# LayerXcom/zero-chain

Hardware: AMD Instinct MI355X
Metric: Groth16 proofs/sec (Transfer circuit) (higher is better)
Workload: dtype u32 limbs (Fq 381-bit: 14 x 28-bit; Fr 255-bit: 8 x 32-bit; modular integer arithmetic)

## Files before the change

### include/zkamd.h

```cpp
#ifndef ZKAMD_H
#define ZKAMD_H

#include <stddef.h>
#include <stdint.h>

#ifdef __cplusplus
extern "C" {
#endif

typedef int32_t zk_status;

enum {
    ZK_OK = 0,
    ZK_ERR_ASSIGNMENT_MISSING = 1,
    ZK_ERR_DIVISION_BY_ZERO = 2,
    ZK_ERR_UNSATISFIABLE = 3,
    ZK_ERR_POLYNOMIAL_DEGREE_TOO_LARGE = 4,
    ZK_ERR_UNEXPECTED_IDENTITY = 5,
    ZK_ERR_IO = 6,
    ZK_ERR_MALFORMED_VERIFYING_KEY = 7,
    ZK_ERR_UNCONSTRAINED_VARIABLE = 8,
    ZK_ERR_INVALID_ARGUMENT = 16,
    ZK_ERR_DEVICE = 17,
    ZK_ERR_NO_DEVICE = 18,
    ZK_ERR_OUT_OF_MEMORY = 19
};

#define ZK_FR_MONTGOMERY 1u

const char* zk_strerror(zk_status st);
const char* zk_last_error(void);
zk_status zk_device_count(int* count);
void zk_set_host_threads(int n);

zk_status zk_bind_host_to_device(int device, int* numa_node_out, int* n_cpus_out);

typedef struct zk_params zk_params;

typedef struct {
    uint32_t n_ic, n_h, n_l, n_a, n_b_g1, n_b_g2;
    uint32_t log_domain;
    uint32_t window_bits;
    uint32_t n_windows;
    uint32_t device;
    uint64_t device_bytes;
} zk_params_info;

zk_status zk_params_load(const uint8_t* pk_bytes, size_t len, int checked, int device, zk_params** out);
zk_status zk_params_get_info(const zk_params* p, zk_params_info* info);
zk_status zk_params_get_windows(const zk_params* p, uint32_t out[4]);
zk_status zk_params_get_merged(const zk_params* p, uint32_t out[3]);
void zk_params_free(zk_params* p);

typedef struct {
    uint32_t n_rows;
    uint32_t n_inputs;
    uint32_t n_aux;
    uint32_t flags;
    const uint8_t* a;
    const uint8_t* b;
    const uint8_t* c;
    const uint8_t* inputs;
    const uint8_t* aux;
    const uint8_t* a_aux_density;
    const uint8_t* b_input_density;
    const uint8_t* b_aux_density;
} zk_assignment;

zk_status zk_prove(zk_params* p, const zk_assignment* asg, const uint8_t r[32], const uint8_t s[32],
                   uint8_t proof_out[192]);

zk_status zk_prove_batch(zk_params* p, size_t n, const zk_assignment* asgs, const uint8_t* rs,
                         uint8_t* proofs_out);

typedef struct {
    uint32_t n_rows, n_inputs, n_aux, flags;
    const void* d_a;
    const void* d_b;
    const void* d_c;
    const void* d_wit;
    const uint8_t* a_aux_density;
    const uint8_t* b_input_density;
    const uint8_t* b_aux_density;
} zk_batch_dev;
zk_status zk_prove_batch_dev(zk_params* p, size_t n, const zk_batch_dev* batch, const uint8_t* rs,
                             uint8_t* proofs_out);

typedef struct zk_r1cs zk_r1cs;
typedef struct {
    const uint32_t* row_ptr;
    const uint32_t* col;
    const uint8_t* coeff;
} zk_csr;
zk_status zk_r1cs_load(uint32_t n_inputs, uint32_t n_aux, uint32_t n_constraints, const zk_csr* a, const zk_csr* b,
                       const zk_csr* c, int device, zk_r1cs** out);
void zk_r1cs_free(zk_r1cs* r);
zk_status zk_transfer_r1cs_load(int device, zk_r1cs** out);
zk_status zk_transfer_r1cs_fingerprint(uint8_t hash_out[32], uint32_t* n_inputs, uint32_t* n_aux, uint32_t* n_constraints);
zk_status zk_prove_batch_witness(zk_params* p, zk_r1cs* circuit, size_t n, const uint8_t* witness, uint32_t flags,
                                 const uint8_t* rs, uint8_t* proofs_out);

#define ZK_TRANSFER_N_INPUTS 23u
#define ZK_TRANSFER_N_AUX 19955u
typedef struct {
    uint32_t amount, remaining_balance, fee, reserved;
    uint8_t randomness[32], alpha[32], dec_key_sender[32];
    uint8_t proof_generation_key[32], enc_key_recipient[32], enc_balance_left[32], enc_balance_right[32], g_epoch[32];
} zk_transfer_statement;
zk_status zk_transfer_witness(const zk_transfer_statement* st, size_t n, uint32_t flags, uint8_t* witness_out);
zk_status zk_transfer_prove_batch(zk_params* p, zk_r1cs* circuit, size_t n, const zk_transfer_statement* st,
                                  const uint8_t* rs, uint8_t* proofs_out);
zk_status zk_transfer_witness_gpu(zk_r1cs* circuit, const zk_transfer_statement* st, size_t n, uint32_t flags,
                                  uint8_t* witness_out);

typedef struct zk_pipeline zk_pipeline;
zk_status zk_pipeline_create(zk_params* p, zk_r1cs* circuit, zk_pipeline** out);
zk_status zk_pipeline_submit(zk_pipeline* pl, size_t n, const zk_transfer_statement* st, const uint8_t* rs,
                             uint8_t* proofs_out);
zk_status zk_pipeline_wait(zk_pipeline* pl);
int zk_pipeline_lanes(const zk_pipeline* pl);
void zk_pipeline_free(zk_pipeline* pl);

typedef struct {
    uint32_t amount, fee, remaining_balance, reserved;
    uint8_t spending_key[32];
    uint8_t enc_key_recipient[32], enc_balance_left[32], enc_balance_right[32], g_epoch[32];
    uint8_t randomness[32], alpha[32];
} zk_transfer_request;
typedef struct {
    uint8_t proof[192];
    uint8_t enc_key_sender[32], enc_key_recipient[32], left_amount_sender[32], left_amount_recipient[32], left_fee[32],
        right_randomness[32], rsk[32], rvk[32], enc_balance[64], nonce[32];
} zk_confidential_xt;
zk_status zk_spending_key_from_seed(const uint8_t* seed, size_t len, uint8_t spending_key_out[32]);
// ... 173 lines not shown
```

### include/zkamd_sys.rs

```rust
#![allow(non_camel_case_types, dead_code)]
use std::os::raw::{c_char, c_int, c_void};

pub type zk_status = i32;
pub const ZK_OK: zk_status = 0;
pub const ZK_ERR_ASSIGNMENT_MISSING: zk_status = 1;
pub const ZK_ERR_DIVISION_BY_ZERO: zk_status = 2;
pub const ZK_ERR_UNSATISFIABLE: zk_status = 3;
pub const ZK_ERR_POLYNOMIAL_DEGREE_TOO_LARGE: zk_status = 4;
pub const ZK_ERR_UNEXPECTED_IDENTITY: zk_status = 5;
pub const ZK_ERR_IO: zk_status = 6;
pub const ZK_ERR_MALFORMED_VERIFYING_KEY: zk_status = 7;
pub const ZK_ERR_UNCONSTRAINED_VARIABLE: zk_status = 8;
pub const ZK_ERR_INVALID_ARGUMENT: zk_status = 16;
pub const ZK_ERR_DEVICE: zk_status = 17;
pub const ZK_ERR_NO_DEVICE: zk_status = 18;
pub const ZK_ERR_OUT_OF_MEMORY: zk_status = 19;
pub const ZK_SCAN_SENDER: u8 = 1;
pub const ZK_SCAN_RECIPIENT: u8 = 2;
pub const ZK_SCAN_FOUND_SENT: u8 = 1;
pub const ZK_SCAN_FOUND_FEE: u8 = 2;
pub const ZK_SCAN_FOUND_RECEIVED: u8 = 4;
pub const ZK_PROOF_BAD_ENCODING: u8 = 1;
pub const ZK_PROOF_NOT_ON_CURVE: u8 = 2;
pub const ZK_PROOF_NOT_IN_SUBGROUP: u8 = 3;
// ... 188 lines not shown
pub struct zk_anonymous_statement {
    pub amount: u32,
    pub remaining_balance: u32,
    pub s_index: u32,
    pub t_index: u32,
    pub randomness: [u8; 32],
    pub alpha: [u8; 32],
    pub dec_key: [u8; 32],
    pub proof_generation_key: [u8; 32],
    pub g_epoch: [u8; 32],
    pub enc_keys: [[u8; 32]; ZK_ANONYMOUS_SIZE],
    pub left_ciphertexts: [[u8; 32]; ZK_ANONYMOUS_SIZE],
    pub enc_balances_left: [[u8; 32]; ZK_ANONYMOUS_SIZE],
    pub enc_balances_right: [[u8; 32]; ZK_ANONYMOUS_SIZE],
}
#[repr(C)]
#[derive(Clone, Copy)]
pub struct zk_anonymous_request {
    pub amount: u32,
    pub remaining_balance: u32,
    pub s_index: u32,
    pub t_index: u32,
    pub spending_key: [u8; 32],
    pub enc_key_recipient: [u8; 32],
    pub enc_keys_decoy: [[u8; 32]; { ZK_ANONYMOUS_SIZE - 2 }],
    pub enc_balances_left: [[u8; 32]; ZK_ANONYMOUS_SIZE],
    pub enc_balances_right: [[u8; 32]; ZK_ANONYMOUS_SIZE],
    pub g_epoch: [u8; 32],
    pub randomness: [u8; 32],
    pub alpha: [u8; 32],
}
#[repr(C)]
#[derive(Clone, Copy)]
pub struct zk_anonymous_xt {
    pub proof: [u8; 192],
    pub enc_keys: [[u8; 32]; ZK_ANONYMOUS_SIZE],
    pub left_ciphertexts: [[u8; 32]; ZK_ANONYMOUS_SIZE],
    pub right_ciphertext: [u8; 32],
    pub nonce: [u8; 32],
    pub rsk: [u8; 32],
    pub rvk: [u8; 32],
}
#[repr(C)]
#[derive(Clone, Copy)]
pub struct zk_block_account {
    pub enc_key: [u8; 32],
    pub balance: [u8; 64],
    pub pending: [u8; 64],
    pub flags: u32,
}
#[repr(C)]
#[derive(Clone, Copy)]
pub struct zk_block_verdict {
    pub verdict: u8,
    pub detail: u8,
    pub reserved: [u8; 2],
}
#[repr(C)]
#[derive(Clone, Copy)]
pub struct zk_block_stats {
    pub rounds: u32,
    pub proofs_verified: u32,
    pub points_decoded: u32,
    pub reserved: u32,
}

#[link(name = "zkamd")]
extern "C" {
    pub fn zk_strerror(st: zk_status) -> *const c_char;
    pub fn zk_last_error() -> *const c_char;
    pub fn zk_device_count(count: *mut c_int) -> zk_status;
    pub fn zk_set_host_threads(n: c_int);
    pub fn zk_bind_host_to_device(device: c_int, numa_node_out: *mut c_int, n_cpus_out: *mut c_int) -> zk_status;
    pub fn zk_params_load(
        pk_bytes: *const u8,
        len: usize,
        checked: c_int,
        device: c_int,
        out: *mut *mut zk_params,
    ) -> zk_status;
    pub fn zk_params_get_info(p: *const zk_params, info: *mut zk_params_info) -> zk_status;
    pub fn zk_params_get_windows(p: *const zk_params, out: *mut [u32; 4]) -> zk_status;
    pub fn zk_params_get_merged(p: *const zk_params, out: *mut [u32; 3]) -> zk_status;
    pub fn zk_params_free(p: *mut zk_params);
    pub fn zk_prove(
        p: *mut zk_params,
        asg: *const zk_assignment,
        r: *const [u8; 32],
        s: *const [u8; 32],
        proof_out: *mut [u8; 192],
    ) -> zk_status;
    pub fn zk_prove_batch(
        p: *mut zk_params,
        n: usize,
        asgs: *const zk_assignment,
        rs: *const u8,
        proofs_out: *mut u8,
    ) -> zk_status;
    pub fn zk_prove_batch_dev(
        p: *mut zk_params,
        n: usize,
        batch: *const zk_batch_dev,
        rs: *const u8,
        proofs_out: *mut u8,
    ) -> zk_status;
    pub fn zk_r1cs_load(
        n_inputs: u32,
        n_aux: u32,
        n_constraints: u32,
        a: *const zk_csr,
        b: *const zk_csr,
        c: *const zk_csr,
        device: c_int,
        out: *mut *mut zk_r1cs,
    ) -> zk_status;
    pub fn zk_r1cs_free(r: *mut zk_r1cs);
    pub fn zk_transfer_r1cs_load(device: c_int, out: *mut *mut zk_r1cs) -> zk_status;
    pub fn zk_transfer_r1cs_fingerprint(
        hash_out: *mut [u8; 32],
        n_inputs: *mut u32,
        n_aux: *mut u32,
        n_constraints: *mut u32,
    ) -> zk_status;
    pub fn zk_prove_batch_witness(
        p: *mut zk_params,
        circuit: *mut zk_r1cs,
        n: usize,
        witness: *const u8,
        flags: u32,
        rs: *const u8,
        proofs_out: *mut u8,
    ) -> zk_status;
    pub fn zk_transfer_witness(st: *const zk_transfer_statement, n: usize, flags: u32, witness_out: *mut u8) -> zk_status;
    pub fn zk_transfer_prove_batch(
        p: *mut zk_params,
        circuit: *mut zk_r1cs,
        n: usize,
        st: *const zk_transfer_statement,
        rs: *const u8,
        proofs_out: *mut u8,
    ) -> zk_status;
    pub fn zk_transfer_witness_gpu(
        circuit: *mut zk_r1cs,
        st: *const zk_transfer_statement,
        n: usize,
        flags: u32,
        witness_out: *mut u8,
    ) -> zk_status;
    pub fn zk_pipeline_create(p: *mut zk_params, circuit: *mut zk_r1cs, out: *mut *mut zk_pipeline) -> zk_status;
    pub fn zk_pipeline_submit(
        pl: *mut zk_pipeline,
        n: usize,
        st: *const zk_transfer_statement,
        rs: *const u8,
        proofs_out: *mut u8,
    ) -> zk_status;
    pub fn zk_pipeline_wait(pl: *mut zk_pipeline) -> zk_status;
    pub fn zk_pipeline_lanes(pl: *const zk_pipeline) -> c_int;
    pub fn zk_pipeline_free(pl: *mut zk_pipeline);
    pub fn zk_spending_key_from_seed(seed: *const u8, len: usize, spending_key_out: *mut [u8; 32]) -> zk_status;
    pub fn zk_jubjub_base_mul(scalars: *const u8, n: usize, points_out: *mut u8) -> zk_status;
    pub fn zk_elgamal_encrypt(
        values: *const u32,
        randomness: *const u8,
        enc_keys: *const u8,
        n: usize,
// ... 243 lines not shown
```

### zero-chain_amd/_api.py

```python
import ctypes as C

import numpy as np

from . import _lib
from ._shard import shard_bounds, gather_proofs, prove_sharded
from ._lib import (ZkError, ZkLib, ZK_FR_MONTGOMERY, ZK_NTT_INVERSE, ZK_NTT_COSET, ZK_NTT_IN_BITREV,
                   ZK_NTT_OUT_BITREV)

__all__ = ["Parameters", "Proof", "generate_parameters", "generate_random_parameters", "PreparedVerifyingKey", "prepare_verifying_key", "verify_proof", "verify_proofs", "read_proofs",
           "verify_transfer_batch", "jubjub_into_xy", "redjubjub_sign", "redjubjub_verify", "REDJUBJUB_REASONS", "verify_confidential_xts", "verify_anonymous_xts", "execute_confidential_block", "g_epoch", "BLOCK_VERDICTS", "BLOCK_ROLLOVER_DUE", "BLOCK_ROLLED", "INTO_XY_REASONS", "SCAN_SENDER", "SCAN_RECIPIENT", "CONFIDENTIAL_XT_POINTS", "ANONYMOUS_XT_POINTS", "ProvingAssignment", "create_proof", "create_random_proof", "create_proofs", "create_proofs_dev", "stream", "bind_host_to_device", "KernelTimer", "kernel_forms",
           "multiexp", "multiexp_cache_release", "memory_stats", "MultiexpContext", "ConstraintMatrices", "create_proofs_from_witness", "fs_rand", "spending_key_from_seed", "jubjub_base_mul", "elgamal_encrypt", "ElGamalTable", "elgamal_add", "ledger_apply", "LEDGER_SUBTRACT", "LEDGER_SKIP", "LEDGER_SCAN_WIDTH", "balance_query", "ELGAMAL_DECRYPT_LIMIT", "ZERO_CIPHERTEXT", "transfer_requests", "transfer_derive", "gen_proofs", "xt_fields", "gen_proof", "XT_FIELDS",
           "FS_MODULUS", "transfer_statements", "transfer_witness", "transfer_witness_gpu", "transfer_r1cs_fingerprint", "anonymous_r1cs_fingerprint", "ANONYMOUS_N_INPUTS", "ANONYMOUS_N_AUX", "anonymous_statements", "anonymous_requests", "anonymous_derive", "anonymous_gen_proofs", "anonymous_witness", "anonymous_witness_gpu", "anonymous_prove_batch",
           "transfer_prove_batch", "TransferPipeline", "set_host_threads", "TRANSFER_N_INPUTS", "TRANSFER_N_AUX", "EvaluationDomain", "XorShiftRng", "fr_rand", "ZkError", "FR_MODULUS",
           "scalars_to_bytes", "bytes_to_scalars", "load_library", "ZK_FR_MONTGOMERY", "ZK_NTT_INVERSE",
           "ZK_NTT_COSET", "ZK_NTT_IN_BITREV", "ZK_NTT_OUT_BITREV", "shard_bounds", "gather_proofs", "prove_sharded"]

FR_MODULUS = 0x73eda753299d7d483339d80809a1d80553bda402fffe5bfeffffffff00000001
_FR_R_INV = pow(1 << 256, -1, FR_MODULUS)
PROOF_SIZE = 192


def load_library():
    return _lib.load()

# ... 76 lines not shown

def fr_rand(rng):
    while True:
        limbs = [rng.next_u64() for _ in range(4)]
        limbs[3] &= 0xFFFFFFFFFFFFFFFF >> 1
        v = sum(l << (64 * i) for i, l in enumerate(limbs))
        if v < FR_MODULUS:
            return v * _FR_R_INV % FR_MODULUS


class Proof:

    def __init__(self, data):
        data = bytes(data)
        if len(data) != PROOF_SIZE:
            raise ValueError("a proof is exactly 192 bytes")
        self.bytes = data

    @property
    def a(self):
        return self.bytes[:48]

    @property
    def b(self):
        return self.bytes[48:144]

    @property
    def c(self):
        return self.bytes[144:]

    def write(self, writer=None):
        if writer is not None:
            writer.write(self.bytes)
        return self.bytes

    @classmethod
    def read(cls, reader):
        data = reader if isinstance(reader, (bytes, bytearray)) else reader.read(PROOF_SIZE)
        return cls(data)

    def __eq__(self, other):
        return isinstance(other, Proof) and other.bytes == self.bytes

    def __repr__(self):
        return "Proof(%s)" % self.bytes.hex()


class Parameters:

    def __init__(self, lib, handle, pk_bytes):
        self._lib = lib
        self._h = handle
        self._pk = pk_bytes
        info = _lib.ParamsInfo()
        lib.check(lib.zk_params_get_info(handle, C.byref(info)))
        self.info = {f[0]: getattr(info, f[0]) for f in info._fields_}
        self.info.update(zip(("n_merged_a", "n_merged_b1", "n_merged_b2"), self.merged_bases))

    @classmethod
    def read(cls, reader, checked=True, device=0, lib=None):
        lib = lib or _lib.load()
        data = bytes(reader if isinstance(reader, (bytes, bytearray)) else reader.read())
        buf = _u8(data)
        h = C.c_void_p()
        lib.check(lib.zk_params_load(_ptr(buf), buf.size, 1 if checked else 0, device, C.byref(h)))
        return cls(lib, h, data)

    def write(self, writer=None):
        if writer is not None:
            writer.write(self._pk)
        return self._pk

    @property
    def windows(self):
        w = (C.c_uint32 * 4)()
        self._lib.check(self._lib.zk_params_get_windows(self._h, w))
        return tuple(int(x) for x in w)

    @property
    def merged_bases(self):
        n = (C.c_uint32 * 3)()
        self._lib.check(self._lib.zk_params_get_merged(self._h, n))
        return tuple(int(x) for x in n)

    @property
    def vk(self):
        n_ic = self.info["n_ic"]
        b = self._pk
        return {"alpha_g1": b[0:96], "beta_g1": b[96:192], "beta_g2": b[192:384], "gamma_g2": b[384:576],
                "delta_g1": b[576:672], "delta_g2": b[672:864],
                "ic": [b[868 + 96 * i: 868 + 96 * (i + 1)] for i in range(n_ic)]}

    def close(self):
        if self._h:
            self._lib.zk_params_free(self._h)
            self._h = None

    def __del__(self):
        try:
            self.close()
        except Exception:
            pass


G1_GENERATOR = bytes.fromhex(
    "17f1d3a73197d7942695638c4fa9ac0fc3688c4f9774b905a14e3a3f171bac586c55e83ff97a1aeffb3af00adb22c6bb"
    "08b3f481e3aaa0f1a09e30ed741d8ae4fcf5e095d5d00af600db18cb2c04b3edd03cc744a2888ae40caa232946c5e7e1")
G2_GENERATOR = bytes.fromhex(
    "13e02b6052719f607dacd3a088274f65596bd0d09920b61ab5da61bbdc7f5049334cf11213945d57e5ac7d055d042b7e"
    "024aa2b2f08f0a91260805272dc51051c6e47ad4fa403b02b4510b647ae3d1770bac0326a805bbefd48056c8c121bdb8"
    "0606c4a02ea734cc32acd2b02bc28b99cb3e287e85a763af267492ab572e99ab3f370d275cec1da1aaa9075ff05f79be"
    "0ce5d527727d6e118cc9cdc6da2e351aadfd9baa8cbdd3a76d429a695160d12c923ac9cc3baca289e193548608b82801")


def generate_parameters(matrices, alpha, beta, gamma, delta, tau, g1=None, g2=None):
    lib = matrices._lib
    sc = [scalars_to_bytes([int(v)]) for v in (alpha, beta, gamma, delta, tau)]
    b1, b2 = _u8(g1 or G1_GENERATOR, 96), _u8(g2 or G2_GENERATOR, 192)
    n = C.c_size_t(0)
    args = [matrices._h, _ptr(b1), _ptr(b2)] + [_ptr(x) for x in sc]
    lib.check(lib.zk_generate_parameters(*args, None, 0, C.byref(n)))
    out = np.zeros(n.value, dtype=np.uint8)
    lib.check(lib.zk_generate_parameters(*args, _ptr(out), out.size, C.byref(n)))
    return out[:n.value].tobytes()


def generate_random_parameters(matrices, rng, g1=None, g2=None):
    alpha, beta, gamma, delta, tau = (fr_rand(rng) for _ in range(5))
    return generate_parameters(matrices, alpha, beta, gamma, delta, tau, g1=g1, g2=g2)


class PreparedVerifyingKey:

    def __init__(self, lib, handle):
        self._lib = lib
        self._h = handle
        n = C.c_uint32(0)
        lib.check(lib.zk_vk_num_inputs(handle, C.byref(n)))
        self.n_inputs = n.value

    @classmethod
    def read(cls, reader, device=0, lib=None):
        lib = lib or _lib.load()
        buf = _u8(bytes(reader if isinstance(reader, (bytes, bytearray)) else reader.read()))
        h = C.c_void_p()
        lib.check(lib.zk_vk_read(_ptr(buf), buf.size, device, C.byref(h)))
        return cls(lib, h)

    def write(self, writer=None):
        n = C.c_size_t(0)
        self._lib.check(self._lib.zk_vk_write(self._h, None, 0, C.byref(n)))
        out = np.zeros(n.value, dtype=np.uint8)
        self._lib.check(self._lib.zk_vk_write(self._h, _ptr(out), out.size, C.byref(n)))
        data = out.tobytes()
        if writer is not None:
            writer.write(data)
        return data

    def close(self):
        if self._h:
            self._lib.zk_vk_free(self._h)
            self._h = None

    def __del__(self):
        try:
            self.close()
# ... 926 lines not shown
```

### zero-chain_amd/_lib.py

```python
import ctypes as C
import os

HERE = os.path.dirname(os.path.abspath(__file__))
LIB_PATH = os.path.join(HERE, "libzkamd.so")
HOOKS_LIB_PATH = os.path.join(HERE, "libzkamd_hooks.so")

ZK_OK = 0
ZK_FR_MONTGOMERY = 1
ZK_NTT_INVERSE, ZK_NTT_COSET, ZK_NTT_IN_BITREV, ZK_NTT_OUT_BITREV = 1, 2, 4, 8

STATUS_NAMES = {
    0: "Ok", 1: "AssignmentMissing", 2: "DivisionByZero", 3: "Unsatisfiable",
    4: "PolynomialDegreeTooLarge", 5: "UnexpectedIdentity", 6: "IoError",
    7: "MalformedVerifyingKey", 8: "UnconstrainedVariable", 16: "InvalidArgument",
    17: "DeviceError", 18: "NoDevice", 19: "OutOfMemory",
}


class ZkError(Exception):

    def __init__(self, status, detail):
        self.status = status
        self.variant = STATUS_NAMES.get(status, "Unknown")
        super().__init__("%s (%d): %s" % (self.variant, status, detail))
# ... 11 lines not shown


class Csr(C.Structure):
    _fields_ = [("row_ptr", C.c_void_p), ("col", C.c_void_p), ("coeff", C.c_void_p)]


class TransferStatement(C.Structure):
    _fields_ = [("amount", C.c_uint32), ("remaining_balance", C.c_uint32), ("fee", C.c_uint32), ("reserved", C.c_uint32)] + \
               [(n, C.c_uint8 * 32) for n in ("randomness", "alpha", "dec_key_sender", "proof_generation_key",
                                              "enc_key_recipient", "enc_balance_left", "enc_balance_right", "g_epoch")]


class TransferRequest(C.Structure):
    _fields_ = [("amount", C.c_uint32), ("fee", C.c_uint32), ("remaining_balance", C.c_uint32), ("reserved", C.c_uint32)] + \
               [(n, C.c_uint8 * 32) for n in ("spending_key", "enc_key_recipient", "enc_balance_left", "enc_balance_right",
                                              "g_epoch", "randomness", "alpha")]


class ConfidentialXt(C.Structure):
    _fields_ = [("proof", C.c_uint8 * 192)] + \
               [(n, C.c_uint8 * 32) for n in ("enc_key_sender", "enc_key_recipient", "left_amount_sender", "left_amount_recipient",
                                              "left_fee", "right_randomness", "rsk", "rvk")] + \
               [("enc_balance", C.c_uint8 * 64), ("nonce", C.c_uint8 * 32)]


class AnonymousStatement(C.Structure):
    _fields_ = [("amount", C.c_uint32), ("remaining_balance", C.c_uint32), ("s_index", C.c_uint32), ("t_index", C.c_uint32)] + \
               [(n, C.c_uint8 * 32) for n in ("randomness", "alpha", "dec_key", "proof_generation_key", "g_epoch")] + \
               [(n, (C.c_uint8 * 32) * 12) for n in ("enc_keys", "left_ciphertexts", "enc_balances_left", "enc_balances_right")]


class AnonymousRequest(C.Structure):
    _fields_ = [("amount", C.c_uint32), ("remaining_balance", C.c_uint32), ("s_index", C.c_uint32), ("t_index", C.c_uint32),
                ("spending_key", C.c_uint8 * 32), ("enc_key_recipient", C.c_uint8 * 32), ("enc_keys_decoy", (C.c_uint8 * 32) * 10),
                ("enc_balances_left", (C.c_uint8 * 32) * 12), ("enc_balances_right", (C.c_uint8 * 32) * 12),
                ("g_epoch", C.c_uint8 * 32), ("randomness", C.c_uint8 * 32), ("alpha", C.c_uint8 * 32)]


class AnonymousXt(C.Structure):
    _fields_ = [("proof", C.c_uint8 * 192), ("enc_keys", (C.c_uint8 * 32) * 12), ("left_ciphertexts", (C.c_uint8 * 32) * 12)] + \
               [(n, C.c_uint8 * 32) for n in ("right_ciphertext", "nonce", "rsk", "rvk")]


class LedgerOp(C.Structure):
    _fields_ = [("slot", C.c_uint32), ("flags", C.c_uint32), ("left", C.c_uint8 * 32), ("right", C.c_uint8 * 32)]


class BlockAccount(C.Structure):
    _fields_ = [("enc_key", C.c_uint8 * 32), ("balance", C.c_uint8 * 64), ("pending", C.c_uint8 * 64), ("flags", C.c_uint32)]


class BlockVerdict(C.Structure):
    _fields_ = [("verdict", C.c_uint8), ("detail", C.c_uint8), ("reserved", C.c_uint16)]


class BlockStats(C.Structure):
    _fields_ = [(n, C.c_uint32) for n in ("rounds", "proofs_verified", "points_decoded", "reserved")]


class ConfidentialScanResult(C.Structure):
    _fields_ = [("role", C.c_uint8), ("found", C.c_uint8), ("refusal", C.c_uint8), ("reserved", C.c_uint8),
                ("amount_sent", C.c_uint32), ("fee", C.c_uint32), ("amount_received", C.c_uint32)]


class AnonymousScanResult(C.Structure):
    _fields_ = [("members", C.c_uint16), ("found", C.c_uint8), ("refusal", C.c_uint8), ("reserved", C.c_uint32), ("delta", C.c_int64)]


class BatchDev(C.Structure):
    _fields_ = [("n_rows", C.c_uint32), ("n_inputs", C.c_uint32), ("n_aux", C.c_uint32), ("flags", C.c_uint32),
                ("d_a", C.c_void_p), ("d_b", C.c_void_p), ("d_c", C.c_void_p), ("d_wit", C.c_void_p),
                ("a_aux_density", C.c_void_p), ("b_input_density", C.c_void_p), ("b_aux_density", C.c_void_p)]


_PROTOS = {
    "zk_strerror": (C.c_char_p, [C.c_int32]),
    "zk_last_error": (C.c_char_p, []),
    "zk_device_count": (C.c_int32, [C.POINTER(C.c_int)]),
    "zk_set_host_threads": (None, [C.c_int]),
    "zk_params_load": (C.c_int32, [C.c_void_p, C.c_size_t, C.c_int, C.c_int, C.POINTER(C.c_void_p)]),
    "zk_params_get_info": (C.c_int32, [C.c_void_p, C.POINTER(ParamsInfo)]),
    "zk_params_get_windows": (C.c_int32, [C.c_void_p, C.POINTER(C.c_uint32)]),
    "zk_params_get_merged": (C.c_int32, [C.c_void_p, C.POINTER(C.c_uint32)]),
    "zk_bind_host_to_device": (C.c_int32, [C.c_int, C.POINTER(C.c_int), C.POINTER(C.c_int)]),
    "zk_params_free": (None, [C.c_void_p]),
    "zk_prove": (C.c_int32, [C.c_void_p, C.POINTER(Assignment), C.c_void_p, C.c_void_p, C.c_void_p]),
    "zk_prove_batch": (C.c_int32, [C.c_void_p, C.c_size_t, C.POINTER(Assignment), C.c_void_p, C.c_void_p]),
    "zk_prove_batch_dev": (C.c_int32, [C.c_void_p, C.c_size_t, C.POINTER(BatchDev), C.c_void_p, C.c_void_p]),
    "zk_r1cs_load": (C.c_int32, [C.c_uint32, C.c_uint32, C.c_uint32, C.POINTER(Csr), C.POINTER(Csr), C.POINTER(Csr), C.c_int,
                                 C.POINTER(C.c_void_p)]),
    "zk_r1cs_free": (None, [C.c_void_p]),
    "zk_transfer_r1cs_load": (C.c_int32, [C.c_int, C.POINTER(C.c_void_p)]),
    "zk_transfer_r1cs_fingerprint": (C.c_int32, [C.c_void_p, C.POINTER(C.c_uint32), C.POINTER(C.c_uint32), C.POINTER(C.c_uint32)]),
    "zk_anonymous_r1cs_load": (C.c_int32, [C.c_int, C.POINTER(C.c_void_p)]),
    "zk_anonymous_derive": (C.c_int32, [C.POINTER(AnonymousRequest), C.c_size_t, C.POINTER(AnonymousStatement), C.c_void_p]),
    "zk_anonymous_gen_proof_batch": (C.c_int32, [C.c_void_p, C.c_void_p, C.c_void_p, C.c_size_t, C.POINTER(AnonymousRequest), C.c_void_p,
                                                 C.POINTER(AnonymousXt)]),
    "zk_anonymous_r1cs_fingerprint": (C.c_int32, [C.c_void_p, C.POINTER(C.c_uint32), C.POINTER(C.c_uint32), C.POINTER(C.c_uint32)]),
    "zk_prove_batch_witness": (C.c_int32, [C.c_void_p, C.c_void_p, C.c_size_t, C.c_void_p, C.c_uint32, C.c_void_p, C.c_void_p]),
    "zk_transfer_witness": (C.c_int32, [C.POINTER(TransferStatement), C.c_size_t, C.c_uint32, C.c_void_p]),
    "zk_transfer_witness_gpu": (C.c_int32, [C.c_void_p, C.POINTER(TransferStatement), C.c_size_t, C.c_uint32, C.c_void_p]),
    "zk_transfer_prove_batch": (C.c_int32, [C.c_void_p, C.c_void_p, C.c_size_t, C.POINTER(TransferStatement), C.c_void_p,
                                            C.c_void_p]),
    "zk_pipeline_create": (C.c_int32, [C.c_void_p, C.c_void_p, C.POINTER(C.c_void_p)]),
    "zk_pipeline_submit": (C.c_int32, [C.c_void_p, C.c_size_t, C.POINTER(TransferStatement), C.c_void_p, C.c_void_p]),
    "zk_pipeline_wait": (C.c_int32, [C.c_void_p]),
    "zk_pipeline_lanes": (C.c_int, [C.c_void_p]),
    "zk_pipeline_free": (None, [C.c_void_p]),
    "zk_spending_key_from_seed": (C.c_int32, [C.c_void_p, C.c_size_t, C.c_void_p]),
    "zk_jubjub_base_mul": (C.c_int32, [C.c_void_p, C.c_size_t, C.c_void_p]),
    "zk_elgamal_encrypt": (C.c_int32, [C.c_void_p, C.c_void_p, C.c_void_p, C.c_size_t, C.c_void_p, C.c_void_p]),
    "zk_elgamal_table_create": (C.c_int32, [C.c_uint32, C.c_int, C.POINTER(C.c_void_p)]),
    "zk_elgamal_decrypt": (C.c_int32, [C.c_void_p, C.c_size_t, C.c_void_p, C.c_void_p, C.c_void_p, C.c_size_t, C.c_uint64, C.c_void_p,
                                       C.c_void_p]),
    "zk_elgamal_table_free": (None, [C.c_void_p]),
    "zk_elgamal_add": (C.c_int32, [C.c_void_p, C.c_void_p, C.c_void_p, C.c_void_p, C.c_size_t, C.c_int, C.c_void_p, C.c_void_p]),
    "zk_confidential_scan": (C.c_int32, [C.c_void_p, C.c_size_t, C.POINTER(ConfidentialXt), C.c_void_p, C.c_uint64,
                                         C.POINTER(ConfidentialScanResult)]),
    "zk_anonymous_scan": (C.c_int32, [C.c_void_p, C.c_size_t, C.POINTER(AnonymousXt), C.c_void_p, C.c_uint64, C.POINTER(AnonymousScanResult)]),
    "zk_elgamal_ledger_apply": (C.c_int32, [C.c_size_t, C.c_void_p, C.c_size_t, C.POINTER(LedgerOp), C.c_int, C.c_void_p, C.c_void_p, C.c_void_p,
                                            C.c_void_p]),
    "zk_transfer_derive": (C.c_int32, [C.POINTER(TransferRequest), C.c_size_t, C.POINTER(TransferStatement), C.c_void_p]),
    "zk_transfer_gen_proof_batch": (C.c_int32, [C.c_void_p, C.c_void_p, C.c_void_p, C.c_size_t, C.POINTER(TransferRequest), C.c_void_p,
                                                C.POINTER(ConfidentialXt)]),
    "zk_anonymous_witness": (C.c_int32, [C.POINTER(AnonymousStatement), C.c_size_t, C.c_uint32, C.c_void_p]),
    "zk_anonymous_witness_gpu": (C.c_int32, [C.c_void_p, C.POINTER(AnonymousStatement), C.c_size_t, C.c_uint32, C.c_void_p]),
    "zk_generate_parameters": (C.c_int32, [C.c_void_p] + [C.c_void_p] * 7 + [C.c_void_p, C.c_size_t, C.POINTER(C.c_size_t)]),
    "zk_params_write_vk": (C.c_int32, [C.c_void_p, C.c_void_p, C.c_size_t, C.POINTER(C.c_size_t)]),
    "zk_vk_prepare": (C.c_int32, [C.c_void_p, C.c_size_t, C.c_int, C.POINTER(C.c_void_p)]),
    "zk_vk_read": (C.c_int32, [C.c_void_p, C.c_size_t, C.c_int, C.POINTER(C.c_void_p)]),
    "zk_vk_write": (C.c_int32, [C.c_void_p, C.c_void_p, C.c_size_t, C.POINTER(C.c_size_t)]),
    "zk_vk_num_inputs": (C.c_int32, [C.c_void_p, C.POINTER(C.c_uint32)]),
    "zk_vk_free": (None, [C.c_void_p]),
    "zk_verify_batch": (C.c_int32, [C.c_void_p, C.c_size_t, C.c_void_p, C.c_void_p, C.c_size_t, C.c_void_p]),
    "zk_verify_batch_rlc": (C.c_int32, [C.c_void_p, C.c_size_t, C.c_void_p, C.c_void_p, C.c_size_t, C.c_void_p]),
    "zk_verify_proof": (C.c_int32, [C.c_void_p, C.c_void_p, C.c_void_p, C.c_size_t, C.POINTER(C.c_int)]),
    "zk_proof_read_batch": (C.c_int32, [C.c_void_p, C.c_size_t, C.c_void_p, C.c_void_p]),
    "zk_jubjub_into_xy": (C.c_int32, [C.c_void_p, C.c_size_t, C.c_int, C.c_void_p, C.c_void_p]),
    "zk_confidential_verify_batch": (C.c_int32, [C.c_void_p, C.c_size_t, C.POINTER(ConfidentialXt), C.c_void_p, C.c_void_p, C.c_size_t,
                                                 C.c_void_p, C.c_void_p]),
    "zk_anonymous_verify_batch": (C.c_int32, [C.c_void_p, C.c_size_t, C.POINTER(AnonymousXt), C.c_void_p, C.c_void_p, C.c_size_t,
                                              C.c_void_p, C.c_void_p]),
    "zk_confidential_block_execute": (C.c_int32, [C.c_void_p, C.c_size_t, C.POINTER(ConfidentialXt), C.c_void_p, C.c_void_p, C.c_void_p, C.c_size_t,
                                                  C.POINTER(BlockAccount), C.c_size_t, C.c_void_p, C.c_void_p, C.POINTER(BlockAccount),
                                                  C.POINTER(BlockVerdict), C.POINTER(BlockStats)]),
    "zk_g_epoch": (C.c_int32, [C.c_uint32, C.c_void_p]),
    "zk_redjubjub_sign": (C.c_int32, [C.c_size_t, C.c_void_p, C.c_void_p, C.c_void_p, C.c_void_p, C.c_void_p]),
    "zk_redjubjub_verify_batch": (C.c_int32, [C.c_size_t, C.c_void_p, C.c_void_p, C.c_void_p, C.c_void_p, C.c_int, C.c_void_p, C.c_void_p]),
    "zk_anonymous_prove_batch": (C.c_int32, [C.c_void_p, C.c_void_p, C.c_size_t, C.POINTER(AnonymousStatement), C.c_void_p,
                                             C.c_void_p]),
    "zk_msm_create": (C.c_int32, [C.c_int, C.c_void_p, C.c_size_t, C.c_int, C.c_int, C.c_int, C.POINTER(C.c_void_p)]),
    "zk_msm_create_variable": (C.c_int32, [C.c_int, C.c_void_p, C.c_size_t, C.c_int, C.c_int, C.c_int, C.POINTER(C.c_void_p)]),
    "zk_msm_run": (C.c_int32, [C.c_void_p, C.c_void_p, C.c_uint32, C.c_void_p]),
    "zk_msm_run_dev": (C.c_int32, [C.c_void_p, C.c_void_p, C.c_uint32, C.c_void_p]),
    "zk_msm_free": (None, [C.c_void_p]),
    "zk_msm_g1": (C.c_int32, [C.c_void_p, C.c_void_p, C.c_size_t, C.c_void_p]),
    "zk_msm_g2": (C.c_int32, [C.c_void_p, C.c_void_p, C.c_size_t, C.c_void_p]),
    "zk_msm_cache_release": (None, []),
    "zk_memory_stats": (None, [C.POINTER(C.c_uint64)]),
    "zk_ntt_fr": (C.c_int32, [C.c_void_p, C.c_uint32, C.c_int, C.c_int]),
    "zk_ntt_create": (C.c_int32, [C.c_uint32, C.c_int, C.POINTER(C.c_void_p)]),
    "zk_ntt_run_dev": (C.c_int32, [C.c_void_p, C.c_void_p, C.c_uint32, C.c_uint32]),
    "zk_ntt_free": (None, [C.c_void_p]),
    "zk_debug_field_mul": (C.c_int32, [C.c_int, C.c_void_p, C.c_void_p, C.c_void_p, C.c_size_t]),
    "zk_profile_begin": (None, []),
    "zk_profile_get": (C.c_int, [C.c_char_p, C.POINTER(C.c_double)]),
# ... 44 lines not shown
```

### zero-chain_amd/csrc/msm_group.h

```cpp
#pragma once
#include <stdio.h>
#include <stdlib.h>
#include <string.h>
#include <string>
#include <vector>
#include <algorithm>
#include <utility>
#include <mutex>
#include "../../include/zkamd.h"
#include "gpu_rt.h"
#include "host_common.h"
#include "host_math.h"
#include "msm.h"
#include "coop_tail.h"
#include "msm_plan.h"

namespace zkrt {

inline uint32_t pick_window(size_t n, int group) {
    const char* env = getenv(group == 2 ? "ZKAMD_WINDOW_BITS_G2" : group == 3 ? "ZKAMD_WINDOW_BITS_G1A" : "ZKAMD_WINDOW_BITS_G1");
    if (!env) env = getenv("ZKAMD_WINDOW_BITS");
    if (env && atoi(env) >= 2 && atoi(env) <= 22) return (uint32_t)atoi(env);
    const char* benv = getenv(group == 2 ? "ZKAMD_BUCKET_COST_G2" : "ZKAMD_BUCKET_COST_G1");
    const double beta = benv && atof(benv) > 0 ? atof(benv) : (group == 2 ? 12.0 : group == 1 ? 4.0 : 6.0);
// ... 70 lines not shown
#ifdef ZK_HAVE_RED_ASM
template <> constexpr bool asm_reduce<zkdev::Fq28>() { return true; }
template <>
void launch_red_asm<zkdev::Fq28>(const zkdev::XYZZ<zkdev::Fq28>* tsums, const uint32_t* cnt, const uint32_t* toff, const uint32_t* tbase,
                                 zkdev::XYZZ<zkdev::Fq28>* S, zkdev::XYZZ<zkdev::Fq28>* A, uint32_t nb, uint32_t L, dim3 grid,
                                 hipStream_t st, uint32_t* n_fallback, uint32_t* fallback);
#endif
#ifdef ZK_HAVE_MADD_ASM
int persist_wgs(int group = 1);
template <> constexpr bool asm_loop<zkdev::Fq28>() { return true; }
template <> constexpr bool asm_loop<zkdev::Fq2x>() { return true; }
template <>
void launch_asm_loop<zkdev::Fq28>(const zkdev::Affine<zkdev::Fq28>* table, const uint32_t* pairs, const uint4* sorted,
                                  const uint32_t* d_total, zkdev::XYZZ<zkdev::Fq28>* tsums, uint32_t* d_nredo, uint32_t* redo,
                                  unsigned blocks, hipStream_t st);
template <>
void launch_asm_loop<zkdev::Fq2x>(const zkdev::Affine<zkdev::Fq2x>* table, const uint32_t* pairs, const uint4* sorted,
                                  const uint32_t* d_total, zkdev::XYZZ<zkdev::Fq2x>* tsums, uint32_t* d_nredo, uint32_t* redo,
                                  unsigned blocks, hipStream_t st);
#endif

template <class HF, class DF>
struct MsmGroup {
    typedef zkhost::Affine<HF> HAffine;
    typedef zkhost::Point<HF> HPoint;
    typedef zkdev::Affine<DF> DAffine;
    typedef zkdev::XYZZ<DF> DPoint;
    static_assert(sizeof(HAffine) == 2 * 4 * zkdev::HostWords<DF>::N, "host affine layout");
    static_assert(sizeof(HPoint) == 4 * 4 * zkdev::HostWords<DF>::N, "host point layout");

    static constexpr bool IS_G2 = zkdev::HostWords<DF>::N == 24;

    uint32_t c = 0, maxd = 0, nb = 0;
    size_t n_points = 0;
    DevBuf table;
    DevBuf jobs_d, cnt, off, toff, ntasks, hist, tclass, sorted, heavy, light, blockbase, coarse, tbase, rank, pairs, tsums, red_r, red_w, red_t, result, redo;
    DPoint* res_dev = nullptr;
    PinBuf pin_jobs;
    size_t bytes = 0;
    DevBuf dstat;

    zk_status set_geometry(uint32_t c_, size_t n, bool with_table) {
        c = c_;
        maxd = with_table ? zkdev::msm_max_digits(c) : 1u;
        nb = 1u << (c - 2);
        n_points = n;
        const uint32_t npos = with_table ? zkdev::MSM_NPOS : 1u;
        if ((uint64_t)n_points * npos >= (1ull << 31)) return fail(ZK_ERR_INVALID_ARGUMENT, "doubling table too large");
        bytes = sizeof(DAffine) * n_points * npos;
        return ZK_OK;
    }
    void alias(const MsmGroup& o, uint32_t c_) {
        (void)set_geometry(c_, o.n_points, true);
        bytes = 0;
        table.borrow(o.table);
    }
    zk_status decode_enqueue(const uint8_t* bases, size_t n, uint32_t c_, bool with_table, DevBuf& raw, DevBuf& map, hipStream_t st);
    zk_status decode_finish(const char* what, uint32_t* n_inf, size_t* bad_index = nullptr) {
        uint32_t v[2] = {0xffffffffu, 0};
        HIP_TRY(hipMemcpy(v, dstat.p, 8, hipMemcpyDeviceToHost));
        if (v[0] != 0xffffffffu) {
            if (bad_index) *bad_index = v[0];
            return fail(ZK_ERR_IO, std::string("invalid ") + (IS_G2 ? "G2" : "G1") + " encoding at " + what + " " + std::to_string(v[0]));
        }
        *n_inf = v[1];
        return ZK_OK;
    }
    zk_status table_enqueue(DevBuf& scratch, hipStream_t st);
    zk_status finish_build(bool checked, const char* what, bool with_table);
    zk_status build(const std::vector<HAffine>& pts, uint32_t c_, bool checked, const char* what, bool with_table = true);

    zk_status build_with_tail(const std::vector<HAffine>& pts, const MsmGroup& o, size_t from, size_t count, uint32_t c_);

    zk_status enqueue(std::vector<MsmJob>& jobs, std::vector<HPoint>& out, hipStream_t st, bool to_host = true);
    zk_status normalize_to_host(const DPoint* src, size_t n, HPoint* out, DevBuf& stage, hipStream_t st);
    zk_status export_to_host(const DPoint* src, size_t n, HPoint* out, DevBuf& stage, hipStream_t st);
    zk_status normalize2_to_host(const DPoint* src0, const DPoint* src1, size_t n, HPoint* out0, HPoint* out1, DevBuf& stage0,
                                 DevBuf& stage1, hipStream_t st);
    zk_status collect(hipStream_t st) {
        HIP_TRY(hipStreamSynchronize(st));
        return ZK_OK;
    }
    zk_status run(std::vector<MsmJob>& jobs, std::vector<HPoint>& out);

private:
    zk_status launch_table_build(DevBuf& scratch, hipStream_t st);
    zk_status reserve(const MsmPlan& p, bool to_host);
    zk_status upload_jobs(const std::vector<MsmJob>& jobs, const MsmPlan& p, hipStream_t st);
    zk_status sort_pairs(const MsmPlan& p, hipStream_t st);
    zk_status order_tasks(const MsmPlan& p, hipStream_t st);
    zk_status accumulate(const MsmPlan& p, hipStream_t st);
    zk_status merge_partials(const MsmPlan& p, hipStream_t st);
    zk_status level1(const MsmPlan& p, hipStream_t st);
    zk_status tail(const MsmPlan& p, hipStream_t st);
    zk_status copy_to_host(const DevBuf& stage, size_t n, HPoint* out, hipStream_t st);
    void dump_redo(const MsmPlan& p, hipStream_t st, bool after_level1);
    void dump_heavy(const MsmPlan& p, hipStream_t st);
    enum Counter { N_TASKS = 0, N_HEAVY = 1, N_REDO = 2, N_LIGHT = 4, N_FALLBACK = 5 };
    uint32_t* counter(const MsmPlan& p, Counter k) const { return hist.as<uint32_t>() + 2 * p.n_class + k; }
    DPoint* node_s() const { return red_r.as<DPoint>(); }
    DPoint* node_w() const { return red_w.as<DPoint>(); }
    DPoint* job_sums(const MsmPlan& p) const { return node_w() + p.nj * (size_t)p.T; }
};

typedef MsmGroup<zkhost::Fq, zkdev::Fq> MsmG1;
typedef zkdev::Fq2x DevFq2;
typedef MsmGroup<zkhost::Fq2, DevFq2> MsmG2;
typedef zkhost::Affine<zkhost::Fq> HG1A;
typedef zkhost::Affine<zkhost::Fq2> HG2A;
typedef zkhost::Point<zkhost::Fq> HG1;
typedef zkhost::Point<zkhost::Fq2> HG2;

zk_status calibrate_g2_accumulate(const zkdev::Affine<DevFq2>* table, uint32_t n_entries, float ms[2]);
zk_status calibrate_g1_reduce(const zkdev::Affine<zkdev::Fq28>* table, uint32_t n_entries, float ms[2]);

#ifndef ZK_MSM_GROUP_INSTANTIATE
extern template struct MsmGroup<zkhost::Fq, zkdev::Fq>;
extern template struct MsmGroup<zkhost::Fq2, DevFq2>;
extern template zk_status check_points_dev<zkhost::Fq, zkdev::Fq>(const zkdev::Affine<zkdev::Fq>*, size_t, const char*);
extern template zk_status check_points_dev<zkhost::Fq2, DevFq2>(const zkdev::Affine<DevFq2>*, size_t, const char*);
extern template zk_status check_points_host<zkhost::Fq, zkdev::Fq>(const std::vector<zkhost::Affine<zkhost::Fq>>&, const char*);
extern template zk_status check_points_host<zkhost::Fq2, DevFq2>(const std::vector<zkhost::Affine<zkhost::Fq2>>&, const char*);
#endif

}
```

### zero-chain_amd/csrc/ntt.h

```cpp
#pragma once
#include "dev_field.h"
#include "prove_plan.h"

namespace zkdev {

constexpr int NTT_MAX_G = 8;
constexpr int NTT_TILE_LOG = 10;
constexpr int NTT_THREADS = 256;
constexpr int NTT_BIG_LOG = 17, NTT_BIG_MAX_G = 10, NTT_BIG_TILE_LOG = 12, NTT_BIG_THREADS = 1024;

struct NttPass {
    uint32_t log_n;
    uint32_t t0;
    uint32_t g;
    uint32_t log_cw;
    uint32_t dif;
    uint32_t stride;
    uint32_t src_stride;
    uint32_t src_valid;
};

ZK_DI Fr ld_fr(const uint32_t* p) {
    Fr r;
    const uint4* q = reinterpret_cast<const uint4*>(p);
// ... 161 lines not shown
        if (e & 1u) r = mul(r, base);
        base = sqr(base);
        e >>= 1;
    }
    return r;
}

static __global__ void __launch_bounds__(256)
k_fr_pow_table(uint32_t* out, const uint32_t* __restrict__ base, const uint32_t* __restrict__ scale,
               uint32_t log_n, uint32_t mode, uint32_t raw_out, uint32_t count) {
    uint32_t i = blockIdx.x * blockDim.x + threadIdx.x;
    if (i >= count) return;
    uint32_t e = i;
    if (mode == 1) e = log_n ? (__builtin_bitreverse32(i) >> (32 - log_n)) : 0;
    Fr v;
    if (mode == 3) {
        v = Fr::zero();
        v.l[0] = log_n ? (__builtin_bitreverse32(i) >> (32 - log_n)) : 0;
        v = to_mont(v);
    } else {
        v = fr_pow_u32(ld_fr(base), e);
    }
    if (mode) v = mul(v, ld_fr(scale));
    if (raw_out) v = from_mont(v);
    st_fr(out + (size_t)i * 8, v);
}

static __global__ void __launch_bounds__(256)
k_fr_convert(uint32_t* out, const uint32_t* __restrict__ in, uint32_t from, size_t count, uint32_t* bad = nullptr) {
    size_t i = (size_t)blockIdx.x * blockDim.x + threadIdx.x;
    if (i >= count) return;
    Fr v = ld_fr(in + i * 8);
    if (bad && fr_geq_r(v)) raise_flag(bad, ZK_BAD_SCALAR);
    st_fr(out + i * 8, from ? from_mont(v) : to_mont(v));
}

static __global__ void __launch_bounds__(256)
k_fr_first_noncanonical(const uint32_t* __restrict__ in, size_t count, uint32_t* stat) {
    size_t i = (size_t)blockIdx.x * blockDim.x + threadIdx.x;
    if (i >= count) return;
    if (fr_geq_r(ld_fr(in + i * 8))) atomicMin(&stat[0], (uint32_t)i);
}

template <class C>
static __global__ void __launch_bounds__(64)
k_field_mul_raw(uint32_t* out, const uint32_t* __restrict__ a, const uint32_t* __restrict__ b, uint32_t n) {
    uint32_t i = blockIdx.x * blockDim.x + threadIdx.x;
    if (i >= n) return;
    Fp<C> x, y;
#pragma unroll
    for (int j = 0; j < C::N; j++) {
        x.l[j] = a[(size_t)i * C::N + j];
        y.l[j] = b[(size_t)i * C::N + j];
    }
    Fp<C> z = mul(x, y);
#pragma unroll
    for (int j = 0; j < C::N; j++) out[(size_t)i * C::N + j] = z.l[j];
}

struct R1csMat {
    const uint32_t* row_ptr;
    const uint32_t* col;
    const uint32_t* coeff;
};
static __global__ void __launch_bounds__(256)
k_r1cs_eval(R1csMat ma, R1csMat mb, R1csMat mc, const uint32_t* __restrict__ z, uint32_t* out, uint32_t n_con,
            uint32_t n_in, uint32_t nv, uint32_t n_rows, size_t out_mat_stride) {
    uint32_t row = blockIdx.x * blockDim.x + threadIdx.x;
    if (row >= n_rows) return;
    const uint32_t mat = blockIdx.y;
    const size_t p = blockIdx.z;
    const R1csMat m = mat == 0 ? ma : (mat == 1 ? mb : mc);
    const uint32_t* zp = z + p * (size_t)nv * 8;
    Fr acc = Fr::zero();
    if (row < n_con) {
        for (uint32_t k = m.row_ptr[row]; k < m.row_ptr[row + 1]; k++)
            acc = add(acc, mul(ld_fr(m.coeff + (size_t)k * 8), ld_fr(zp + (size_t)m.col[k] * 8)));
    } else if (mat == 0) {
        acc = ld_fr(zp + (size_t)(row - n_con) * 8);
    }
    st_fr(out + (size_t)mat * out_mat_stride * 8 + (p * n_rows + row) * 8, acc);
}

static __global__ void __launch_bounds__(256)
k_build_scalars(uint32_t* wit_out, uint32_t* cvec, const uint32_t* __restrict__ wit, const uint32_t* __restrict__ tail,
                const zkrt::CJobLayout L, uint32_t mont, uint32_t* bad, const uint32_t* __restrict__ groups) {
    uint32_t i = blockIdx.x * blockDim.x + threadIdx.x;
    if (i >= L.wstride + L.gb1) return;
    const size_t p = blockIdx.y;
    uint32_t* cv = cvec + p * (size_t)L.cstride * 8;
    const uint32_t nv = L.w_one, fold = L.fold;
    Fr r = ld_fr(tail + (p * 3 + 1) * 8);
    Fr sR = fold ? mul(ld_fr(tail + (p * 3 + 2) * 8), Fr::r2()) : Fr::zero();
    Fr v;
    if (i >= L.w_sum_a) {
        const uint32_t g = i - L.w_sum_a;
        const uint32_t* mem = groups + (L.ga + L.gb2 + L.gb1 + 1);
        Fr sum = Fr::zero();
        for (uint32_t k = groups[g]; k < groups[g + 1]; k++) {
            const Fr raw = ld_fr(wit + (p * nv + mem[k]) * 8);
            if (!fr_geq_r(raw)) sum = add(sum, raw);
        }
        if (i < L.wstride) {
            v = mont ? from_mont(sum) : sum;
            if (fold && g < L.ga) st_fr(cv + (size_t)(L.sum_a + g) * 8, mul(v, sR));
            st_fr(wit_out + (p * L.wstride + i) * 8, v);
        } else {
            const Fr rz = mont ? mul(sum, r) : mul(mul(sum, r), Fr::r2());
            st_fr(cv + (size_t)(L.sum_b1 + (i - L.wstride)) * 8, rz);
        }
        return;
    }
    if (i < nv) {
        Fr raw = ld_fr(wit + (p * nv + i) * 8);
        if (fr_geq_r(raw)) {
            raise_flag(bad, ZK_BAD_SCALAR);
            raw = Fr::zero();
        }
        if (i == 0 && !(mont ? raw == Fr::one() : (raw.l[0] == 1u && (raw.l[1] | raw.l[2] | raw.l[3] | raw.l[4] | raw.l[5] | raw.l[6] | raw.l[7]) == 0u)))
            raise_flag(bad, ZK_BAD_ONE);
        Fr rz;
        if (mont) {
            v = from_mont(raw);
            rz = mul(raw, r);
        } else {
            v = raw;
            rz = mul(mul(raw, r), Fr::r2());
        }
        if (i >= L.n_in) st_fr(cv + (size_t)(L.aux + (i - L.n_in)) * 8, v);
        st_fr(cv + (size_t)(L.rz + i) * 8, rz);
        if (fold) st_fr(cv + (size_t)(L.sz + i) * 8, mul(v, sR));
        if (L.in_tail && i < L.n_in) st_fr(cv + (size_t)(L.in_tail + i) * 8, v);
    } else {
        v = ld_fr(tail + (p * 3 + (i - nv)) * 8);
        if (i == nv) st_fr(cv + (size_t)L.r * 8, r);
        if (fold && i == nv + 1) st_fr(cv + (size_t)L.rs * 8, mul(r, sR));
        if (fold && i == nv + 2) st_fr(cv + (size_t)L.s * 8, v);
    }
    st_fr(wit_out + (p * L.wstride + i) * 8, v);
}

}
```

### zero-chain_amd/csrc/prove_plan.h

```cpp
#pragma once
#include <stddef.h>
#include <stdint.h>
#include <stdlib.h>

namespace zkrt {

constexpr size_t PROVE_FOLD_IN_MSM_MAX = 128;

struct ProveTunables {
    size_t batch_chunk;
    size_t host_chunk;
    size_t fold_in_msm_max;
    size_t g2_lone_max;
    size_t host_normalize_max;
    size_t split_min;
    bool no_overlap;
    bool trace_host;

    static ProveTunables read() {
        auto env_chunk = [](const char* name, size_t dflt) {
            const char* e = getenv(name);
            return e && atoi(e) > 0 ? (size_t)atoi(e) : dflt;
        };
        auto env_n = [](const char* name, size_t dflt) {
            const char* e = getenv(name);
            return e ? (size_t)atoll(e) : dflt;
        };
        ProveTunables t;
        t.batch_chunk = env_chunk("ZKAMD_BATCH_CHUNK", 1024);
        t.host_chunk = env_chunk("ZKAMD_HOST_CHUNK", 0);
        t.fold_in_msm_max = env_n("ZKAMD_FOLD_IN_MSM_MAX", PROVE_FOLD_IN_MSM_MAX);
        t.g2_lone_max = env_n("ZKAMD_G2_LONE_MAX", 2);
        t.host_normalize_max = env_n("ZKAMD_HOST_NORMALIZE_MAX", 16);
        t.split_min = env_n("ZKAMD_SPLIT_MIN", 64);
        t.no_overlap = getenv("ZKAMD_NO_OVERLAP") != nullptr;
        t.trace_host = getenv("ZKAMD_TRACE_HOST") != nullptr;
        return t;
    }
};

struct CJobLayout {
    uint32_t n_in, n_aux, head, ga, gb2, gb1, fold, derived;
    uint32_t w_one, w_sum_a, w_sum_b2, wstride;
    uint32_t aux, rz, r;
    uint32_t sz, s, rs;
    uint32_t in_tail;
    uint32_t sum_b1, sum_a;
    uint32_t cstride;
};

inline CJobLayout cjob_layout(uint32_t n_in, uint32_t n_aux, uint32_t head, uint32_t ga, uint32_t gb2, uint32_t gb1, bool fold,
                              bool derived) {
    const uint32_t nv = n_in + n_aux;
    CJobLayout L = {};
    L.n_in = n_in; L.n_aux = n_aux; L.head = head; L.ga = ga; L.gb2 = gb2; L.gb1 = gb1; L.fold = fold; L.derived = derived;
    L.w_one = nv;
    L.w_sum_a = nv + 3;
    L.w_sum_b2 = L.w_sum_a + ga;
    L.wstride = L.w_sum_b2 + gb2;
    uint32_t at = head;
    auto section = [&at](uint32_t len) { const uint32_t off = at; at += len; return off; };
    L.aux = section(n_aux);
    L.rz = section(nv);
    L.r = section(1);
    if (fold) {
        L.sz = section(nv);
        L.s = section(1);
        L.rs = section(1);
    }
    if (derived) L.in_tail = section(n_in);
    L.sum_b1 = section(gb1);
    if (fold) L.sum_a = section(ga);
    L.cstride = at;
    return L;
}

enum class PG1 { G1, G1_LONE, G1D, G1D_LONE };
enum class PMap { MAP_C, MAP_CF, MAP_CD, MAP_CFD };

struct ProvePlan {
    bool fold_in_msm;
    bool host_norm;
    bool g2_lone;
    bool split;
    bool one_stream;
    PG1 g1;
    PMap map;
    CJobLayout layout;
};

inline ProvePlan prove_plan(size_t np, uint32_t n_in, uint32_t n_aux, uint32_t n_rows, size_t m, uint32_t ga, uint32_t gb2,
                            uint32_t gb1, bool derived, const ProveTunables& tun) {
    ProvePlan p;
    p.fold_in_msm = np <= tun.fold_in_msm_max;
    p.host_norm = np <= tun.host_normalize_max;
    p.g2_lone = np <= tun.g2_lone_max;
    p.split = np >= tun.split_min;
    p.one_stream = tun.no_overlap;
    p.g1 = derived ? (p.split ? PG1::G1D : PG1::G1D_LONE) : (p.split ? PG1::G1 : PG1::G1_LONE);
    p.map = derived ? (p.fold_in_msm ? PMap::MAP_CFD : PMap::MAP_CD) : (p.fold_in_msm ? PMap::MAP_CF : PMap::MAP_C);
    p.layout = cjob_layout(n_in, n_aux, derived ? 2 * n_rows : (uint32_t)m, ga, gb2, gb1, p.fold_in_msm, derived);
    return p;
}

}
```

### zero-chain_amd/csrc/zkamd.cpp

```cpp
#include <stdio.h>
#include <stdlib.h>
#include <string.h>
#include <string>
#include <vector>
#include <map>
#include <thread>
#include <chrono>
#include <algorithm>
#include <new>
#include <mutex>
#include <condition_variable>
#include <deque>
#if defined(__linux__)
#include <sched.h>
#endif

#include "../../include/zkamd.h"
#include "gpu_rt.h"
#include "host_common.h"
#include "host_math.h"
#include "ntt.h"
#include "msm_group.h"
#include "prove_plan.h"
#include "transfer_witness.h"
#include "handles.h"
#include "transfer_r1cs.h"

using zkdev::MsmJob;
using zkdev::NttPass;

namespace {

using namespace zkrt;

using zkhost::Fr;

Fr fr_from_u64(uint64_t v) {
    Fr x = Fr::zero();
    x.l[0] = v;
    return x.to_mont();
}
Fr fr_const(const uint64_t (&v)[4]) {
    Fr x;
    for (int i = 0; i < 4; i++) x.l[i] = v[i];
    return x;
}


struct NttPlan {
    uint32_t log_n = 0;
    size_t n = 0;
    DevBuf tw_fwd, tw_inv;
    DevBuf s1_plain, s1_mont, s2;
    DevBuf sc_plain, sc_mont;
    DevBuf coset_fwd, coset_inv;
    DevBuf dt;
    DevBuf consts;
    Fr w_inv, n_inv, z_inv;
    DevBuf scratch;
    size_t bytes = 0;

    static int tile_form() {
        static const int f = [] {
            const char* e = getenv("ZKAMD_NTT_TILES");
            return !e ? 1 : !strcmp(e, "big") ? 2 : !strcmp(e, "small") ? 0 : 1;
        }();
        return f;
    }
    static bool big(uint32_t k) { return tile_form() == 2 && k >= (uint32_t)zkdev::NTT_BIG_LOG; }
    static bool mid(uint32_t k) { return tile_form() == 1 && k >= (uint32_t)zkdev::NTT_BIG_LOG; }
    static uint32_t threads_for(uint32_t k) { return mid(k) ? 512u : big(k) ? (uint32_t)zkdev::NTT_BIG_THREADS : (uint32_t)zkdev::NTT_THREADS; }
    static bool latency_form(uint32_t k, uint32_t batch) { return k >= 9 && k < (uint32_t)zkdev::NTT_BIG_LOG && ((uint64_t)batch << k) <= (1u << 17); }
    static std::vector<NttPass> passes(uint32_t k, bool dif, uint32_t stride, bool latency = false) {
        std::vector<NttPass> out;
        if (k == 0) return out;
        std::vector<uint32_t> gs;
        uint32_t tile_log;
        if (latency) {
            tile_log = 8;
            const uint32_t np = (k + 7) / 8;
            for (uint32_t i = 0; i < np; i++) gs.push_back(k / np + (i < k % np ? 1 : 0));
        } else if (mid(k)) {
            tile_log = 11;
            const uint32_t g0 = 11, rest = k - g0, np = (rest + 8) / 9;
            std::vector<uint32_t> strided;
            for (uint32_t i = 0; i < np; i++) strided.push_back(rest / np + (i < rest % np ? 1 : 0));
            if (dif) {
                gs = strided;
                gs.push_back(g0);
            } else {
                gs.push_back(g0);
                gs.insert(gs.end(), strided.begin(), strided.end());
            }
        } else {
            const uint32_t max_g = big(k) ? zkdev::NTT_BIG_MAX_G : zkdev::NTT_MAX_G;
            tile_log = big(k) ? zkdev::NTT_BIG_TILE_LOG : zkdev::NTT_TILE_LOG;
            const uint32_t np = (k + max_g - 1) / max_g;
            for (uint32_t i = 0; i < np; i++) gs.push_back(k / np + (i < k % np ? 1 : 0));
        }
        uint32_t t0 = 0;
        for (uint32_t g : gs) {
            NttPass p;
            p.log_n = k;
            p.t0 = t0;
            p.g = g;
            uint32_t lcw = tile_log - p.g;
            if (lcw > k - p.g) lcw = k - p.g;
// ... 85 lines not shown
            if (shmem > 65536) {
                static std::mutex mu;
                static uint64_t raised = 0;
                std::lock_guard<std::mutex> lock(mu);
                const uint64_t bit = 1ull << (g_device & 63);
                if (!(raised & bit)) {
                    HIP_TRY(hipFuncSetAttribute(reinterpret_cast<const void*>(zkdev::k_ntt_pass), hipFuncAttributeMaxDynamicSharedMemorySize, 160 * 1024));
                    raised |= bit;
                }
            }
#endif
            ZK_LAUNCH_SYNC(zkdev::k_ntt_pass, grid, dim3(latency ? (1u << (p.g + p.log_cw - 1)) : threads_for(log_n)), shmem, g_stream, data, s, tw,
                           i == 0 ? pre : (const uint32_t*)nullptr,
                           i + 1 == ps.size() ? post : (const uint32_t*)nullptr, p, i == 0 && s ? bad : (uint32_t*)nullptr,
                           i + 1 == ps.size() ? sub : (const uint32_t*)nullptr, sub_stride);
        }
        if (ps.empty() && (pre || post || src)) return fail(ZK_ERR_INVALID_ARGUMENT, "size-1 transform");
        HIP_TRY(hipGetLastError());
        return ZK_OK;
    }
};



struct Reader {
    const uint8_t* p;
    size_t left;
    bool take(size_t n, const uint8_t** out) {
        if (left < n) return false;
        *out = p;
        p += n;
        left -= n;
        return true;
    }
    bool u32be(uint32_t* v) {
        const uint8_t* b;
        if (!take(4, &b)) return false;
        *v = ((uint32_t)b[0] << 24) | ((uint32_t)b[1] << 16) | ((uint32_t)b[2] << 8) | b[3];
        return true;
    }
};

zk_status read_g1(Reader& r, HG1A* out, const char* what, bool allow_inf = false) {
    const uint8_t* b;
    if (!r.take(96, &b)) return fail(ZK_ERR_IO, std::string("unexpected end of parameters in ") + what);
    if (zkhost::g1_from_uncompressed(b, out) != zkhost::DEC_OK) return fail(ZK_ERR_IO, std::string("invalid G1 encoding in ") + what);
    if (!allow_inf && out->is_inf()) return fail(ZK_ERR_IO, std::string("point at infinity in ") + what);
    return ZK_OK;
}
zk_status read_g2(Reader& r, HG2A* out, const char* what, bool allow_inf = false) {
    const uint8_t* b;
    if (!r.take(192, &b)) return fail(ZK_ERR_IO, std::string("unexpected end of parameters in ") + what);
    if (zkhost::g2_from_uncompressed(b, out) != zkhost::DEC_OK) return fail(ZK_ERR_IO, std::string("invalid G2 encoding in ") + what);
    if (!allow_inf && out->is_inf()) return fail(ZK_ERR_IO, std::string("point at infinity in ") + what);
    return ZK_OK;
}

bool scalar_lt_r(const uint64_t v[4]) { return !Fr::geq_p(v); }

}

struct zk_params {
    int device = 0;
    uint32_t n_ic = 0, n_h = 0, n_l = 0, n_a = 0, n_b1 = 0, n_b2 = 0;
    uint32_t log_m = 0;
    size_t m = 0;
    uint32_t off_h = 0, off_l = 0, off_a = 0, off_b1 = 0;
    MsmG1 g1;
    MsmG1 g1a, g1_lone;
    MsmG2 g2;
    MsmG2 g2_lone;
    NttPlan ntt;
    struct Derived {
        bool ready = false;
        uint64_t circuit = 0;
        uint32_t serial = 0;
        uint32_t n_rows = 0;
        uint32_t off_a = 0, off_b1 = 0;
        std::vector<int32_t> pos;
        double bind_ms = 0;
    } drv;
    MsmG1 g1d, g1d_lone;
    DevBuf map_cd, map_cfd;
    std::vector<uint8_t> dens_key;
    DevBuf map_a, map_b2, map_c, map_cf;
    uint32_t map_nv = 0;
    struct Groups {
        std::vector<uint32_t> ptr, mem;
        uint32_t count() const { return ptr.empty() ? 0u : (uint32_t)ptr.size() - 1; }
        uint32_t merged() const { return (uint32_t)mem.size() - count(); }
    } grp_a, grp_b1, grp_b2;
    uint32_t mg_a = 0, mg_b2 = 0, mg_b1 = 0;
    DevBuf grp_dev;
    DevBuf abc, wit, cvec, tail, stage_a, stage_b, stage_c, stage_w, fold_tbl, fold_c, fold_a1, fold_c1, fold_b2;
    PinBuf pin_g1, pin_g2, pin_tail;
    DevBuf bad;
    PinBuf pin_bad;
    bool alpha_g1_inf = false, beta_g1_inf = false, beta_g2_inf = false, delta_g1_inf = false, delta_g2_inf = false;
    std::vector<uint8_t> vk_bytes;
    std::vector<MsmJob> jobs1, jobs1a, jobs2;
    std::vector<HG1> res1, res1a;
    std::vector<HG2> res2;
};

namespace {

zk_status calibrate_kernel_forms(zk_params* P);

void group_equal_points(const uint8_t* enc, uint32_t n, size_t size, zk_params::Groups& G) {
    std::vector<uint32_t> order;
    order.reserve(n);
    for (uint32_t i = 0; i < n; i++)
        if (!(enc[i * size] & 0x40)) order.push_back(i);
    std::sort(order.begin(), order.end(), [&](uint32_t x, uint32_t y) {
        const int c = memcmp(enc + x * size, enc + y * size, size);
        return c ? c < 0 : x < y;
    });
    std::vector<std::pair<uint32_t, uint32_t>> runs;
    for (size_t i = 0, j; i < order.size(); i = j) {
        for (j = i + 1; j < order.size() && !memcmp(enc + order[i] * size, enc + order[j] * size, size);) j++;
        if (j - i > 1) runs.push_back({order[i], (uint32_t)i});
    }
    std::sort(runs.begin(), runs.end());
    G.ptr.assign(1, 0u);
    G.mem.clear();
    for (const auto& run : runs) {
        for (size_t j = run.second; j < order.size() && !memcmp(enc + run.first * size, enc + order[j] * size, size); j++)
            G.mem.push_back(order[j]);
        G.ptr.push_back((uint32_t)G.mem.size());
    }
}

zk_status params_load(const uint8_t* pk, size_t len, int checked, int device, zk_params** out) {
    ZK_TRY(use_device(device));
    zk_params* P = new (std::nothrow) zk_params();
    if (!P) return fail(ZK_ERR_OUT_OF_MEMORY, "host allocation failed");
    struct Guard {
        zk_params* p;
        ~Guard() { delete p; }
    } guard{P};
    P->device = device;
    Reader r{pk, len};
    HG1A alpha_g1, beta_g1, delta_g1;
    HG2A beta_g2, gamma_g2, delta_g2;
    ZK_TRY(read_g1(r, &alpha_g1, "vk.alpha_g1", true));
    ZK_TRY(read_g1(r, &beta_g1, "vk.beta_g1", true));
    ZK_TRY(read_g2(r, &beta_g2, "vk.beta_g2", true));
    ZK_TRY(read_g2(r, &gamma_g2, "vk.gamma_g2", true));
    ZK_TRY(read_g1(r, &delta_g1, "vk.delta_g1", true));
    ZK_TRY(read_g2(r, &delta_g2, "vk.delta_g2", true));
    P->alpha_g1_inf = alpha_g1.is_inf();
    P->beta_g1_inf = beta_g1.is_inf();
    P->beta_g2_inf = beta_g2.is_inf();
    P->delta_g1_inf = delta_g1.is_inf();
    P->delta_g2_inf = delta_g2.is_inf();
    if (!r.u32be(&P->n_ic)) return fail(ZK_ERR_IO, "unexpected end of parameters (ic length)");
    if ((size_t)P->n_ic * 96 > r.left) return fail(ZK_ERR_IO, "unexpected end of parameters in vk.ic");
    std::vector<HG1A> ic(P->n_ic);
    for (uint32_t i = 0; i < P->n_ic; i++) ZK_TRY(read_g1(r, &ic[i], "vk.ic"));

    P->vk_bytes.assign(pk, pk + (len - r.left));
    struct Section {
        const uint8_t* at;
        uint32_t n;
        const char* what;
        bool inf_ok;
    };
    auto locate = [&](uint32_t* n, size_t size, const char* what, const uint8_t** at) -> zk_status {
        if (!r.u32be(n)) return fail(ZK_ERR_IO, std::string("unexpected end of parameters (length of ") + what + ")");
        if ((size_t)*n * size > r.left) return fail(ZK_ERR_IO, std::string("unexpected end of parameters in ") + what);
        (void)r.take((size_t)*n * size, at);
        return ZK_OK;
    };
    const uint8_t *at_h, *at_l, *at_a, *at_b1, *at_b2;
    ZK_TRY(locate(&P->n_h, 96, "h", &at_h));
    ZK_TRY(locate(&P->n_l, 96, "l", &at_l));
    ZK_TRY(locate(&P->n_a, 96, "a", &at_a));
    ZK_TRY(locate(&P->n_b1, 96, "b_g1", &at_b1));
    ZK_TRY(locate(&P->n_b2, 192, "b_g2", &at_b2));
    group_equal_points(at_a, P->n_a, 96, P->grp_a);
    group_equal_points(at_b1, P->n_b1, 96, P->grp_b1);
    group_equal_points(at_b2, P->n_b2, 192, P->grp_b2);
    const Section sec1[7] = {{at_h, P->n_h, "h", false},       {at_l, P->n_l, "l", false},          {at_a, P->n_a, "a", false},
                             {pk, 1, "vk.alpha_g1", true},     {pk + 576, 1, "vk.delta_g1", true},  {at_b1, P->n_b1, "b_g1", false},
                             {pk + 96, 1, "vk.beta_g1", true}};
    const Section sec2[3] = {{at_b2, P->n_b2, "b_g2", false}, {pk + 192, 1, "vk.beta_g2", true}, {pk + 672, 1, "vk.delta_g2", true}};
    P->off_h = 0;
    P->off_l = P->n_h;
    P->off_a = P->off_l + P->n_l;
    P->off_b1 = P->off_a + P->n_a + 2;
    auto gather = [](const Section* sec, int k, size_t size, std::vector<uint8_t>& out) {
        size_t total = 0;
        for (int i = 0; i < k; i++) total += sec[i].n;
        out.resize(total * size);
        size_t at = 0;
        for (int i = 0; i < k; i++) {
            memcpy(out.data() + at, sec[i].at, (size_t)sec[i].n * size);
            at += (size_t)sec[i].n * size;
        }
        return total;
    };
    std::vector<uint8_t> enc1, enc2;
    const size_t n1 = gather(sec1, 7, 96, enc1), n2 = gather(sec2, 3, 192, enc2);
    auto name_of = [](const Section* sec, int k, size_t idx) -> const Section& {
        for (int i = 0; i < k; i++) {
            if (idx < sec[i].n) return sec[i];
            idx -= sec[i].n;
        }
        return sec[k - 1];
    };
    auto infinity_check = [&](const Section* sec, int k, size_t size, const std::vector<uint8_t>& enc, uint32_t n_inf) -> zk_status {
        if (!n_inf) return ZK_OK;
        size_t idx = 0;
        for (int i = 0; i < k; i++)
            for (uint32_t j = 0; j < sec[i].n; j++, idx++)
                if ((enc[idx * size] & 0x40) && !sec[i].inf_ok) return fail(ZK_ERR_IO, std::string("point at infinity in ") + sec[i].what);
        return ZK_OK;
    };

    size_t m = (size_t)P->n_h + 1;
    if (m < 2 || (m & (m - 1))) return fail(ZK_ERR_IO, "h query length + 1 is not a power of two");
    P->m = m;
    while (((size_t)1 << P->log_m) < m) P->log_m++;
    {
        std::vector<HG1A> vk1 = ic;
        vk1.push_back(alpha_g1);
        vk1.push_back(beta_g1);
        vk1.push_back(delta_g1);
        ZK_TRY((check_points_host<zkhost::Fq, zkdev::Fq>(vk1, "vk (G1: ic | alpha | beta | delta)")));
        ZK_TRY((check_points_host<zkhost::Fq2, DevFq2>(std::vector<HG2A>{beta_g2, gamma_g2, delta_g2}, "vk (G2: beta | gamma | delta)")));
    }
    const uint32_t c_avg = pick_window(((size_t)P->n_h + P->n_l + P->n_a + P->n_b1) / 2, 4);
    const uint32_t c1 = pick_window((size_t)P->n_h + P->n_l + P->n_b1, 1);
    const uint32_t c2 = pick_window(P->n_b2, 2);
    {
        DevBuf raw1, raw2, map1, map2, scratch1, scratch2;
        ZK_TRY(P->g1.decode_enqueue(enc1.data(), n1, c1, true, raw1, map1, g_stream));
        ZK_TRY(P->g2.decode_enqueue(enc2.data(), n2, c2, true, raw2, map2, g_stream2));
        HIP_TRY(hipStreamSynchronize(g_stream));
        HIP_TRY(hipStreamSynchronize(g_stream2));
        uint32_t inf1 = 0, inf2 = 0;
        size_t bad1 = (size_t)-1, bad2 = (size_t)-1;
        zk_status d1 = P->g1.decode_finish("", &inf1, &bad1);
        if (d1 != ZK_OK) return bad1 != (size_t)-1 ? fail(ZK_ERR_IO, std::string("invalid G1 encoding in ") + name_of(sec1, 7, bad1).what) : d1;
        zk_status d2 = P->g2.decode_finish("", &inf2, &bad2);
        if (d2 != ZK_OK) return bad2 != (size_t)-1 ? fail(ZK_ERR_IO, std::string("invalid G2 encoding in ") + name_of(sec2, 3, bad2).what) : d2;
        ZK_TRY(infinity_check(sec1, 7, 96, enc1, inf1));
        ZK_TRY(infinity_check(sec2, 3, 192, enc2, inf2));
        if (checked) {
            ZK_TRY((check_points_dev<zkhost::Fq, zkdev::Fq>(P->g1.table.as<zkdev::Affine<zkdev::Fq>>(), n1, "parameters (G1)")));
            ZK_TRY((check_points_dev<zkhost::Fq2, DevFq2>(P->g2.table.as<zkdev::Affine<DevFq2>>(), n2, "parameters (G2)")));
        }
        ZK_TRY(P->g1.table_enqueue(scratch1, g_stream));
        ZK_TRY(P->g2.table_enqueue(scratch2, g_stream2));
        HIP_TRY(hipStreamSynchronize(g_stream));
        HIP_TRY(hipStreamSynchronize(g_stream2));
    }
    P->g1a.alias(P->g1, pick_window(P->n_a, 3));
    P->g1_lone.alias(P->g1, c_avg);
    P->g2_lone.alias(P->g2, getenv("ZKAMD_WINDOW_BITS_G2") || c2 <= 10 ? c2 : 10u);
    ZK_TRY(P->ntt.init(P->log_m));
    ZK_TRY(calibrate_kernel_forms(P));
    guard.p = nullptr;
    *out = P;
    return ZK_OK;
}

zk_status calibrate_kernel_forms(zk_params* P) {
#if defined(ZK_HAVE_MADD_ASM) && defined(ZK_HAVE_RED_ASM)
    std::lock_guard<std::mutex> lock(g_forms_mu);
    KernelForms& F = g_forms[P->device & 63];
    if (F.done) return ZK_OK;
    const uint32_t n2 = (uint32_t)std::min<size_t>(P->g2.n_points * (size_t)zkdev::MSM_NPOS, 1u << 24);
    const uint32_t n1 = (uint32_t)std::min<size_t>(P->g1.n_points * (size_t)zkdev::MSM_NPOS, 1u << 24);
    if (n1 < 1024 || n2 < 1024 || getenv("ZKAMD_NO_CALIBRATE")) {
        F.done = true;
        return ZK_OK;
    }
    ZK_TRY(calibrate_g2_accumulate(P->g2.table.as<zkdev::Affine<DevFq2>>(), n2, &F.ms[0]));
    ZK_TRY(calibrate_g1_reduce(P->g1.table.as<zkdev::Affine<zkdev::Fq28>>(), n1, &F.ms[2]));
    const float slow = hook_env("ZKAMD_INJECT_SCRATCH_SLOW") && atoi(hook_env("ZKAMD_INJECT_SCRATCH_SLOW")) ? 3.0f : 1.0f;
    F.ms[0] *= slow;
    F.ms[2] *= slow;
    F.form[0] = F.ms[0] > 1.4f * F.ms[1] ? 1u : 0u;
    F.form[1] = F.ms[2] > 1.4f * F.ms[3] ? 1u : 0u;
    F.done = true;
#else
    (void)P;
#endif
    return ZK_OK;
}

zk_params* params_clone_for_lane(const zk_params* P) {
    zk_params* Q = new (std::nothrow) zk_params();
    if (!Q) return nullptr;
    Q->device = P->device;
    Q->n_ic = P->n_ic; Q->n_h = P->n_h; Q->n_l = P->n_l; Q->n_a = P->n_a; Q->n_b1 = P->n_b1; Q->n_b2 = P->n_b2;
    Q->log_m = P->log_m;
    Q->m = P->m;
    Q->off_h = P->off_h; Q->off_l = P->off_l; Q->off_a = P->off_a; Q->off_b1 = P->off_b1;
    Q->g1.alias(P->g1, P->g1.c);
    Q->g1a.alias(P->g1, P->g1a.c);
    Q->g1_lone.alias(P->g1, P->g1_lone.c);
    Q->g2.c = P->g2.c; Q->g2.maxd = P->g2.maxd; Q->g2.nb = P->g2.nb; Q->g2.n_points = P->g2.n_points;
    Q->g2.table.borrow(P->g2.table);
    Q->g2_lone.alias(P->g2, P->g2_lone.c);
    if (P->drv.ready) {
        Q->drv = P->drv;
        Q->g1d.alias(P->g1d, P->g1d.c);
        Q->g1d_lone.alias(P->g1d, P->g1d_lone.c);
    }
    Q->ntt.log_n = P->ntt.log_n;
    Q->ntt.n = P->ntt.n;
    Q->ntt.tw_fwd.borrow(P->ntt.tw_fwd);
    Q->ntt.tw_inv.borrow(P->ntt.tw_inv);
    Q->ntt.s1_plain.borrow(P->ntt.s1_plain);
    Q->ntt.s1_mont.borrow(P->ntt.s1_mont);
    Q->ntt.s2.borrow(P->ntt.s2);
    Q->ntt.dt.borrow(P->ntt.dt);
    Q->ntt.sc_plain.borrow(P->ntt.sc_plain);
    Q->ntt.sc_mont.borrow(P->ntt.sc_mont);
    Q->ntt.coset_fwd.borrow(P->ntt.coset_fwd);
    Q->ntt.coset_inv.borrow(P->ntt.coset_inv);
    Q->ntt.consts.borrow(P->ntt.consts);
    Q->alpha_g1_inf = P->alpha_g1_inf; Q->beta_g1_inf = P->beta_g1_inf; Q->beta_g2_inf = P->beta_g2_inf;
    Q->delta_g1_inf = P->delta_g1_inf; Q->delta_g2_inf = P->delta_g2_inf;
    Q->vk_bytes = P->vk_bytes;
    Q->grp_a = P->grp_a; Q->grp_b1 = P->grp_b1; Q->grp_b2 = P->grp_b2;
    return Q;
}
zk_r1cs* r1cs_clone_for_lane(const zk_r1cs* R) {
    zk_r1cs* Q = new (std::nothrow) zk_r1cs();
    if (!Q) return nullptr;
    Q->device = R->device;
    Q->id = R->id;
    Q->n_in = R->n_in; Q->n_aux = R->n_aux; Q->n_con = R->n_con;
    for (int m = 0; m < 3; m++) {
        Q->row_ptr[m].borrow(R->row_ptr[m]);
        Q->col[m].borrow(R->col[m]);
        Q->coeff[m].borrow(R->coeff[m]);
    }
    Q->a_aux_density = R->a_aux_density;
    Q->b_input_density = R->b_input_density;
    Q->b_aux_density = R->b_aux_density;
    return Q;
}

zk_status ensure_maps(zk_params* P, uint32_t n_in, uint32_t n_aux, const uint8_t* a_aux_d, const uint8_t* b_in_d,
                      const uint8_t* b_aux_d) {
    const char* merge_env = getenv("ZKAMD_MERGE_BASES");
    const bool merge = !(merge_env && atoi(merge_env) == 0);
    std::vector<uint8_t> key;
    key.reserve(9 + n_in + 2 * (size_t)n_aux);
    for (int i = 0; i < 4; i++) key.push_back((uint8_t)(n_in >> (8 * i)));
    for (int i = 0; i < 4; i++) key.push_back((uint8_t)(n_aux >> (8 * i)));
    key.insert(key.end(), a_aux_d, a_aux_d + n_aux);
    key.insert(key.end(), b_in_d, b_in_d + n_in);
    key.insert(key.end(), b_aux_d, b_aux_d + n_aux);
    for (int i = 0; i < 4; i++) key.push_back((uint8_t)((P->drv.ready ? P->drv.serial : 0u) >> (8 * i)));
    key.push_back(merge ? 1 : 0);
    if (key == P->dens_key) return ZK_OK;
    const uint32_t nv = n_in + n_aux;
    std::vector<int32_t> ma(nv + 3, -1), mb1(nv + 3, -1), mb2(nv + 3, -1);
    std::vector<uint32_t> var_a, var_b;
    var_a.reserve(P->n_a);
    var_b.reserve(P->n_b1);
    uint32_t pa = n_in;
    for (uint32_t i = 0; i < n_in; i++) {
        ma[i] = (int32_t)i;
        var_a.push_back(i);
    }
    for (uint32_t j = 0; j < n_aux; j++)
        if (a_aux_d[j]) {
            ma[n_in + j] = (int32_t)pa++;
            var_a.push_back(n_in + j);
        }
    if (pa != P->n_a)
        return fail(ZK_ERR_IO, "the A density of the assignment (" + std::to_string(pa) + ") differs from the key's a query (" +
                                   std::to_string(P->n_a) + ")");
    if (!P->alpha_g1_inf) ma[nv] = (int32_t)P->n_a;
    ma[nv + 1] = (int32_t)P->n_a + 1;
    uint32_t pb = 0;
    for (uint32_t i = 0; i < n_in; i++)
        if (b_in_d[i]) {
            mb1[i] = mb2[i] = (int32_t)pb++;
            var_b.push_back(i);
        }
    for (uint32_t j = 0; j < n_aux; j++)
        if (b_aux_d[j]) {
            mb1[n_in + j] = mb2[n_in + j] = (int32_t)pb++;
            var_b.push_back(n_in + j);
        }
    if (pb != P->n_b1 || pb != P->n_b2)
        return fail(ZK_ERR_IO, "the B density of the assignment (" + std::to_string(pb) + ") differs from the key's b queries (" +
                                   std::to_string(P->n_b1) + " in G1, " + std::to_string(P->n_b2) + " in G2)");
    if (!P->beta_g1_inf) mb1[nv] = (int32_t)P->n_b1;
    if (!P->beta_g2_inf) mb2[nv] = (int32_t)P->n_b2;
    mb2[nv + 2] = (int32_t)P->n_b2 + 1;
    static const zk_params::Groups none;
    std::vector<uint32_t> gptr(1, 0u), gmem;
    auto mute = [&](const zk_params::Groups& G, const std::vector<uint32_t>& var, std::vector<int32_t>& map, std::vector<int32_t>& base) {
        for (uint32_t g = 0; g < G.count(); g++) {
            base.push_back((int32_t)G.mem[G.ptr[g]]);
            for (uint32_t k = G.ptr[g]; k < G.ptr[g + 1]; k++) {
                map[var[G.mem[k]]] = -1;
                gmem.push_back(var[G.mem[k]]);
            }
            gptr.push_back((uint32_t)gmem.size());
        }
    };
    std::vector<int32_t> base_a, base_b2, base_b1;
    mute(merge ? P->grp_a : none, var_a, ma, base_a);
    mute(merge ? P->grp_b2 : none, var_b, mb2, base_b2);
    mute(merge ? P->grp_b1 : none, var_b, mb1, base_b1);
    const uint32_t ga = (uint32_t)base_a.size(), gb2 = (uint32_t)base_b2.size(), gb1 = (uint32_t)base_b1.size();
    const CJobLayout W = cjob_layout(n_in, n_aux, (uint32_t)P->m, ga, gb2, gb1, false, false);
    ma.resize(W.wstride, -1);
    mb2.resize(W.wstride, -1);
    for (uint32_t g = 0; g < ga; g++) ma[W.w_sum_a + g] = base_a[g];
    for (uint32_t g = 0; g < gb2; g++) mb2[W.w_sum_b2 + g] = base_b2[g];
    std::vector<int32_t> mh(P->m);
    for (size_t pos = 0; pos < P->m; pos++) {
        uint32_t e = P->log_m ? (__builtin_bitreverse32((uint32_t)pos) >> (32 - P->log_m)) : 0;
        mh[pos] = e < P->n_h ? (int32_t)e : -1;
    }
    auto upload = [](DevBuf& dst, const auto& v) -> zk_status {
        ZK_TRY(dst.ensure(v.size() * 4));
        HIP_TRY(hipMemcpy(dst.p, v.data(), v.size() * 4, hipMemcpyHostToDevice));
        return ZK_OK;
    };
    auto upload_c_map = [&](DevBuf& dst, const CJobLayout& L, const int32_t* head, const int32_t* aux, const int32_t* inputs,
                            uint32_t off_a, uint32_t off_b1) -> zk_status {
        std::vector<int32_t> map(head, head + L.head);
        map.reserve(L.cstride);
        bool fits = true;
        auto section = [&](uint32_t off) { fits = fits && map.size() == off; };
        auto query = [&](const std::vector<int32_t>& q, uint32_t from, uint32_t n, uint32_t off) {
            for (uint32_t i = from; i < from + n; i++) map.push_back(q[i] < 0 ? -1 : (int32_t)(off + q[i]));
        };
        section(L.aux);
        map.insert(map.end(), aux, aux + n_aux);
        section(L.rz);
        query(mb1, 0, nv, off_b1);
        section(L.r);
        query(mb1, nv, 1, off_b1);
        if (L.fold) {
            section(L.sz);
            query(ma, 0, nv, off_a);
            section(L.s);
            query(ma, nv, 1, off_a);
            section(L.rs);
            query(ma, nv + 1, 1, off_a);
        }
        if (L.derived) {
            section(L.in_tail);
            map.insert(map.end(), inputs, inputs + n_in);
        }
        section(L.sum_b1);
        query(base_b1, 0, gb1, off_b1);
        if (L.fold) {
            section(L.sum_a);
            query(base_a, 0, ga, off_a);
        }
        section(L.cstride);
        if (!fits) return fail(ZK_ERR_INVALID_ARGUMENT, "internal: the C map does not follow its layout");
        return upload(dst, map);
    };
    std::vector<int32_t> hk;
    hk.reserve(P->m + n_aux);
    for (size_t pos = 0; pos < P->m; pos++) hk.push_back(mh[pos] < 0 ? -1 : (int32_t)(P->off_h + mh[pos]));
    for (uint32_t j = 0; j < n_aux; j++) hk.push_back((int32_t)(P->off_l + j));
    for (bool fold : {false, true})
        ZK_TRY(upload_c_map(fold ? P->map_cf : P->map_c, cjob_layout(n_in, n_aux, (uint32_t)P->m, ga, gb2, gb1, fold, false), hk.data(),
                            hk.data() + P->m, nullptr, P->off_a, P->off_b1));
    if (P->drv.ready && P->drv.pos.size() == 2 * (size_t)P->drv.n_rows + nv) {
        const zk_params::Derived& D = P->drv;
        const uint32_t head = 2 * D.n_rows;
        for (bool fold : {false, true})
            ZK_TRY(upload_c_map(fold ? P->map_cfd : P->map_cd, cjob_layout(n_in, n_aux, head, ga, gb2, gb1, fold, true), D.pos.data(),
                                D.pos.data() + head + n_in, D.pos.data() + head, D.off_a, D.off_b1));
    }
    gptr.insert(gptr.end(), gmem.begin(), gmem.end());
    ZK_TRY(upload(P->grp_dev, gptr));
    ZK_TRY(upload(P->map_a, ma));
    ZK_TRY(upload(P->map_b2, mb2));
    P->dens_key.swap(key);
    P->map_nv = nv;
    P->mg_a = ga;
    P->mg_b2 = gb2;
    P->mg_b1 = gb1;
    return ZK_OK;
}


static_assert(PROVE_FOLD_IN_MSM_MAX == MSM_FEW_JOBS, "the fold rides in the multiexp up to the few-jobs limit of a launch set");
typedef zkdev::XYZZ<zkdev::Fq> DP1;
struct ChunkRun {
    zk_params* P;
    size_t np;
    const zk_batch_dev* bt;
    size_t first;
    bool derived, mont;
    ProvePlan plan;
    hipStream_t side;
    MsmG2* G2;
    MsmG1* G1C;
    const int32_t* map_c;
    uint32_t *wit, *cvec, *bad;
    const DP1* a_dev = nullptr;

    zk_status scalars(const uint8_t* rs) {
        const CJobLayout& L = plan.layout;
        const uint32_t nv = L.n_in + L.n_aux;
        ZK_TRY(P->wit.ensure(np * (size_t)L.wstride * 32));
        wit = P->wit.as<uint32_t>();
        ZK_TRY(P->pin_tail.ensure(np * 96));
        uint8_t* tail = P->pin_tail.as<uint8_t>();
        memset(tail, 0, np * 96);
        std::vector<uint64_t> rsv(np * 8);
        for (size_t p = 0; p < np; p++) {
            const uint8_t* rr = rs + (first + p) * 64;
            load_scalar_le(rr, &rsv[p * 8]);
            load_scalar_le(rr + 32, &rsv[p * 8 + 4]);
            if (!scalar_lt_r(&rsv[p * 8]) || !scalar_lt_r(&rsv[p * 8 + 4]))
                return fail(ZK_ERR_INVALID_ARGUMENT, "r or s is not a canonical scalar (>= field modulus)");
            tail[p * 96] = 1;
            memcpy(&tail[p * 96 + 32], rr, 64);
        }
        ZK_TRY(P->tail.ensure(np * 96));
        HIP_TRY(hipMemcpyAsync(P->tail.p, tail, np * 96, hipMemcpyHostToDevice, g_stream));
        ZK_TRY(P->bad.ensure(8));
        ZK_TRY(P->pin_bad.ensure(8));
        bad = P->bad.as<uint32_t>();
        HIP_TRY(hipMemsetAsync(bad, 0, 4, g_stream));
        ZK_TRY(P->cvec.ensure(np * (size_t)L.cstride * 32));
        cvec = P->cvec.as<uint32_t>();
        ZK_LAUNCH(zkdev::k_build_scalars, dim3((L.wstride + L.gb1 + 255) / 256, (unsigned)np), dim3(256), 0, g_stream, wit, cvec,
                  (const uint32_t*)bt->d_wit + first * (size_t)nv * 8, P->tail.as<uint32_t>(), L, mont ? 1u : 0u, bad,
                  P->grp_dev.as<uint32_t>());
        return ZK_OK;
    }

    zk_status g2_set() {
        const uint32_t wstride = plan.layout.wstride;
        P->jobs2.clear();
        for (size_t p = 0; p < np; p++) {
            MsmJob j2 = {wit + p * (size_t)wstride * 8, P->map_b2.as<int32_t>(), wstride, 0, (uint32_t)P->g2.n_points, 0, 0, 0};
            P->jobs2.push_back(j2);
        }
        HIP_TRY(hipEventRecord(g_ev_fork, g_stream));
        HIP_TRY(hipStreamWaitEvent(side, g_ev_fork, 0));
        ZK_TRY(G2->enqueue(P->jobs2, P->res2, side, false));
        ZK_TRY(P->pin_g2.ensure(np * sizeof(HG2)));
        if (plan.host_norm) ZK_TRY(G2->export_to_host(G2->res_dev, np, P->pin_g2.as<HG2>(), P->fold_b2, side));
        else ZK_TRY(G2->normalize_to_host(G2->res_dev, np, P->pin_g2.as<HG2>(), P->fold_b2, side));
        return ZK_OK;
    }

    zk_status h_pipeline() {
        const size_t m = P->m;
        const uint32_t n_rows = bt->n_rows, cstride = plan.layout.cstride;
        ZK_TRY(P->abc.ensure((derived ? 2 : 3) * np * m * 32));
        uint32_t* A = P->abc.as<uint32_t>();
        uint32_t* B = A + np * m * 8;
        uint32_t* C = B + np * m * 8;
        const uint32_t* srcs[3] = {(const uint32_t*)bt->d_a + first * (size_t)n_rows * 8,
                                   (const uint32_t*)bt->d_b + first * (size_t)n_rows * 8,
                                   (const uint32_t*)bt->d_c + first * (size_t)n_rows * 8};
        uint32_t* dsts[3] = {A, B, C};
        const uint32_t* s1 = derived ? P->ntt.dt.as<uint32_t>() : mont ? P->ntt.s1_mont.as<uint32_t>() : P->ntt.s1_plain.as<uint32_t>();
        const uint32_t* sc = mont ? P->ntt.sc_mont.as<uint32_t>() : P->ntt.sc_plain.as<uint32_t>();
        for (int k = 0; k < (derived ? 2 : 3); k++)
            ZK_TRY(P->ntt.chain(dsts[k], (uint32_t)np, (uint32_t)m, true, true, nullptr, k < 2 ? s1 : sc, srcs[k], n_rows, n_rows, bad));
        ZK_TRY(P->ntt.chain(A, (uint32_t)(2 * np), (uint32_t)m, false, false, nullptr, nullptr));
        {
            ProfScope ps("h_pointwise");
            if (derived) {
                const size_t count = np * (size_t)n_rows;
                ZK_LAUNCH(zkdev::k_h_live_rows, dim3((unsigned)((count + 255) / 256)), dim3(256), 0, g_stream, (const uint32_t*)A,
                          (const uint32_t*)B, srcs[0], srcs[1], srcs[2], cvec, (uint32_t)m, n_rows, cstride, count);
            } else {
                const size_t count = np * m;
                ZK_LAUNCH(zkdev::k_h_pointwise, dim3((unsigned)((count + 255) / 256)), dim3(256), 0, g_stream, (const uint32_t*)A,
                          (const uint32_t*)B, (const uint32_t*)nullptr, P->ntt.consts.as<uint32_t>() + 8, cvec, (uint32_t)m, cstride, count);
            }
        }
        if (!derived)
            ZK_TRY(P->ntt.chain(cvec, (uint32_t)np, cstride, true, true, nullptr, P->ntt.s2.as<uint32_t>(), nullptr, 0, 0, nullptr,
                                (const uint32_t*)C, (uint32_t)m));
        return ZK_OK;
    }

    zk_status g1_sets() {
        const bool split = plan.split;
        const uint32_t wstride = plan.layout.wstride, cstride = plan.layout.cstride;
        const uint32_t npts1 = (uint32_t)P->g1.n_points, npts1c = (uint32_t)G1C->n_points;
        P->jobs1.clear();
        P->jobs1a.clear();
        for (size_t p = 0; p < np; p++) {
            MsmJob jc = {cvec + p * (size_t)cstride * 8, map_c, cstride, 0, npts1c, 0, 0, 0};
            P->jobs1.push_back(jc);
        }
        for (size_t p = 0; p < np; p++) {
            MsmJob ja = {wit + p * (size_t)wstride * 8, P->map_a.as<int32_t>(), wstride, P->off_a, npts1, 0, 0, 0};
            if (!split && derived) {
                ja.table_base = P->drv.off_a;
                ja.n_table = npts1c;
            }
            (split ? P->jobs1a : P->jobs1).push_back(ja);
        }
        if (split) {
            ZK_TRY(P->g1a.enqueue(P->jobs1a, P->res1a, side, false));
            a_dev = P->g1a.res_dev;
            HIP_TRY(hipEventRecord(g_ev_join, side));
            ZK_TRY(G1C->enqueue(P->jobs1, P->res1, g_stream, false));
            HIP_TRY(hipStreamWaitEvent(g_stream, g_ev_join, 0));
        } else {
            ZK_TRY(G1C->enqueue(P->jobs1, P->res1, g_stream, false));
            a_dev = G1C->res_dev + np;
        }
        return ZK_OK;
    }

    zk_status fold_export() {
        ProfScope ps("proof_fold", g_stream);
        const DP1* cprime = G1C->res_dev;
        const DP1* cfin = cprime;
        if (!plan.fold_in_msm) {
            ZK_TRY(P->fold_tbl.ensure(np * 15 * sizeof(DP1)));
            ZK_TRY(P->fold_c.ensure(np * sizeof(DP1)));
            zkcoop::scale_add(a_dev, cprime, (const uint32_t*)P->tail.as<uint32_t>() + 16, 24u, P->fold_tbl.as<DP1>(),
                              P->fold_c.as<DP1>(), (uint32_t)np, g_stream);
            cfin = P->fold_c.as<DP1>();
        }
        ZK_TRY(P->pin_g1.ensure(2 * np * sizeof(HG1)));
        if (plan.host_norm) {
            ZK_TRY(G1C->export_to_host(a_dev, np, P->pin_g1.as<HG1>() + np, P->fold_a1, g_stream));
            ZK_TRY(G1C->export_to_host(cfin, np, P->pin_g1.as<HG1>(), P->fold_c1, g_stream));
        } else {
            ZK_TRY(G1C->normalize2_to_host(a_dev, cfin, np, P->pin_g1.as<HG1>() + np, P->pin_g1.as<HG1>(), P->fold_a1, P->fold_c1, g_stream));
        }
        return ZK_OK;
    }

    zk_status collect(std::chrono::steady_clock::time_point& t_wait) {
        HIP_TRY(hipMemcpyAsync(P->pin_bad.p, bad, 8, hipMemcpyDeviceToHost, g_stream));
        t_wait = std::chrono::steady_clock::now();
        ZK_TRY(G1C->collect(g_stream));
        ZK_TRY(G2->collect(side));
        const uint32_t flags = P->pin_bad.as<uint32_t>()[0];
        if (flags & zkdev::ZK_BAD_SCALAR)
            return fail(ZK_ERR_INVALID_ARGUMENT, "an assignment scalar (a, b, c, input or aux) is not a canonical field element (>= r)");
        if (flags & zkdev::ZK_BAD_ONE) return fail(ZK_ERR_INVALID_ARGUMENT, "input 0 of an assignment is not ONE = 1");
        return ZK_OK;
    }

    void encode(uint8_t* proofs_out) {
        const unsigned nthreads = host_threads(np, 32);
        uint8_t* const own_affine = g_own_affine_sink;
        auto work = [&](size_t lo, size_t hi) {
            for (size_t p = lo; p < hi; p++)
            {
                uint8_t* out = proofs_out + (first + p) * 192;
                const HG1A pa = zkhost::to_affine(P->pin_g1.as<HG1>()[np + p]), pc = zkhost::to_affine(P->pin_g1.as<HG1>()[p]);
                const HG2A pb = zkhost::to_affine(P->pin_g2.as<HG2>()[p]);
                zkhost::g1_to_compressed(pa, out);
                zkhost::g2_to_compressed(pb, out + 48);
                zkhost::g1_to_compressed(pc, out + 144);
                if (own_affine) {
                    uint8_t* o = own_affine + p * OWN_AFFINE_BYTES;
                    memcpy(o, &pa.x, 48);
                    memcpy(o + 48, &pa.y, 48);
                    memcpy(o + 96, &pb.x, 96);
                    memcpy(o + 192, &pb.y, 96);
                    memcpy(o + 288, &pc.x, 48);
                    memcpy(o + 336, &pc.y, 48);
                }
            }
        };
        auto part = [&](unsigned t) { work(np * t / nthreads, np * (t + 1) / nthreads); };
        run_threads(nthreads, part);
        if (g_own_affine_sink) g_own_affine_sink += np * OWN_AFFINE_BYTES;
    }
};

zk_status prove_chunk(zk_params* P, size_t np, const zk_batch_dev* bt, size_t first, const uint8_t* rs, uint8_t* proofs_out, bool derived) {
    const auto t_begin = std::chrono::steady_clock::now();
    const ProveTunables tun = ProveTunables::read();
    const bool mont = (bt->flags & ZK_FR_MONTGOMERY) != 0;
    if (derived && (!mont || P->drv.n_rows != bt->n_rows)) return fail(ZK_ERR_INVALID_ARGUMENT, "internal: the batch is not the derived set's");
    ChunkRun c = {P, np, bt, first, derived, mont,
                  prove_plan(np, bt->n_inputs, bt->n_aux, bt->n_rows, P->m, P->mg_a, P->mg_b2, P->mg_b1, derived, tun)};
    c.side = c.plan.one_stream ? g_stream : g_stream2;
    c.G2 = c.plan.g2_lone ? &P->g2_lone : &P->g2;
    MsmG1* const g1s[] = {&P->g1, &P->g1_lone, &P->g1d, &P->g1d_lone};
    DevBuf* const maps[] = {&P->map_c, &P->map_cf, &P->map_cd, &P->map_cfd};
    c.G1C = g1s[(int)c.plan.g1];
    c.map_c = maps[(int)c.plan.map]->as<int32_t>();
    ZK_TRY(c.scalars(rs));
    ZK_TRY(c.g2_set());
    ZK_TRY(c.h_pipeline());
    ZK_TRY(c.g1_sets());
    ZK_TRY(c.fold_export());
    std::chrono::steady_clock::time_point t_wait;
    ZK_TRY(c.collect(t_wait));
    const auto t_enc = std::chrono::steady_clock::now();
    c.encode(proofs_out);
    if (tun.trace_host) {
        const auto t_end = std::chrono::steady_clock::now();
        fprintf(stderr, "[zkamd] chunk of %zu: enqueue %.2f ms, wait for the GPU %.2f ms, host encoding %.2f ms\n", np,
                std::chrono::duration<double, std::milli>(t_wait - t_begin).count(),
                std::chrono::duration<double, std::milli>(t_enc - t_wait).count(),
                std::chrono::duration<double, std::milli>(t_end - t_enc).count());
    }
    return ZK_OK;
}

zk_status prove_batch_dev(zk_params* P, size_t n, const zk_batch_dev* bt, const uint8_t* rs, uint8_t* proofs_out, bool derived = false) {
    if (!P || !bt || !rs || !proofs_out) return fail(ZK_ERR_INVALID_ARGUMENT, "null argument");
    if (n == 0) return ZK_OK;
    ZK_TRY(use_device(P->device));
    if (P->delta_g1_inf || P->delta_g2_inf) return fail(ZK_ERR_UNEXPECTED_IDENTITY, "vk.delta is the point at infinity");
    if (bt->n_inputs == 0) return fail(ZK_ERR_INVALID_ARGUMENT, "n_inputs must include ONE");
    if (bt->n_rows > P->m) return fail(ZK_ERR_POLYNOMIAL_DEGREE_TOO_LARGE, "more rows than the key's evaluation domain");
    if (bt->n_inputs != P->n_ic) return fail(ZK_ERR_MALFORMED_VERIFYING_KEY, "number of inputs differs from vk.ic");
    if (bt->n_aux != P->n_l) return fail(ZK_ERR_IO, "number of aux variables differs from the l query");
    if (!bt->d_a || !bt->d_b || !bt->d_c || !bt->d_wit || !bt->a_aux_density || !bt->b_input_density || !bt->b_aux_density)
        return fail(ZK_ERR_ASSIGNMENT_MISSING, "assignment pointer is null");
    ZK_TRY(ensure_maps(P, bt->n_inputs, bt->n_aux, bt->a_aux_density, bt->b_input_density, bt->b_aux_density));
    const size_t chunk = ProveTunables::read().batch_chunk;
    for (size_t first = 0; first < n; first += chunk) {
        size_t np = std::min(chunk, n - first);
        ZK_TRY(prove_chunk(P, np, bt, first, rs, proofs_out, derived));
    }
    return ZK_OK;
}

bool same_circuit(const zk_assignment& x, const zk_assignment& y) {
    return x.n_rows == y.n_rows && x.n_inputs == y.n_inputs && x.n_aux == y.n_aux && x.flags == y.flags &&
           memcmp(x.a_aux_density, y.a_aux_density, x.n_aux) == 0 &&
           memcmp(x.b_input_density, y.b_input_density, x.n_inputs) == 0 &&
           memcmp(x.b_aux_density, y.b_aux_density, x.n_aux) == 0;
}

zk_status prove_batch_host(zk_params* P, size_t n, const zk_assignment* asgs, const uint8_t* rs, uint8_t* proofs_out) {
    if (!P || !asgs || !rs || !proofs_out) return fail(ZK_ERR_INVALID_ARGUMENT, "null argument");
    if (n == 0) return ZK_OK;
    ZK_TRY(use_device(P->device));
    const zk_assignment& z = asgs[0];
    for (size_t i = 0; i < n; i++) {
        const zk_assignment& x = asgs[i];
        if (!x.a || !x.b || !x.c || !x.inputs || !x.aux || !x.a_aux_density || !x.b_input_density || !x.b_aux_density)
            return fail(ZK_ERR_ASSIGNMENT_MISSING, "assignment pointer is null");
        if (i && !same_circuit(z, x)) return fail(ZK_ERR_INVALID_ARGUMENT, "batch mixes different circuits");
    }
    const size_t rb = (size_t)z.n_rows * 32, nvb = (size_t)(z.n_inputs + z.n_aux) * 32;
    const ProveTunables tun = ProveTunables::read();
    const size_t chunk = tun.batch_chunk;
    size_t hc = n > chunk ? chunk : (n >= 512 ? (n + 1) / 2 : n);
    if (tun.host_chunk) hc = std::min(chunk, tun.host_chunk);
    hc = std::min(hc, n);
    const size_t slots = n > hc ? 2 : 1;
    ZK_TRY(P->stage_a.ensure(slots * hc * rb));
    ZK_TRY(P->stage_b.ensure(slots * hc * rb));
    ZK_TRY(P->stage_c.ensure(slots * hc * rb));
    ZK_TRY(P->stage_w.ensure(slots * hc * nvb));
    const hipStream_t copy_stream = g_copy_stream;
    auto stage = [&, copy_stream](size_t slot, size_t first, size_t np) -> zk_status {
        HIP_TRY(hipSetDevice(P->device));
        uint8_t* da = (uint8_t*)P->stage_a.p + slot * hc * rb;
        uint8_t* db = (uint8_t*)P->stage_b.p + slot * hc * rb;
        uint8_t* dc = (uint8_t*)P->stage_c.p + slot * hc * rb;
        uint8_t* dw = (uint8_t*)P->stage_w.p + slot * hc * nvb;
        for (size_t i = 0; i < np; i++) {
            const zk_assignment& x = asgs[first + i];
            HIP_TRY(hipMemcpyAsync(da + i * rb, x.a, rb, hipMemcpyHostToDevice, copy_stream));
            HIP_TRY(hipMemcpyAsync(db + i * rb, x.b, rb, hipMemcpyHostToDevice, copy_stream));
            HIP_TRY(hipMemcpyAsync(dc + i * rb, x.c, rb, hipMemcpyHostToDevice, copy_stream));
            HIP_TRY(hipMemcpyAsync(dw + i * nvb, x.inputs, (size_t)z.n_inputs * 32, hipMemcpyHostToDevice, copy_stream));
            HIP_TRY(hipMemcpyAsync(dw + i * nvb + (size_t)z.n_inputs * 32, x.aux, (size_t)z.n_aux * 32, hipMemcpyHostToDevice,
                                   copy_stream));
        }
        HIP_TRY(hipStreamSynchronize(copy_stream));
        return ZK_OK;
    };
    ZK_TRY(stage(0, 0, hc));
    size_t cur = 0;
    for (size_t first = 0; first < n; first += hc) {
        const size_t np = std::min(hc, n - first), next = first + hc;
        zk_status next_rc = ZK_OK;
        std::string next_err;
        SideThread copier;
        if (next < n)
            copier.start([&, next] {
                next_rc = stage(cur ^ 1, next, std::min(hc, n - next));
                if (next_rc != ZK_OK) next_err = g_err;
// ... 8 lines not shown
        bt.d_c = (uint8_t*)P->stage_c.p + cur * hc * rb;
        bt.d_wit = (uint8_t*)P->stage_w.p + cur * hc * nvb;
        bt.a_aux_density = z.a_aux_density;
        bt.b_input_density = z.b_input_density;
        bt.b_aux_density = z.b_aux_density;
        zk_status rc = prove_batch_dev(P, np, &bt, rs + first * 64, proofs_out + first * 192);
        copier.join();
        if (rc != ZK_OK) return rc;
        if (next_rc != ZK_OK) return fail(next_rc, next_err);
        cur ^= 1;
    }
    return ZK_OK;
}

}

namespace {

zk_status r1cs_load(uint32_t n_in, uint32_t n_aux, uint32_t n_con, const zk_csr* const mats[3], int device, zk_r1cs** out) {
    ZK_TRY(use_device(device));
    if (n_in == 0) return fail(ZK_ERR_INVALID_ARGUMENT, "n_inputs must include ONE");
    zk_r1cs* R = new (std::nothrow) zk_r1cs();
    if (!R) return fail(ZK_ERR_OUT_OF_MEMORY, "host allocation failed");
    struct Guard {
        zk_r1cs* p;
        ~Guard() { delete p; }
    } guard{R};
    R->device = device;
    static std::atomic<uint64_t> next_id{1};
    R->id = next_id++;
    R->n_in = n_in;
    R->n_aux = n_aux;
    R->n_con = n_con;
    const uint32_t nv = n_in + n_aux;
    R->a_aux_density.assign(n_aux, 0);
    R->b_input_density.assign(n_in, 0);
    R->b_aux_density.assign(n_aux, 0);
    for (int m = 0; m < 3; m++) {
        const zk_csr* M = mats[m];
        if (!M || !M->row_ptr || (n_con && M->row_ptr[n_con] && (!M->col || !M->coeff)))
            return fail(ZK_ERR_INVALID_ARGUMENT, "null matrix pointer");
        if (M->row_ptr[0] != 0) return fail(ZK_ERR_INVALID_ARGUMENT, "row_ptr[0] must be 0");
        for (uint32_t r = 0; r < n_con; r++)
            if (M->row_ptr[r + 1] < M->row_ptr[r]) return fail(ZK_ERR_INVALID_ARGUMENT, "row_ptr is not monotone");
        const uint32_t nnz = M->row_ptr[n_con];
        for (uint32_t k = 0; k < nnz; k++) {
            const uint32_t v = M->col[k];
            if (v >= nv) return fail(ZK_ERR_INVALID_ARGUMENT, "variable index out of range in matrix " + std::to_string(m));
            uint64_t c[4];
            load_scalar_le(M->coeff + (size_t)k * 32, c);
            if (!scalar_lt_r(c)) return fail(ZK_ERR_INVALID_ARGUMENT, "coefficient is not < r");
            if (m == 0 && v >= n_in) R->a_aux_density[v - n_in] = 1;
            if (m == 1) {
                if (v >= n_in)
                    R->b_aux_density[v - n_in] = 1;
                else
                    R->b_input_density[v] = 1;
            }
        }
        R->h_row_ptr[m].assign(M->row_ptr, M->row_ptr + n_con + 1);
        R->h_col[m].assign(M->col, M->col + nnz);
        R->h_coeff[m].resize(nnz);
        for (uint32_t k = 0; k < nnz; k++) {
            zkhost::Fr c;
            load_scalar_le(M->coeff + (size_t)k * 32, c.l);
            R->h_coeff[m][k] = c.to_mont();
        }
        ZK_TRY(R->row_ptr[m].ensure(((size_t)n_con + 1) * 4));
        ZK_TRY(R->col[m].ensure((size_t)(nnz ? nnz : 1) * 4));
        ZK_TRY(R->coeff[m].ensure((size_t)(nnz ? nnz : 1) * 32));
        HIP_TRY(hipMemcpy(R->row_ptr[m].p, M->row_ptr, ((size_t)n_con + 1) * 4, hipMemcpyHostToDevice));
        if (nnz) {
            HIP_TRY(hipMemcpy(R->col[m].p, M->col, (size_t)nnz * 4, hipMemcpyHostToDevice));
            HIP_TRY(hipMemcpy(R->coeff[m].p, M->coeff, (size_t)nnz * 32, hipMemcpyHostToDevice));
            ZK_LAUNCH(zkdev::k_fr_convert, dim3((nnz + 255) / 256), dim3(256), 0, g_stream, R->coeff[m].as<uint32_t>(),
                      (const uint32_t*)R->coeff[m].as<uint32_t>(), 0u, (size_t)nnz);
        }
    }
    HIP_TRY(hipGetLastError());
    HIP_TRY(hipStreamSynchronize(g_stream));
    guard.p = nullptr;
    *out = R;
    return ZK_OK;
}

zk_status ensure_derived(zk_params* P, zk_r1cs* R) {
    if (P->drv.ready && P->drv.circuit == R->id) return ZK_OK;
    const uint32_t n_in = R->n_in, n_aux = R->n_aux, nv = n_in + n_aux, n_con = R->n_con, n_rows = n_con + n_in, k = P->log_m;
    const size_t m = P->m;
    if (!P->g1.table.owned || R->h_row_ptr[2].size() != (size_t)n_con + 1 || n_in != P->n_ic || n_aux != P->n_l ||
        (size_t)n_con + n_in > m || P->n_h + 1 != m)
        return ZK_OK;
    ZK_TRY(use_device(P->device));
    const auto t0 = std::chrono::steady_clock::now();
    typedef zkdev::XYZZ<zkdev::Fq> DP;
    typedef zkdev::Affine<zkdev::Fq> DA;
    P->drv.ready = false;
    const DA* key = P->g1.table.as<DA>();
    const std::vector<uint32_t>& rp = R->h_row_ptr[2];
    const std::vector<uint32_t>& cl = R->h_col[2];
    const uint32_t nnz = rp[n_con];
    std::vector<uint32_t> ptr(nv + 1, 0), t_row(nnz ? nnz : 1), each(n_rows + 1);
    std::vector<Fr> t_s(nnz ? nnz : 1);
    for (uint32_t e = 0; e < nnz; e++) ptr[cl[e] + 1]++;
    for (uint32_t i = 0; i < nv; i++) ptr[i + 1] += ptr[i];
    {
        std::vector<uint32_t> at(ptr.begin(), ptr.end() - 1);
        for (uint32_t row = 0; row < n_con; row++)
            for (uint32_t e = rp[row]; e < rp[row + 1]; e++) {
                const uint32_t slot = at[cl[e]]++;
                t_row[slot] = row;
                t_s[slot] = R->h_coeff[2][e].from_mont();
            }
    }
    for (uint32_t i = 0; i <= n_rows; i++) each[i] = i;
    std::vector<int32_t> idx(m + nv);
    for (size_t pos = 0; pos < m; pos++) {
        const uint32_t e = k ? (__builtin_bitreverse32((uint32_t)pos) >> (32 - k)) : 0;
        idx[pos] = e < P->n_h ? (int32_t)(P->off_h + e) : -1;
    }
    for (uint32_t i = 0; i < nv; i++) idx[m + i] = i < n_in ? -1 : (int32_t)(P->off_l + (i - n_in));
    const size_t rows = std::max<size_t>(m, nnz), n_set = 2 * (size_t)n_rows + nv;
    DevBuf d_idx, d_ptr, d_each, d_row, d_s, d_tw, d_w, d_sl, d_sm, d_se, src, ping, pong, lam, mk, terms, tbl, all, stage;
    for (DevBuf* b : {&d_idx, &d_ptr, &d_each, &d_row, &d_s, &d_tw, &d_w, &d_sl, &d_sm, &d_se, &src, &ping, &pong, &lam, &mk, &terms, &tbl, &all, &stage})
        b->is_public = true;
    ZK_TRY(d_idx.ensure(idx.size() * 4));
    ZK_TRY(d_ptr.ensure(ptr.size() * 4));
    ZK_TRY(d_each.ensure(each.size() * 4));
    ZK_TRY(d_row.ensure(t_row.size() * 4));
    ZK_TRY(d_s.ensure(t_s.size() * 32));
    ZK_TRY(d_tw.ensure(m * 32));
    ZK_TRY(d_w.ensure(5 * 32));
    ZK_TRY(d_sl.ensure(m * 32));
    ZK_TRY(d_sm.ensure(m * 32));
    ZK_TRY(d_se.ensure((size_t)n_rows * 32));
    ZK_TRY(src.ensure((m + nv) * sizeof(DP)));
    ZK_TRY(ping.ensure(m * sizeof(DP)));
    ZK_TRY(pong.ensure(m * sizeof(DP)));
    ZK_TRY(lam.ensure(m * sizeof(DP)));
    ZK_TRY(mk.ensure(m * sizeof(DP)));
    ZK_TRY(terms.ensure(std::max<size_t>(nnz ? nnz : 1, n_rows) * sizeof(DP)));
    ZK_TRY(tbl.ensure(15 * rows * sizeof(DP)));
    ZK_TRY(all.ensure(n_set * sizeof(DP)));
    HIP_TRY(hipMemcpy(d_idx.p, idx.data(), idx.size() * 4, hipMemcpyHostToDevice));
    HIP_TRY(hipMemcpy(d_ptr.p, ptr.data(), ptr.size() * 4, hipMemcpyHostToDevice));
    HIP_TRY(hipMemcpy(d_each.p, each.data(), each.size() * 4, hipMemcpyHostToDevice));
    HIP_TRY(hipMemcpy(d_row.p, t_row.data(), t_row.size() * 4, hipMemcpyHostToDevice));
    HIP_TRY(hipMemcpy(d_s.p, t_s.data(), t_s.size() * 32, hipMemcpyHostToDevice));
    const Fr ninv2 = P->ntt.n_inv * P->ntt.n_inv;
    const Fr wv[5] = {P->ntt.w_inv, Fr::one(), ninv2, -ninv2, fr_from_u64((uint64_t)m) * P->ntt.z_inv};
    HIP_TRY(hipMemcpy(d_w.p, wv, sizeof(wv), hipMemcpyHostToDevice));
    const uint32_t* cw = d_w.as<uint32_t>();
    auto table = [&](DevBuf& out, const uint32_t* base, const uint32_t* scale, uint32_t mode, size_t count) {
        ZK_LAUNCH(zkdev::k_fr_pow_table, dim3((unsigned)((count + 255) / 256)), dim3(256), 0, g_stream, out.as<uint32_t>(), base, scale,
                  k, mode, 1u, (uint32_t)count);
    };
    if (m > 1) table(d_tw, cw, cw + 8, 0, m / 2);
    table(d_sl, cw + 8, cw + 16, 2, m);
    table(d_sm, cw + 8, cw + 24, 3, m);
    table(d_se, cw + 8, cw + 32, 2, n_rows);
    zkcoop::basis_gather(key, d_idx.as<int32_t>(), src.as<DP>(), (uint32_t)(m + nv), g_stream);
    auto transform = [&](const uint32_t* scale, DP* out) -> zk_status {
        DP *a = ping.as<DP>(), *b = pong.as<DP>();
        zkcoop::basis_scale(src.as<DP>(), nullptr, scale, tbl.as<DP>(), k ? a : out, (uint32_t)m, g_stream);
        for (uint32_t st = 0; st < k; st++) {
            zkcoop::basis_dft_stage(a, st + 1 == k ? out : b, d_tw.as<uint32_t>(), tbl.as<DP>(), k, st, g_stream);
            std::swap(a, b);
        }
        HIP_TRY(hipGetLastError());
        return ZK_OK;
    };
    ZK_TRY(transform(d_sl.as<uint32_t>(), lam.as<DP>()));
    ZK_TRY(transform(d_sm.as<uint32_t>(), mk.as<DP>()));
    DP* set = all.as<DP>();
    HIP_TRY(hipMemcpyAsync(set, lam.p, (size_t)n_rows * sizeof(DP), hipMemcpyDeviceToDevice, g_stream));
    zkcoop::basis_scale(lam.as<DP>(), nullptr, d_se.as<uint32_t>(), tbl.as<DP>(), terms.as<DP>(), n_rows, g_stream);
    zkcoop::basis_segment_sums(mk.as<DP>(), terms.as<DP>(), d_each.as<uint32_t>(), set + n_rows, n_rows, g_stream);
    if (nnz) zkcoop::basis_scale(mk.as<DP>(), d_row.as<uint32_t>(), d_s.as<uint32_t>(), tbl.as<DP>(), terms.as<DP>(), nnz, g_stream);
    zkcoop::basis_segment_sums(src.as<DP>() + m, terms.as<DP>(), d_ptr.as<uint32_t>(), set + 2 * (size_t)n_rows, nv, g_stream);
    HIP_TRY(hipGetLastError());
    std::vector<HG1> host(n_set);
    ZK_TRY(P->g1.normalize_to_host(set, n_set, host.data(), stage, g_stream));
    HIP_TRY(hipStreamSynchronize(g_stream));
    std::vector<HG1A> pts(n_set);
    P->drv.pos.assign(n_set, -1);
    size_t live = 0;
    for (size_t i = 0; i < n_set; i++) {
        pts[i] = host[i].is_inf() ? HG1A::inf() : HG1A{host[i].x, host[i].y};
        if (!host[i].is_inf()) {
            P->drv.pos[i] = (int32_t)i;
            if (i < n_rows || i >= 2 * (size_t)n_rows) live++;
        }
    }
    const uint32_t c_set = pick_window(live + P->n_b1, 1);
    ZK_TRY(P->g1d.build_with_tail(pts, P->g1, P->off_a, P->g1.n_points - P->off_a, c_set));
    P->g1d_lone.alias(P->g1d, P->g1_lone.c);
    P->drv.n_rows = n_rows;
    P->drv.off_a = (uint32_t)n_set;
    P->drv.off_b1 = P->drv.off_a + P->n_a + 2;
    P->drv.circuit = R->id;
    static std::atomic<uint32_t> serial{1};
    P->drv.serial = serial++;
    P->drv.bind_ms = std::chrono::duration<double, std::milli>(std::chrono::steady_clock::now() - t0).count();
    P->drv.ready = true;
    if (getenv("ZKAMD_TRACE_HOST"))
        fprintf(stderr, "[zkamd] derived bases: 2 x %u + %u points, %u entries of C, width %u, %.1f ms, table %.2f GB\n", n_rows, nv, nnz,
                c_set, P->drv.bind_ms, (double)P->g1d.bytes / 1e9);
    return ZK_OK;
}

zk_status prove_from_z(zk_params* P, zk_r1cs* R, size_t np, int slot, const uint8_t* rs, uint8_t* proofs_out, bool derived) {
    const uint32_t nv = R->n_in + R->n_aux, n_rows = R->n_con + R->n_in;
    if (derived) {
        ZK_TRY(ensure_derived(P, R));
        derived = P->drv.ready && P->drv.circuit == R->id;
    }
    ZK_TRY(R->abc.ensure(3 * np * (size_t)n_rows * 32));
    zkdev::R1csMat mm[3];
    for (int m = 0; m < 3; m++)
        mm[m] = zkdev::R1csMat{R->row_ptr[m].as<uint32_t>(), R->col[m].as<uint32_t>(), R->coeff[m].as<uint32_t>()};
    {
        ProfScope ps("r1cs_eval");
        ZK_LAUNCH(zkdev::k_r1cs_eval, dim3((n_rows + 255) / 256, 3, (unsigned)np), dim3(256), 0, g_stream, mm[0], mm[1], mm[2],
                  (const uint32_t*)R->z[slot].as<uint32_t>(), R->abc.as<uint32_t>(), R->n_con, R->n_in, nv, n_rows,
                  np * (size_t)n_rows);
    }
    HIP_TRY(hipGetLastError());
    zk_batch_dev bt;
    bt.n_rows = n_rows;
    bt.n_inputs = R->n_in;
    bt.n_aux = R->n_aux;
    bt.flags = ZK_FR_MONTGOMERY;
    bt.d_a = R->abc.as<uint32_t>();
    bt.d_b = R->abc.as<uint32_t>() + np * (size_t)n_rows * 8;
    bt.d_c = R->abc.as<uint32_t>() + 2 * np * (size_t)n_rows * 8;
    bt.d_wit = R->z[slot].p;
    bt.a_aux_density = R->a_aux_density.data();
    bt.b_input_density = R->b_input_density.data();
    bt.b_aux_density = R->b_aux_density.data();
    return prove_batch_dev(P, np, &bt, rs, proofs_out, derived);
}

zk_status prove_batch_witness(zk_params* P, zk_r1cs* R, size_t n, const uint8_t* witness, uint32_t flags, const uint8_t* rs,
                              uint8_t* proofs_out, bool derived) {
    if (!P || !R || !witness || !rs || !proofs_out) return fail(ZK_ERR_INVALID_ARGUMENT, "null argument");
    if (n == 0) return ZK_OK;
    if (R->device != P->device) return fail(ZK_ERR_INVALID_ARGUMENT, "parameters and circuit live on different devices");
    ZK_TRY(use_device(P->device));
    const uint32_t nv = R->n_in + R->n_aux, n_rows = R->n_con + R->n_in;
    if (n_rows > P->m) return fail(ZK_ERR_POLYNOMIAL_DEGREE_TOO_LARGE, "more rows than the key's evaluation domain");
    const size_t chunk = ProveTunables::read().batch_chunk;
    for (size_t first = 0; first < n; first += chunk) {
        const size_t np = std::min(chunk, n - first);
        ZK_TRY(R->z[0].ensure(np * (size_t)nv * 32));
        HIP_TRY(hipMemcpyAsync(R->z[0].p, witness + first * (size_t)nv * 32, np * (size_t)nv * 32, hipMemcpyHostToDevice, g_stream));
        ZK_TRY(P->bad.ensure(8));
        HIP_TRY(hipMemsetAsync(P->bad.as<uint32_t>() + 1, 0, 4, g_stream));
        if (!(flags & ZK_FR_MONTGOMERY)) {
            const size_t cnt = np * (size_t)nv;
            ZK_LAUNCH(zkdev::k_fr_convert, dim3((unsigned)((cnt + 255) / 256)), dim3(256), 0, g_stream, R->z[0].as<uint32_t>(),
                      (const uint32_t*)R->z[0].as<uint32_t>(), 0u, cnt, P->bad.as<uint32_t>() + 1);
        }
        ZK_TRY(prove_from_z(P, R, np, 0, rs + first * 64, proofs_out + first * 192, derived));
        if (P->pin_bad.as<uint32_t>()[1] & zkdev::ZK_BAD_SCALAR)
            return fail(ZK_ERR_INVALID_ARGUMENT, "a witness scalar is not a canonical field element (>= r)");
    }
    return ZK_OK;
}

}

namespace {

zk_status transfer_decode(const zk_transfer_statement& in, size_t index, zkwit::Statement* out) {
    static const uint64_t FS[4] = ZK_JUBJUB_FS_MODULUS_64;
    auto scalar = [&](const uint8_t* b, uint64_t (&v)[4], const char* what) -> zk_status {
        load_scalar_le(b, v);
        for (int i = 3; i >= 0; i--) {
            if (v[i] < FS[i]) return ZK_OK;
            if (v[i] > FS[i]) break;
        }
        return fail(ZK_ERR_INVALID_ARGUMENT, "statement " + std::to_string(index) + ": " + what + " is not a canonical Fs scalar");
    };
    auto point = [&](const uint8_t* b, zkwit::JPoint* p, const char* what) -> zk_status {
        if (!zkwit::decode_point(b, p))
            return fail(ZK_ERR_INVALID_ARGUMENT, "statement " + std::to_string(index) + ": " + what + " is not a Jubjub point");
        return ZK_OK;
    };
    out->amount = in.amount;
    out->remaining_balance = in.remaining_balance;
// ... 410 lines not shown
    }
    HIP_TRY(hipGetLastError());
    return ZK_OK;
}

}

namespace zkrt {
zk_status lib_prove_from_z(zk_params* P, zk_r1cs* R, size_t np, int slot, const uint8_t* rs, uint8_t* proofs_out) {
    return prove_from_z(P, R, np, slot, rs, proofs_out, true);
}
size_t lib_batch_chunk() { return ProveTunables::read().batch_chunk; }
bool lib_witness_on_host(size_t n) { return witness_on_host(n); }
int lib_params_device(const zk_params* P) { return P->device; }
size_t lib_params_domain(const zk_params* P) { return P->m; }
}

extern "C" {

const char* zk_strerror(zk_status st) {
    switch (st) {
        case ZK_OK: return "ok";
        case ZK_ERR_ASSIGNMENT_MISSING: return "an assignment for a variable could not be computed";
        case ZK_ERR_DIVISION_BY_ZERO: return "division by zero";
        case ZK_ERR_UNSATISFIABLE: return "unsatisfiable constraint system";
        case ZK_ERR_POLYNOMIAL_DEGREE_TOO_LARGE: return "polynomial degree is too large";
        case ZK_ERR_UNEXPECTED_IDENTITY: return "encountered an identity element in the CRS";
        case ZK_ERR_IO: return "encountered an I/O error";
        case ZK_ERR_MALFORMED_VERIFYING_KEY: return "malformed verifying key";
        case ZK_ERR_UNCONSTRAINED_VARIABLE: return "auxiliary variable was unconstrained";
        case ZK_ERR_INVALID_ARGUMENT: return "invalid argument";
        case ZK_ERR_DEVICE: return "HIP runtime error";
        case ZK_ERR_NO_DEVICE: return "no HIP device";
        case ZK_ERR_OUT_OF_MEMORY: return "out of memory";
    }
    return "unknown status";
}
const char* zk_last_error(void) { return g_err.c_str(); }
void zk_set_host_threads(int n) { g_host_threads = n > 0 ? n : 0; }

zk_status zk_device_count(int* count) try {
    if (!count) return fail(ZK_ERR_INVALID_ARGUMENT, "null argument");
    int n = 0;
    if (hipGetDeviceCount(&n) != hipSuccess) n = 0;
    *count = n;
    return ZK_OK;
} ZK_ABI_CATCH

zk_status zk_params_load(const uint8_t* pk_bytes, size_t len, int checked, int device, zk_params** out) try {
    if (!pk_bytes || !out) return fail(ZK_ERR_INVALID_ARGUMENT, "null argument");
    *out = nullptr;
    return params_load(pk_bytes, len, checked, device, out);
} ZK_ABI_CATCH
zk_status zk_params_get_info(const zk_params* p, zk_params_info* info) try {
    if (!p || !info) return fail(ZK_ERR_INVALID_ARGUMENT, "null argument");
    info->n_ic = p->n_ic;
    info->n_h = p->n_h;
    info->n_l = p->n_l;
    info->n_a = p->n_a;
    info->n_b_g1 = p->n_b1;
    info->n_b_g2 = p->n_b2;
    info->log_domain = p->log_m;
    info->window_bits = p->g1.c;
    info->n_windows = zkdev::MSM_NPOS;
    info->device = (uint32_t)p->device;
    info->device_bytes = p->g1.bytes + p->g2.bytes + p->ntt.bytes;
    return ZK_OK;
} ZK_ABI_CATCH
zk_status zk_params_get_windows(const zk_params* p, uint32_t out[4]) try {
    if (!p || !out) return fail(ZK_ERR_INVALID_ARGUMENT, "null argument");
    out[0] = p->g1.c;
    out[1] = p->g1a.c;
    out[2] = p->g1_lone.c;
    out[3] = p->g2.c;
    return ZK_OK;
} ZK_ABI_CATCH
zk_status zk_params_get_merged(const zk_params* p, uint32_t out[3]) try {
    if (!p || !out) return fail(ZK_ERR_INVALID_ARGUMENT, "null argument");
    out[0] = p->grp_a.merged();
    out[1] = p->grp_b1.merged();
    out[2] = p->grp_b2.merged();
    return ZK_OK;
} ZK_ABI_CATCH
void zk_params_free(zk_params* p) { delete p; }
zk_status zk_params_write_vk(const zk_params* p, uint8_t* out, size_t cap, size_t* len) try {
    if (!p || !len) return fail(ZK_ERR_INVALID_ARGUMENT, "null argument");
    *len = p->vk_bytes.size();
    if (out) {
        if (cap < p->vk_bytes.size()) return fail(ZK_ERR_INVALID_ARGUMENT, "output buffer too small");
        memcpy(out, p->vk_bytes.data(), p->vk_bytes.size());
    }
    return ZK_OK;
} ZK_ABI_CATCH

zk_status zk_prove(zk_params* p, const zk_assignment* asg, const uint8_t r[32], const uint8_t s[32], uint8_t proof_out[192]) try {
    if (!r || !s) return fail(ZK_ERR_INVALID_ARGUMENT, "null argument");
    uint8_t rs[64];
    memcpy(rs, r, 32);
    memcpy(rs + 32, s, 32);
    return prove_batch_host(p, 1, asg, rs, proof_out);
} ZK_ABI_CATCH
zk_status zk_prove_batch(zk_params* p, size_t n, const zk_assignment* asgs, const uint8_t* rs, uint8_t* proofs_out) try {
    return prove_batch_host(p, n, asgs, rs, proofs_out);
} ZK_ABI_CATCH
zk_status zk_prove_batch_dev(zk_params* p, size_t n, const zk_batch_dev* batch, const uint8_t* rs, uint8_t* proofs_out) try {
    return prove_batch_dev(p, n, batch, rs, proofs_out);
} ZK_ABI_CATCH

zk_status zk_r1cs_load(uint32_t n_inputs, uint32_t n_aux, uint32_t n_constraints, const zk_csr* a, const zk_csr* b,
                       const zk_csr* c, int device, zk_r1cs** out) try {
    if (!out) return fail(ZK_ERR_INVALID_ARGUMENT, "null argument");
    *out = nullptr;
    const zk_csr* mats[3] = {a, b, c};
    return r1cs_load(n_inputs, n_aux, n_constraints, mats, device, out);
} ZK_ABI_CATCH
void zk_r1cs_free(zk_r1cs* r) { delete r; }

static const zkr1cs::System& transfer_system_cached() {
    static const zkr1cs::System sys = zkr1cs::transfer_system();
    return sys;
}
zk_status zk_transfer_r1cs_fingerprint(uint8_t hash_out[32], uint32_t* n_inputs, uint32_t* n_aux, uint32_t* n_constraints) try {
    const zkr1cs::System& sys = transfer_system_cached();
    if (hash_out) sys.fingerprint(hash_out);
    if (n_inputs) *n_inputs = sys.n_inputs;
    if (n_aux) *n_aux = sys.n_aux;
    if (n_constraints) *n_constraints = sys.n_constraints;
    return ZK_OK;
} ZK_ABI_CATCH
static zk_status system_load(const zkr1cs::System& sys, int device, zk_r1cs** out) {
    std::vector<uint8_t> coeff[3];
    zk_csr mats[3];
    for (int m = 0; m < 3; m++) {
        const zkr1cs::Csr& M = sys.m[m];
        coeff[m].resize(M.coeff.size() * 32 + 32);
        for (size_t k = 0; k < M.coeff.size(); k++) {
            const zkhost::Fr p = M.coeff[k].from_mont();
            memcpy(&coeff[m][k * 32], p.l, 32);
        }
        mats[m].row_ptr = M.row_ptr.data();
        mats[m].col = M.col.data();
        mats[m].coeff = coeff[m].data();
    }
    const zk_csr* ptrs[3] = {&mats[0], &mats[1], &mats[2]};
    return r1cs_load(sys.n_inputs, sys.n_aux, sys.n_constraints, ptrs, device, out);
}
zk_status zk_transfer_r1cs_load(int device, zk_r1cs** out) try {
    if (!out) return fail(ZK_ERR_INVALID_ARGUMENT, "null argument");
    *out = nullptr;
    const zkr1cs::System& sys = transfer_system_cached();
    if (sys.n_inputs != ZK_TRANSFER_N_INPUTS || sys.n_aux != ZK_TRANSFER_N_AUX)
        return fail(ZK_ERR_INVALID_ARGUMENT, "internal: emitted system has the wrong shape");
    return system_load(sys, device, out);
} ZK_ABI_CATCH
static const zkr1cs::System& anonymous_system_cached() {
    static const zkr1cs::System sys = zkr1cs::anonymous_system();
    return sys;
}
zk_status zk_anonymous_r1cs_fingerprint(uint8_t hash_out[32], uint32_t* n_inputs, uint32_t* n_aux, uint32_t* n_constraints) try {
    const zkr1cs::System& sys = anonymous_system_cached();
    if (hash_out) sys.fingerprint(hash_out);
    if (n_inputs) *n_inputs = sys.n_inputs;
    if (n_aux) *n_aux = sys.n_aux;
    if (n_constraints) *n_constraints = sys.n_constraints;
    return ZK_OK;
} ZK_ABI_CATCH
zk_status zk_anonymous_r1cs_load(int device, zk_r1cs** out) try {
    if (!out) return fail(ZK_ERR_INVALID_ARGUMENT, "null argument");
    *out = nullptr;
    const zkr1cs::System& sys = anonymous_system_cached();
    if (sys.n_inputs != ZK_ANONYMOUS_N_INPUTS || sys.n_aux != ZK_ANONYMOUS_N_AUX)
        return fail(ZK_ERR_INVALID_ARGUMENT, "internal: emitted system has the wrong shape");
    return system_load(sys, device, out);
} ZK_ABI_CATCH
zk_status zk_prove_batch_witness(zk_params* p, zk_r1cs* circuit, size_t n, const uint8_t* witness, uint32_t flags,
                                 const uint8_t* rs, uint8_t* proofs_out) try {
    return prove_batch_witness(p, circuit, n, witness, flags, rs, proofs_out, false);
} ZK_ABI_CATCH
#ifdef ZK_TEST_HOOKS
zk_status zk_hook_prove_batch_witness_derived(zk_params* p, zk_r1cs* circuit, size_t n, const uint8_t* witness, uint32_t flags,
                                              const uint8_t* rs, uint8_t* proofs_out, uint32_t info[2]) try {
    const zk_status rc = prove_batch_witness(p, circuit, n, witness, flags, rs, proofs_out, true);
    if (info && p && circuit) {
        info[0] = p->drv.ready && p->drv.circuit == circuit->id ? 1u : 0u;
        info[1] = (uint32_t)std::count(p->drv.pos.begin(), p->drv.pos.end(), -1);
    }
    return rc;
} ZK_ABI_CATCH
zk_status zk_hook_derived_layout(zk_params* p, zk_r1cs* circuit, uint32_t info[7]) try {
    if (!p || !circuit || !info) return fail(ZK_ERR_INVALID_ARGUMENT, "null argument");
    std::fill(info, info + 7, 0u);
    const zk_params::Derived& D = p->drv;
    if (!D.ready || D.circuit != circuit->id) return ZK_OK;
    info[0] = 1;
    info[1] = info[2] = D.n_rows;
    info[3] = (uint32_t)D.pos.size() - 2 * D.n_rows;
    info[4] = D.off_a;
    info[5] = D.off_b1;
    info[6] = p->g1d.c;
    return ZK_OK;
} ZK_ABI_CATCH
zk_status zk_hook_prove_plan(size_t np, uint32_t n_in, uint32_t n_aux, uint32_t n_rows, size_t m, uint32_t ga, uint32_t gb2, uint32_t gb1,
                             int derived, uint64_t* out, size_t out_words) try {
    if (!out || out_words < 32) return fail(ZK_ERR_INVALID_ARGUMENT, "output too short");
    const ProveTunables tun = ProveTunables::read();
    const ProvePlan p = prove_plan(np, n_in, n_aux, n_rows, m, ga, gb2, gb1, derived != 0, tun);
    const CJobLayout& L = p.layout;
    const uint64_t f[32] = {p.fold_in_msm, p.host_norm, p.g2_lone, p.split, p.one_stream, (uint64_t)p.g1, (uint64_t)p.map,
                            tun.batch_chunk, tun.host_chunk, tun.trace_host,
                            L.n_in, L.n_aux, L.head, L.ga, L.gb2, L.gb1, L.fold, L.derived, L.w_one, L.w_sum_a, L.w_sum_b2, L.wstride,
                            L.aux, L.rz, L.r, L.sz, L.s, L.rs, L.in_tail, L.sum_b1, L.sum_a, L.cstride};
    std::copy(f, f + 32, out);
    return ZK_OK;
} ZK_ABI_CATCH
#endif

zk_status zk_transfer_witness(const zk_transfer_statement* st, size_t n, uint32_t flags, uint8_t* witness_out) try {
    return transfer_witness(st, n, flags, witness_out);
} ZK_ABI_CATCH
zk_status zk_anonymous_witness(const zk_anonymous_statement* st, size_t n, uint32_t flags, uint8_t* witness_out) try {
    return anonymous_witness(st, n, flags, witness_out);
} ZK_ABI_CATCH
zk_status zk_transfer_prove_batch(zk_params* p, zk_r1cs* circuit, size_t n, const zk_transfer_statement* st,
                                  const uint8_t* rs, uint8_t* proofs_out) try {
    if (!p || !circuit || !rs || !proofs_out || (!st && n)) return fail(ZK_ERR_INVALID_ARGUMENT, "null argument");
    if (circuit->n_in != ZK_TRANSFER_N_INPUTS || circuit->n_aux != ZK_TRANSFER_N_AUX)
        return fail(ZK_ERR_INVALID_ARGUMENT, "the loaded constraint matrices are not the transfer circuit's");
    if (circuit->device != p->device) return fail(ZK_ERR_INVALID_ARGUMENT, "parameters and circuit live on different devices");
    if (n == 0) return ZK_OK;
    const size_t nv = ZK_TRANSFER_N_INPUTS + ZK_TRANSFER_N_AUX;
    const size_t chunk = ProveTunables::read().batch_chunk;
    zk_status rc = use_device(p->device);
    if (rc != ZK_OK) return rc;
    if ((size_t)circuit->n_con + circuit->n_in > p->m)
        return fail(ZK_ERR_POLYNOMIAL_DEGREE_TOO_LARGE, "more rows than the key's evaluation domain");
    if (!witness_on_host(n)) {
        int slot = 0;
        ZK_TRY(witness_gpu_enqueue(circuit, st, std::min(chunk, n), slot, g_copy_stream));
        for (size_t first = 0; first < n; first += chunk) {
            const size_t np = std::min(chunk, n - first), next = first + chunk;
            ZK_TRY(witness_gpu_finish(circuit, np, slot, first));
            if (next < n) ZK_TRY(witness_gpu_enqueue(circuit, st + next, std::min(chunk, n - next), slot ^ 1, g_copy_stream));
            ZK_TRY(prove_from_z(p, circuit, np, slot, rs + first * 64, proofs_out + first * 192, true));
            slot ^= 1;
        }
        return ZK_OK;
    }
    const size_t cap = std::min(chunk, n) * nv * 32;
    rc = circuit->host_ensure(2 * cap);
    if (rc != ZK_OK) return rc;
    uint8_t* buf[2] = {(uint8_t*)circuit->host_z, (uint8_t*)circuit->host_z + cap};
    rc = transfer_witness(st, std::min(chunk, n), ZK_FR_MONTGOMERY, buf[0]);
    if (rc != ZK_OK) return rc;
    int cur = 0;
    for (size_t first = 0; first < n; first += chunk) {
        const size_t np = std::min(chunk, n - first);
        const size_t next = first + chunk;
        zk_status next_rc = ZK_OK;
        std::string next_err;
        SideThread producer;
        if (next < n)
            producer.start([&, next] {
                next_rc = transfer_witness(st + next, std::min(chunk, n - next), ZK_FR_MONTGOMERY, buf[cur ^ 1], next);
                if (next_rc != ZK_OK) next_err = g_err;
            });
        rc = prove_batch_witness(p, circuit, np, buf[cur], ZK_FR_MONTGOMERY, rs + first * 64, proofs_out + first * 192, true);
        producer.join();
        if (rc != ZK_OK) return rc;
        if (next_rc != ZK_OK) return fail(next_rc, next_err);
        cur ^= 1;
    }
    return ZK_OK;
} ZK_ABI_CATCH

zk_status zk_anonymous_prove_batch(zk_params* p, zk_r1cs* circuit, size_t n, const zk_anonymous_statement* st, const uint8_t* rs,
                                   uint8_t* proofs_out) try {
    if (!p || !circuit || !rs || !proofs_out || (!st && n)) return fail(ZK_ERR_INVALID_ARGUMENT, "null argument");
    if (circuit->n_in != ZK_ANONYMOUS_N_INPUTS || circuit->n_aux != ZK_ANONYMOUS_N_AUX)
        return fail(ZK_ERR_INVALID_ARGUMENT, "the loaded constraint matrices are not the anonymous-transfer circuit's");
    if (n == 0) return ZK_OK;
    ZK_TRY(use_device(p->device));
    const size_t nv = ZK_ANONYMOUS_N_INPUTS + ZK_ANONYMOUS_N_AUX;
    size_t chunk = ProveTunables::read().batch_chunk;
    if (chunk > 512) chunk = 512;
    if (!witness_on_host(n)) {
        if (circuit->device != p->device) return fail(ZK_ERR_INVALID_ARGUMENT, "parameters and circuit live on different devices");
        int slot = 0;
        zk_status rc = witness_anon_gpu_enqueue(circuit, st, std::min(chunk, n), slot, g_copy_stream);
        for (size_t first = 0; first < n && rc == ZK_OK; first += chunk) {
            const size_t np = std::min(chunk, n - first), next = first + chunk;
            rc = witness_anon_gpu_finish(circuit, np, slot, first);
            if (rc == ZK_OK && next < n) rc = witness_anon_gpu_enqueue(circuit, st + next, std::min(chunk, n - next), slot ^ 1, g_copy_stream, next);
            if (rc == ZK_OK) rc = prove_from_z(p, circuit, np, slot, rs + first * 64, proofs_out + first * 192, true);
            slot ^= 1;
        }
// ... 558 lines not shown
```

Baseline: 4433.

## Merge equal-valued witness scalars into pre-summed MSM bases via value-pair chains

Adds setup-time detection, from seeded probe witnesses, of chains of witness variables that usually hold the same full-width value in the A, B and L/aux multiexps. The build-scalars kernel checks equality at run time and, where a pair matches, writes the scalar once into an extra slot for a pre-summed base. It zeroes the two original slots so the bucket MSMs should do fewer point additions. The cost is longer scalar vectors, chain walks and extra memory traffic in the scalar kernel, and more precomputed bases in the parameters.

```diff
diff --git a/include/zkamd.h b/include/zkamd.h
--- a/include/zkamd.h
+++ b/include/zkamd.h
@@ -50,6 +50,7 @@
 zk_status zk_params_get_info(const zk_params* p, zk_params_info* info);
 zk_status zk_params_get_windows(const zk_params* p, uint32_t out[4]);
 zk_status zk_params_get_merged(const zk_params* p, uint32_t out[3]);
+zk_status zk_params_get_pairs(const zk_params* p, uint32_t out[8]);
 void zk_params_free(zk_params* p);
 
 typedef struct {
diff --git a/include/zkamd_sys.rs b/include/zkamd_sys.rs
--- a/include/zkamd_sys.rs
+++ b/include/zkamd_sys.rs
@@ -294,6 +294,7 @@
     pub fn zk_params_get_info(p: *const zk_params, info: *mut zk_params_info) -> zk_status;
     pub fn zk_params_get_windows(p: *const zk_params, out: *mut [u32; 4]) -> zk_status;
     pub fn zk_params_get_merged(p: *const zk_params, out: *mut [u32; 3]) -> zk_status;
+    pub fn zk_params_get_pairs(p: *const zk_params, out: *mut [u32; 8]) -> zk_status;
     pub fn zk_params_free(p: *mut zk_params);
     pub fn zk_prove(
         p: *mut zk_params,
diff --git a/zero-chain_amd/_api.py b/zero-chain_amd/_api.py
--- a/zero-chain_amd/_api.py
+++ b/zero-chain_amd/_api.py
@@ -182,6 +182,13 @@
         n = (C.c_uint32 * 3)()
         self._lib.check(self._lib.zk_params_get_merged(self._h, n))
         return tuple(int(x) for x in n)
+
+    @property
+    def value_pairs(self):
+        n = (C.c_uint32 * 8)()
+        self._lib.check(self._lib.zk_params_get_pairs(self._h, n))
+        names = ("a", "b_g1", "b_g2", "l")
+        return {"bases": dict(zip(names, (int(x) for x in n[:4]))), "expected_merges": dict(zip(names, (int(x) for x in n[4:])))}
 
     @property
     def vk(self):
diff --git a/zero-chain_amd/_lib.py b/zero-chain_amd/_lib.py
--- a/zero-chain_amd/_lib.py
+++ b/zero-chain_amd/_lib.py
@@ -117,6 +117,7 @@
     "zk_params_get_info": (C.c_int32, [C.c_void_p, C.POINTER(ParamsInfo)]),
     "zk_params_get_windows": (C.c_int32, [C.c_void_p, C.POINTER(C.c_uint32)]),
     "zk_params_get_merged": (C.c_int32, [C.c_void_p, C.POINTER(C.c_uint32)]),
+    "zk_params_get_pairs": (C.c_int32, [C.c_void_p, C.POINTER(C.c_uint32)]),
     "zk_bind_host_to_device": (C.c_int32, [C.c_int, C.POINTER(C.c_int), C.POINTER(C.c_int)]),
     "zk_params_free": (None, [C.c_void_p]),
     "zk_prove": (C.c_int32, [C.c_void_p, C.POINTER(Assignment), C.c_void_p, C.c_void_p, C.c_void_p]),
diff --git a/zero-chain_amd/csrc/msm_group.h b/zero-chain_amd/csrc/msm_group.h
--- a/zero-chain_amd/csrc/msm_group.h
+++ b/zero-chain_amd/csrc/msm_group.h
@@ -176,6 +176,14 @@
         return ZK_OK;
     }
     zk_status run(std::vector<MsmJob>& jobs, std::vector<HPoint>& out);
+    zk_status count_pairs(size_t nj, uint64_t* total) {
+        std::vector<uint32_t> h(nj * (size_t)nb);
+        *total = 0;
+        if (h.empty() || !cnt.p) return ZK_OK;
+        HIP_TRY(hipMemcpy(h.data(), cnt.p, h.size() * 4, hipMemcpyDeviceToHost));
+        for (uint32_t x : h) *total += x;
+        return ZK_OK;
+    }
 
 private:
     zk_status launch_table_build(DevBuf& scratch, hipStream_t st);
diff --git a/zero-chain_amd/csrc/ntt.h b/zero-chain_amd/csrc/ntt.h
--- a/zero-chain_amd/csrc/ntt.h
+++ b/zero-chain_amd/csrc/ntt.h
@@ -267,11 +267,43 @@
     st_fr(out + (size_t)mat * out_mat_stride * 8 + (p * n_rows + row) * 8, acc);
 }
 
+constexpr uint32_t PAIR_WALK_MAX = 32;
+ZK_DI uint32_t pair_decide(const int32_t* __restrict__ pairs, uint32_t nv, const uint32_t* __restrict__ zp, uint32_t i, const Fr& raw,
+                           uint32_t* emit, uint32_t mask = 15u) {
+    uint32_t own = 15u;
+    *emit = 0u;
+    if (raw == Fr::zero()) return own;
+    const int32_t* q = pairs + 6 * (size_t)nv;
+#pragma unroll 1
+    for (uint32_t c = 0; c < 3; c++) {
+        if (!(mask & (c == 0 ? 1u : c == 1 ? 10u : 4u))) continue;
+        const int32_t* pred = pairs + 2 * c * (size_t)nv;
+        const int32_t* succ = pred + nv;
+        uint32_t t = 0;
+        for (int32_t k = pred[i]; k >= 0 && t < PAIR_WALK_MAX && ld_fr(zp + (size_t)k * 8) == raw; k = pred[k]) t++;
+        int32_t e = -1;
+        if (t & 1u) {
+            e = (int32_t)i;
+            *emit |= c == 0 ? 1u : c == 1 ? 10u : 4u;
+        } else {
+            const int32_t sc = succ[i];
+            if (sc >= 0 && ld_fr(zp + (size_t)sc * 8) == raw) e = sc;
+        }
+        if (e >= 0) {
+            if (c == 0 && q[e] >= 0) own &= ~1u;
+            if (c == 1 && q[nv + e] >= 0) own &= ~2u;
+            if (c == 2 && q[2 * (size_t)nv + e] >= 0) own &= ~4u;
+            if (c == 1 && q[3 * (size_t)nv + e] >= 0) own &= ~8u;
+        }
+    }
+    return own;
+}
 static __global__ void __launch_bounds__(256)
 k_build_scalars(uint32_t* wit_out, uint32_t* cvec, const uint32_t* __restrict__ wit, const uint32_t* __restrict__ tail,
-                const zkrt::CJobLayout L, uint32_t mont, uint32_t* bad, const uint32_t* __restrict__ groups) {
+                const zkrt::CJobLayout L, uint32_t mont, uint32_t* bad, const uint32_t* __restrict__ groups,
+                const int32_t* __restrict__ pairs = nullptr) {
     uint32_t i = blockIdx.x * blockDim.x + threadIdx.x;
-    if (i >= L.wstride + L.gb1) return;
+    if (i >= L.w_end + L.gb1) return;
     const size_t p = blockIdx.y;
     uint32_t* cv = cvec + p * (size_t)L.cstride * 8;
     const uint32_t nv = L.w_one, fold = L.fold;
@@ -282,17 +314,22 @@
         const uint32_t g = i - L.w_sum_a;
         const uint32_t* mem = groups + (L.ga + L.gb2 + L.gb1 + 1);
         Fr sum = Fr::zero();
+        const bool with_pairs = pairs && L.w_b2v;
+        const uint32_t bit = g < L.ga ? 1u : g < L.ga + L.gb2 ? 2u : 8u;
         for (uint32_t k = groups[g]; k < groups[g + 1]; k++) {
             const Fr raw = ld_fr(wit + (p * nv + mem[k]) * 8);
-            if (!fr_geq_r(raw)) sum = add(sum, raw);
-        }
-        if (i < L.wstride) {
+            if (fr_geq_r(raw)) continue;
+            uint32_t emit;
+            if (with_pairs && !(pair_decide(pairs, nv, wit + p * (size_t)nv * 8, mem[k], raw, &emit, bit) & bit)) continue;
+            sum = add(sum, raw);
+        }
+        if (i < L.w_end) {
             v = mont ? from_mont(sum) : sum;
             if (fold && g < L.ga) st_fr(cv + (size_t)(L.sum_a + g) * 8, mul(v, sR));
             st_fr(wit_out + (p * L.wstride + i) * 8, v);
         } else {
             const Fr rz = mont ? mul(sum, r) : mul(mul(sum, r), Fr::r2());
-            st_fr(cv + (size_t)(L.sum_b1 + (i - L.wstride)) * 8, rz);
+            st_fr(cv + (size_t)(L.sum_b1 + (i - L.w_end)) * 8, rz);
         }
         return;
     }
@@ -312,10 +349,26 @@
             v = raw;
             rz = mul(mul(raw, r), Fr::r2());
         }
-        if (i >= L.n_in) st_fr(cv + (size_t)(L.aux + (i - L.n_in)) * 8, v);
-        st_fr(cv + (size_t)(L.rz + i) * 8, rz);
-        if (fold) st_fr(cv + (size_t)(L.sz + i) * 8, mul(v, sR));
+        const Fr sz = fold ? mul(v, sR) : Fr::zero();
+        uint32_t own = 15u, emit = 0u;
+        int32_t qa = -1, qb2 = -1, ql = -1, qb1 = -1;
+        if (pairs && L.w_b2v) {
+            const int32_t* q = pairs + 6 * (size_t)nv;
+            qa = q[i]; qb2 = q[nv + i]; ql = q[2 * (size_t)nv + i]; qb1 = q[3 * (size_t)nv + i];
+            own = pair_decide(pairs, nv, wit + p * (size_t)nv * 8, i, raw, &emit);
+            const Fr zero = Fr::zero();
+            st_fr(wit_out + (p * L.wstride + L.w_b2v + i) * 8, own & 2u ? v : zero);
+            if (qa >= 0) st_fr(wit_out + (p * L.wstride + L.w_pair_a + qa) * 8, emit & 1u ? v : zero);
+            if (qb2 >= 0) st_fr(wit_out + (p * L.wstride + L.w_pair_b2 + qb2) * 8, emit & 2u ? v : zero);
+            if (ql >= 0) st_fr(cv + (size_t)(L.pair_l + ql) * 8, emit & 4u ? v : zero);
+            if (qb1 >= 0) st_fr(cv + (size_t)(L.pair_b1 + qb1) * 8, emit & 8u ? rz : zero);
+            if (fold && qa >= 0) st_fr(cv + (size_t)(L.pair_a + qa) * 8, emit & 1u ? sz : zero);
+        }
+        if (i >= L.n_in) st_fr(cv + (size_t)(L.aux + (i - L.n_in)) * 8, own & 4u ? v : Fr::zero());
+        st_fr(cv + (size_t)(L.rz + i) * 8, own & 8u ? rz : Fr::zero());
+        if (fold) st_fr(cv + (size_t)(L.sz + i) * 8, own & 1u ? sz : Fr::zero());
         if (L.in_tail && i < L.n_in) st_fr(cv + (size_t)(L.in_tail + i) * 8, v);
+        if (!(own & 1u)) v = Fr::zero();
     } else {
         v = ld_fr(tail + (p * 3 + (i - nv)) * 8);
         if (i == nv) st_fr(cv + (size_t)L.r * 8, r);
diff --git a/zero-chain_amd/csrc/prove_plan.h b/zero-chain_amd/csrc/prove_plan.h
--- a/zero-chain_amd/csrc/prove_plan.h
+++ b/zero-chain_amd/csrc/prove_plan.h
@@ -47,17 +47,33 @@
     uint32_t in_tail;
     uint32_t sum_b1, sum_a;
     uint32_t cstride;
+    uint32_t pa, pb2, pl, pb1;
+    uint32_t w_end;
+    uint32_t w_b2v, w_pair_a, w_pair_b2;
+    uint32_t pair_l, pair_b1, pair_a;
+};
+
+struct PairCounts {
+    uint32_t a = 0, b2 = 0, l = 0, b1 = 0;
+    bool any() const { return (a | b2 | l | b1) != 0; }
 };
 
 inline CJobLayout cjob_layout(uint32_t n_in, uint32_t n_aux, uint32_t head, uint32_t ga, uint32_t gb2, uint32_t gb1, bool fold,
-                              bool derived) {
+                              bool derived, const PairCounts& pc = PairCounts()) {
     const uint32_t nv = n_in + n_aux;
     CJobLayout L = {};
     L.n_in = n_in; L.n_aux = n_aux; L.head = head; L.ga = ga; L.gb2 = gb2; L.gb1 = gb1; L.fold = fold; L.derived = derived;
     L.w_one = nv;
     L.w_sum_a = nv + 3;
     L.w_sum_b2 = L.w_sum_a + ga;
-    L.wstride = L.w_sum_b2 + gb2;
+    L.w_end = L.wstride = L.w_sum_b2 + gb2;
+    L.pa = pc.a; L.pb2 = pc.b2; L.pl = pc.l; L.pb1 = pc.b1;
+    if (pc.any()) {
+        L.w_b2v = L.wstride;
+        L.w_pair_a = L.w_b2v + nv;
+        L.w_pair_b2 = L.w_pair_a + pc.a;
+        L.wstride = L.w_pair_b2 + pc.b2;
+    }
     uint32_t at = head;
     auto section = [&at](uint32_t len) { const uint32_t off = at; at += len; return off; };
     L.aux = section(n_aux);
@@ -71,6 +87,11 @@
     if (derived) L.in_tail = section(n_in);
     L.sum_b1 = section(gb1);
     if (fold) L.sum_a = section(ga);
+    if (pc.any()) {
+        L.pair_l = section(pc.l);
+        L.pair_b1 = section(pc.b1);
+        if (fold) L.pair_a = section(pc.a);
+    }
     L.cstride = at;
     return L;
 }
@@ -90,7 +111,7 @@
 };
 
 inline ProvePlan prove_plan(size_t np, uint32_t n_in, uint32_t n_aux, uint32_t n_rows, size_t m, uint32_t ga, uint32_t gb2,
-                            uint32_t gb1, bool derived, const ProveTunables& tun) {
+                            uint32_t gb1, bool derived, const ProveTunables& tun, const PairCounts& pc = PairCounts()) {
     ProvePlan p;
     p.fold_in_msm = np <= tun.fold_in_msm_max;
     p.host_norm = np <= tun.host_normalize_max;
@@ -99,7 +120,8 @@
     p.one_stream = tun.no_overlap;
     p.g1 = derived ? (p.split ? PG1::G1D : PG1::G1D_LONE) : (p.split ? PG1::G1 : PG1::G1_LONE);
     p.map = derived ? (p.fold_in_msm ? PMap::MAP_CFD : PMap::MAP_CD) : (p.fold_in_msm ? PMap::MAP_CF : PMap::MAP_C);
-    p.layout = cjob_layout(n_in, n_aux, derived ? 2 * n_rows : (uint32_t)m, ga, gb2, gb1, p.fold_in_msm, derived);
+    p.layout = cjob_layout(n_in, n_aux, derived ? 2 * n_rows : (uint32_t)m, ga, gb2, gb1, p.fold_in_msm, derived,
+                           derived ? pc : PairCounts());
     return p;
 }
 
diff --git a/zero-chain_amd/csrc/value_pairs.h b/zero-chain_amd/csrc/value_pairs.h
--- /dev/null
+++ b/zero-chain_amd/csrc/value_pairs.h
@@ -0,0 +1,177 @@
+#pragma once
+#include <stdint.h>
+#include <algorithm>
+#include <map>
+#include <array>
+#include <vector>
+#include "transfer_witness.h"
+
+namespace zkpairs {
+
+using zkhost::Fr;
+
+constexpr uint32_t CHAIN_MAX = 32;
+constexpr int N_PROBES = 8;
+
+inline bool full_width(const Fr& x) {
+    const Fr v = x.from_mont(), w = (-x).from_mont();
+    return (v.l[1] | v.l[2] | v.l[3]) != 0 && (w.l[1] | w.l[2] | w.l[3]) != 0;
+}
+
+inline std::vector<int32_t> links_from_probes(const std::vector<std::vector<Fr>>& probes, const std::vector<uint8_t>& in) {
+    const size_t nv = in.size();
+    std::vector<int32_t> pred(nv, -1);
+    std::vector<uint8_t> seen(nv, 0), clash(nv, 0);
+    for (const std::vector<Fr>& z : probes) {
+        if (z.size() != nv) continue;
+        std::map<std::array<uint64_t, 4>, int32_t> last;
+        for (size_t i = 0; i < nv; i++) {
+            if (!in[i] || !full_width(z[i])) continue;
+            const std::array<uint64_t, 4> key = {z[i].l[0], z[i].l[1], z[i].l[2], z[i].l[3]};
+            auto it = last.find(key);
+            if (it != last.end()) {
+                if (seen[i] && pred[i] != it->second) clash[i] = 1;
+                seen[i] = 1;
+                pred[i] = it->second;
+                it->second = (int32_t)i;
+            } else {
+                last.emplace(key, (int32_t)i);
+            }
+        }
+    }
+    for (size_t i = 0; i < nv; i++)
+        if (clash[i]) pred[i] = -1;
+    return pred;
+}
+
+inline std::vector<int32_t> chains_finalize(std::vector<int32_t>& pred) {
+    const size_t nv = pred.size();
+    std::vector<int32_t> succ(nv, -1);
+    std::vector<uint32_t> depth(nv, 0);
+    for (size_t i = 0; i < nv; i++) {
+        const int32_t p = pred[i];
+        if (p < 0) continue;
+        if ((size_t)p >= i || succ[p] >= 0 || depth[p] + 1 >= CHAIN_MAX) {
+            pred[i] = -1;
+            continue;
+        }
+        succ[p] = (int32_t)i;
+        depth[i] = depth[p] + 1;
+    }
+    return succ;
+}
+
+struct Seeded {
+    uint64_t s;
+    uint64_t next() {
+        uint64_t z = (s += 0x9e3779b97f4a7c15ull);
+        z = (z ^ (z >> 30)) * 0xbf58476d1ce4e5b9ull;
+        z = (z ^ (z >> 27)) * 0x94d049bb133111ebull;
+        return z ^ (z >> 31);
+    }
+    void scalar(uint64_t (&v)[4]) {
+        for (int i = 0; i < 4; i++) v[i] = next();
+        v[3] &= (1ull << 58) - 1;
+    }
+    zkwit::JPoint point() {
+        uint64_t k[4];
+        scalar(k);
+        return zkwit::fixed_base_value(zkwit::fs_bits(k));
+    }
+};
+
+inline std::vector<Fr> flat(const zkwit::Wit& w) {
+    std::vector<Fr> z(w.inputs);
+    z.insert(z.end(), w.aux.begin(), w.aux.end());
+    return z;
+}
+
+inline std::vector<std::vector<Fr>> transfer_probes() {
+    std::vector<std::vector<Fr>> out;
+    for (int k = 0; k < N_PROBES; k++) {
+        Seeded g{0x7a6b616d64000000ull + (uint64_t)k};
+        zkwit::Statement s;
+        s.amount = (uint32_t)g.next();
+        s.remaining_balance = (uint32_t)g.next();
+        s.fee = (uint32_t)g.next();
+        g.scalar(s.randomness);
+        g.scalar(s.alpha);
+        g.scalar(s.dec_key);
+        s.pgk = g.point();
+        s.enc_key_recipient = g.point();
+        s.enc_balance_left = g.point();
+        s.enc_balance_right = g.point();
+        s.g_epoch = g.point();
+        zkwit::Wit w;
+        zkwit::synthesize(s, w);
+        out.push_back(flat(w));
+    }
+    return out;
+}
+
+inline std::vector<std::vector<Fr>> anonymous_probes() {
+    std::vector<std::vector<Fr>> out;
+    for (int k = 0; k < N_PROBES; k++) {
+        Seeded g{0x7a6b616e6f6e0000ull + (uint64_t)k};
+        zkwit::AnonStatement s;
+        s.amount = (uint32_t)g.next();
+        s.remaining_balance = (uint32_t)g.next();
+        s.s_index = (uint32_t)(g.next() % zkwit::ANON_SIZE);
+        s.t_index = (uint32_t)(g.next() % zkwit::ANON_SIZE);
+        g.scalar(s.randomness);
+        g.scalar(s.alpha);
+        g.scalar(s.dec_key);
+        s.pgk = g.point();
+        s.g_epoch = g.point();
+        for (size_t i = 0; i < zkwit::ANON_SIZE; i++) {
+            s.enc_keys[i] = g.point();
+            s.left_ciphertexts[i] = g.point();
+            s.balance_left[i] = g.point();
+            s.balance_right[i] = g.point();
+        }
+        zkwit::Wit w;
+        zkwit::synthesize_anonymous(s, w);
+        out.push_back(flat(w));
+    }
+    return out;
+}
+
+enum Circuit { TRANSFER = 0, ANONYMOUS = 1 };
+
+inline const std::vector<std::vector<Fr>>& circuit_probes(Circuit c) {
+    if (c == TRANSFER) {
+        static const std::vector<std::vector<Fr>> t = transfer_probes();
+        return t;
+    }
+    static const std::vector<std::vector<Fr>> a = anonymous_probes();
+    return a;
+}
+constexpr int N_CHAINS = 3;
+
+inline std::vector<int32_t> chains_of(const std::vector<std::vector<Fr>>& probes, uint32_t n_in, const std::vector<uint8_t>& a_dense,
+                                      const std::vector<uint8_t>& b_dense) {
+    const size_t nv = a_dense.size();
+    std::vector<uint8_t> aux(nv, 0);
+    for (size_t i = n_in; i < nv; i++) aux[i] = 1;
+    std::vector<int32_t> out;
+    for (const std::vector<uint8_t>* in : {&a_dense, &b_dense, (const std::vector<uint8_t>*)&aux}) {
+        std::vector<int32_t> pred = links_from_probes(probes, *in);
+        const std::vector<int32_t> succ = chains_finalize(pred);
+        out.insert(out.end(), pred.begin(), pred.end());
+        out.insert(out.end(), succ.begin(), succ.end());
+    }
+    return out;
+}
+
+inline uint64_t count_merges(const int32_t* pred, const int32_t* q, const std::vector<Fr>& z) {
+    uint64_t merged = 0;
+    for (size_t j = 0; j < z.size(); j++) {
+        if (q[j] < 0 || z[j].is_zero()) continue;
+        uint32_t t = 0;
+        for (int32_t k = pred[j]; k >= 0 && t < CHAIN_MAX && z[k] == z[j]; k = pred[k]) t++;
+        merged += t & 1u;
+    }
+    return merged;
+}
+
+}
diff --git a/zero-chain_amd/csrc/zkamd.cpp b/zero-chain_amd/csrc/zkamd.cpp
--- a/zero-chain_amd/csrc/zkamd.cpp
+++ b/zero-chain_amd/csrc/zkamd.cpp
@@ -23,6 +23,7 @@
 #include "msm_group.h"
 #include "prove_plan.h"
 #include "transfer_witness.h"
+#include "value_pairs.h"
 #include "handles.h"
 #include "transfer_r1cs.h"
 
@@ -274,6 +275,18 @@
     } drv;
     MsmG1 g1d, g1d_lone;
     DevBuf map_cd, map_cfd;
+    struct Pairs {
+        bool ready = false;
+        std::vector<int32_t> links;
+        uint32_t base_l = 0, base_b1 = 0, base_a = 0, base_b2 = 0;
+        PairCounts n;
+        uint32_t exp_a = 0, exp_b2 = 0, exp_l = 0, exp_b1 = 0;
+    } prs;
+    MsmG1 g1da;
+    MsmG2 g2p, g2p_lone;
+    DevBuf map_ad, map_b2d, pairs_dev;
+    PairCounts mpairs;
+    std::vector<uint8_t> enc_a, enc_b1, enc_b2;
     std::vector<uint8_t> dens_key;
     DevBuf map_a, map_b2, map_c, map_cf;
     uint32_t map_nv = 0;
@@ -373,6 +386,11 @@
     group_equal_points(at_a, P->n_a, 96, P->grp_a);
     group_equal_points(at_b1, P->n_b1, 96, P->grp_b1);
     group_equal_points(at_b2, P->n_b2, 192, P->grp_b2);
+    if ((P->n_ic == ZK_TRANSFER_N_INPUTS && P->n_l == ZK_TRANSFER_N_AUX) || (P->n_ic == ZK_ANONYMOUS_N_INPUTS && P->n_l == ZK_ANONYMOUS_N_AUX)) {
+        P->enc_a.assign(at_a, at_a + (size_t)P->n_a * 96);
+        P->enc_b1.assign(at_b1, at_b1 + (size_t)P->n_b1 * 96);
+        P->enc_b2.assign(at_b2, at_b2 + (size_t)P->n_b2 * 192);
+    }
     const Section sec1[7] = {{at_h, P->n_h, "h", false},       {at_l, P->n_l, "l", false},          {at_a, P->n_a, "a", false},
                              {pk, 1, "vk.alpha_g1", true},     {pk + 576, 1, "vk.delta_g1", true},  {at_b1, P->n_b1, "b_g1", false},
                              {pk + 96, 1, "vk.beta_g1", true}};
@@ -501,6 +519,13 @@
         Q->drv = P->drv;
         Q->g1d.alias(P->g1d, P->g1d.c);
         Q->g1d_lone.alias(P->g1d, P->g1d_lone.c);
+        if (P->prs.ready) {
+            Q->prs = P->prs;
+            Q->g1da.alias(P->g1d, P->g1da.c);
+            Q->g2p.c = P->g2p.c; Q->g2p.maxd = P->g2p.maxd; Q->g2p.nb = P->g2p.nb; Q->g2p.n_points = P->g2p.n_points;
+            Q->g2p.table.borrow(P->g2p.table);
+            Q->g2p_lone.alias(P->g2p, P->g2p_lone.c);
+        }
     }
     Q->ntt.log_n = P->ntt.log_n;
     Q->ntt.n = P->ntt.n;
@@ -538,6 +563,11 @@
     return Q;
 }
 
+bool merge_values_on() {
+    const char* e = getenv("ZKAMD_MERGE_VALUES");
+    return !(e && atoi(e) == 0);
+}
+
 zk_status ensure_maps(zk_params* P, uint32_t n_in, uint32_t n_aux, const uint8_t* a_aux_d, const uint8_t* b_in_d,
                       const uint8_t* b_aux_d) {
     const char* merge_env = getenv("ZKAMD_MERGE_BASES");
@@ -551,8 +581,11 @@
     key.insert(key.end(), b_aux_d, b_aux_d + n_aux);
     for (int i = 0; i < 4; i++) key.push_back((uint8_t)((P->drv.ready ? P->drv.serial : 0u) >> (8 * i)));
     key.push_back(merge ? 1 : 0);
+    const uint32_t nv = n_in + n_aux;
+    const bool pairs = merge_values_on() && P->drv.ready && P->prs.ready && P->prs.links.size() == 10 * (size_t)nv;
+    key.push_back(pairs ? 1 : 0);
     if (key == P->dens_key) return ZK_OK;
-    const uint32_t nv = n_in + n_aux;
+    const PairCounts pc = pairs ? P->prs.n : PairCounts();
     std::vector<int32_t> ma(nv + 3, -1), mb1(nv + 3, -1), mb2(nv + 3, -1);
     std::vector<uint32_t> var_a, var_b;
     var_a.reserve(P->n_a);
@@ -654,6 +687,16 @@
             section(L.sum_a);
             query(base_a, 0, ga, off_a);
         }
+        if (L.w_b2v) {
+            section(L.pair_l);
+            for (uint32_t k = 0; k < L.pl; k++) map.push_back((int32_t)(P->prs.base_l + k));
+            section(L.pair_b1);
+            for (uint32_t k = 0; k < L.pb1; k++) map.push_back((int32_t)(P->prs.base_b1 + k));
+            if (L.fold) {
+                section(L.pair_a);
+                for (uint32_t k = 0; k < L.pa; k++) map.push_back((int32_t)(P->prs.base_a + k));
+            }
+        }
         section(L.cstride);
         if (!fits) return fail(ZK_ERR_INVALID_ARGUMENT, "internal: the C map does not follow its layout");
         return upload(dst, map);
@@ -669,8 +712,22 @@
         const zk_params::Derived& D = P->drv;
         const uint32_t head = 2 * D.n_rows;
         for (bool fold : {false, true})
-            ZK_TRY(upload_c_map(fold ? P->map_cfd : P->map_cd, cjob_layout(n_in, n_aux, head, ga, gb2, gb1, fold, true), D.pos.data(),
+            ZK_TRY(upload_c_map(fold ? P->map_cfd : P->map_cd, cjob_layout(n_in, n_aux, head, ga, gb2, gb1, fold, true, pc), D.pos.data(),
                                 D.pos.data() + head + n_in, D.pos.data() + head, D.off_a, D.off_b1));
+    }
+    if (pairs) {
+        const CJobLayout Wp = cjob_layout(n_in, n_aux, 0, ga, gb2, gb1, false, true, pc);
+        std::vector<int32_t> mad(Wp.wstride, -1), mbd(Wp.wstride, -1);
+        for (uint32_t i = 0; i < W.wstride; i++) {
+            if (ma[i] >= 0) mad[i] = (int32_t)(P->drv.off_a + ma[i]);
+            if (i >= nv) mbd[i] = mb2[i];
+        }
+        for (uint32_t i = 0; i < nv; i++) mbd[Wp.w_b2v + i] = mb2[i];
+        for (uint32_t k = 0; k < pc.a; k++) mad[Wp.w_pair_a + k] = (int32_t)(P->prs.base_a + k);
+        for (uint32_t k = 0; k < pc.b2; k++) mbd[Wp.w_pair_b2 + k] = (int32_t)(P->prs.base_b2 + k);
+        ZK_TRY(upload(P->map_ad, mad));
+        ZK_TRY(upload(P->map_b2d, mbd));
+        ZK_TRY(upload(P->pairs_dev, P->prs.links));
     }
     gptr.insert(gptr.end(), gmem.begin(), gmem.end());
     ZK_TRY(upload(P->grp_dev, gptr));
@@ -681,6 +738,7 @@
     P->mg_a = ga;
     P->mg_b2 = gb2;
     P->mg_b1 = gb1;
+    P->mpairs = pc;
     return ZK_OK;
 }
 
@@ -700,6 +758,7 @@
     const int32_t* map_c;
     uint32_t *wit, *cvec, *bad;
     const DP1* a_dev = nullptr;
+    bool pairs = false;
 
     zk_status scalars(const uint8_t* rs) {
         const CJobLayout& L = plan.layout;
@@ -727,9 +786,9 @@
         HIP_TRY(hipMemsetAsync(bad, 0, 4, g_stream));
         ZK_TRY(P->cvec.ensure(np * (size_t)L.cstride * 32));
         cvec = P->cvec.as<uint32_t>();
-        ZK_LAUNCH(zkdev::k_build_scalars, dim3((L.wstride + L.gb1 + 255) / 256, (unsigned)np), dim3(256), 0, g_stream, wit, cvec,
+        ZK_LAUNCH(zkdev::k_build_scalars, dim3((L.w_end + L.gb1 + 255) / 256, (unsigned)np), dim3(256), 0, g_stream, wit, cvec,
                   (const uint32_t*)bt->d_wit + first * (size_t)nv * 8, P->tail.as<uint32_t>(), L, mont ? 1u : 0u, bad,
-                  P->grp_dev.as<uint32_t>());
+                  P->grp_dev.as<uint32_t>(), pairs ? (const int32_t*)P->pairs_dev.as<int32_t>() : (const int32_t*)nullptr);
         return ZK_OK;
     }
 
@@ -737,7 +796,7 @@
         const uint32_t wstride = plan.layout.wstride;
         P->jobs2.clear();
         for (size_t p = 0; p < np; p++) {
-            MsmJob j2 = {wit + p * (size_t)wstride * 8, P->map_b2.as<int32_t>(), wstride, 0, (uint32_t)P->g2.n_points, 0, 0, 0};
+            MsmJob j2 = {wit + p * (size_t)wstride * 8, (pairs ? P->map_b2d : P->map_b2).as<int32_t>(), wstride, 0, (uint32_t)G2->n_points, 0, 0, 0};
             P->jobs2.push_back(j2);
         }
         HIP_TRY(hipEventRecord(g_ev_fork, g_stream));
@@ -795,15 +854,20 @@
         }
         for (size_t p = 0; p < np; p++) {
             MsmJob ja = {wit + p * (size_t)wstride * 8, P->map_a.as<int32_t>(), wstride, P->off_a, npts1, 0, 0, 0};
-            if (!split && derived) {
+            if (pairs) {
+                ja.map = P->map_ad.as<int32_t>();
+                ja.table_base = 0;
+                ja.n_table = (uint32_t)P->g1d.n_points;
+            } else if (!split && derived) {
                 ja.table_base = P->drv.off_a;
                 ja.n_table = npts1c;
             }
             (split ? P->jobs1a : P->jobs1).push_back(ja);
         }
         if (split) {
-            ZK_TRY(P->g1a.enqueue(P->jobs1a, P->res1a, side, false));
-            a_dev = P->g1a.res_dev;
+            MsmG1& G1A = pairs ? P->g1da : P->g1a;
+            ZK_TRY(G1A.enqueue(P->jobs1a, P->res1a, side, false));
+            a_dev = G1A.res_dev;
             HIP_TRY(hipEventRecord(g_ev_join, side));
             ZK_TRY(G1C->enqueue(P->jobs1, P->res1, g_stream, false));
             HIP_TRY(hipStreamWaitEvent(g_stream, g_ev_join, 0));
@@ -882,9 +946,10 @@
     const bool mont = (bt->flags & ZK_FR_MONTGOMERY) != 0;
     if (derived && (!mont || P->drv.n_rows != bt->n_rows)) return fail(ZK_ERR_INVALID_ARGUMENT, "internal: the batch is not the derived set's");
     ChunkRun c = {P, np, bt, first, derived, mont,
-                  prove_plan(np, bt->n_inputs, bt->n_aux, bt->n_rows, P->m, P->mg_a, P->mg_b2, P->mg_b1, derived, tun)};
+                  prove_plan(np, bt->n_inputs, bt->n_aux, bt->n_rows, P->m, P->mg_a, P->mg_b2, P->mg_b1, derived, tun, P->mpairs)};
+    c.pairs = c.plan.layout.w_b2v != 0;
     c.side = c.plan.one_stream ? g_stream : g_stream2;
-    c.G2 = c.plan.g2_lone ? &P->g2_lone : &P->g2;
+    c.G2 = c.pairs ? (c.plan.g2_lone ? &P->g2p_lone : &P->g2p) : (c.plan.g2_lone ? &P->g2_lone : &P->g2);
     MsmG1* const g1s[] = {&P->g1, &P->g1_lone, &P->g1d, &P->g1d_lone};
     DevBuf* const maps[] = {&P->map_c, &P->map_cf, &P->map_cd, &P->map_cfd};
     c.G1C = g1s[(int)c.plan.g1];
@@ -904,6 +969,12 @@
                 std::chrono::duration<double, std::milli>(t_wait - t_begin).count(),
                 std::chrono::duration<double, std::milli>(t_enc - t_wait).count(),
                 std::chrono::duration<double, std::milli>(t_end - t_enc).count());
+        uint64_t pc1 = 0, pa1 = 0, p2 = 0;
+        ZK_TRY(c.G1C->count_pairs(c.plan.split ? np : 2 * np, &pc1));
+        if (c.plan.split) ZK_TRY((c.pairs ? P->g1da : P->g1a).count_pairs(np, &pa1));
+        ZK_TRY(c.G2->count_pairs(np, &p2));
+        fprintf(stderr, "[zkamd] chunk of %zu: pairs per proof: %s %.0f, A set %.0f, G2 set %.0f\n", np, c.plan.split ? "C' set" : "C' and A set",
+                (double)pc1 / (double)np, (double)pa1 / (double)np, (double)p2 / (double)np);
     }
     return ZK_OK;
 }
@@ -1078,6 +1149,129 @@
     guard.p = nullptr;
     *out = R;
     return ZK_OK;
+}
+
+const zkr1cs::System& builtin_system(zkpairs::Circuit c) {
+    if (c == zkpairs::TRANSFER) {
+        static const zkr1cs::System sys = zkr1cs::transfer_system();
+        return sys;
+    }
+    static const zkr1cs::System sys = zkr1cs::anonymous_system();
+    return sys;
+}
+struct PairBases {
+    std::vector<HG1A> l, b1, a;
+    std::vector<HG2A> b2;
+};
+template <class A>
+A sum_of_two(const A& x, const A& y) {
+    typedef decltype(x.x) F;
+    return zkhost::to_affine(zkhost::padd(zkhost::Point<F>::from_affine(x), zkhost::Point<F>::from_affine(y)));
+}
+void derived_pairs(zk_params* P, const zk_r1cs* R, const std::vector<HG1A>& set, uint32_t n_rows, PairBases& out) {
+    zk_params::Pairs& X = P->prs;
+    X = zk_params::Pairs();
+    const uint32_t n_in = R->n_in, n_aux = R->n_aux, nv = n_in + n_aux;
+    zkpairs::Circuit kind;
+    if (n_in == ZK_TRANSFER_N_INPUTS && n_aux == ZK_TRANSFER_N_AUX) kind = zkpairs::TRANSFER;
+    else if (n_in == ZK_ANONYMOUS_N_INPUTS && n_aux == ZK_ANONYMOUS_N_AUX) kind = zkpairs::ANONYMOUS;
+    else return;
+    if (P->enc_a.size() != (size_t)P->n_a * 96 || P->enc_b1.size() != (size_t)P->n_b1 * 96 || P->enc_b2.size() != (size_t)P->n_b2 * 192) return;
+    std::vector<uint8_t> a_dense(nv, 1), b_dense(nv, 0);
+    for (uint32_t i = 0; i < nv; i++) {
+        if (i >= n_in) a_dense[i] = R->a_aux_density[i - n_in];
+        b_dense[i] = i < n_in ? R->b_input_density[i] : R->b_aux_density[i - n_in];
+    }
+    {
+        const zkr1cs::System& sys = builtin_system(kind);
+        if (sys.n_inputs != n_in || sys.n_aux != n_aux || sys.n_constraints != R->n_con) return;
+        std::vector<uint8_t> sa(nv, 0), sb(nv, 0);
+        for (uint32_t i = 0; i < n_in; i++) sa[i] = 1;
+        for (uint32_t v : sys.m[0].col) sa[v] = 1;
+        for (uint32_t v : sys.m[1].col) sb[v] = 1;
+        if (sa != a_dense || sb != b_dense) return;
+    }
+    const std::vector<std::vector<Fr>>& probes = zkpairs::circuit_probes(kind);
+    if (probes.empty() || probes[0].size() != nv || set.size() != 2 * (size_t)n_rows + nv) return;
+    const std::vector<int32_t> chains = zkpairs::chains_of(probes, n_in, a_dense, b_dense);
+    const int32_t *pred_a = chains.data(), *pred_b = pred_a + 2 * (size_t)nv, *pred_l = pred_a + 4 * (size_t)nv;
+    std::vector<int32_t> pa(nv, -1), pb1(nv, -1), pb2(nv, -1), pl(nv, -1);
+    uint32_t at = 0;
+    for (uint32_t i = 0; i < nv; i++)
+        if (i < n_in || R->a_aux_density[i - n_in]) pa[i] = (int32_t)at++;
+    if (at != P->n_a) return;
+    at = 0;
+    for (uint32_t i = 0; i < nv; i++)
+        if (i < n_in ? R->b_input_density[i] : R->b_aux_density[i - n_in]) pb1[i] = pb2[i] = (int32_t)at++;
+    if (at != P->n_b1 || at != P->n_b2) return;
+    for (uint32_t i = n_in; i < nv; i++)
+        if (!set[2 * (size_t)n_rows + i].is_inf()) pl[i] = (int32_t)(2 * n_rows + i);
+    struct Cand {
+        uint32_t j;
+        int32_t p, q;
+    };
+    std::vector<Cand> ca, cb1, cb2, cl;
+    for (uint32_t j = 0; j < nv; j++) {
+        int32_t p = pred_a[j];
+        if (p >= 0 && pa[j] >= 0 && pa[p] >= 0) ca.push_back({j, pa[p], pa[j]});
+        p = pred_b[j];
+        if (p >= 0 && pb1[j] >= 0 && pb1[p] >= 0) cb1.push_back({j, pb1[p], pb1[j]});
+        if (p >= 0 && pb2[j] >= 0 && pb2[p] >= 0) cb2.push_back({j, pb2[p], pb2[j]});
+        p = pred_l[j];
+        if (p >= 0 && pl[j] >= 0 && pl[p] >= 0) cl.push_back({j, pl[p], pl[j]});
+    }
+    std::vector<HG1A> sa(ca.size()), sb1(cb1.size()), sl(cl.size());
+    std::vector<HG2A> sb2(cb2.size());
+    auto g1_at = [](const std::vector<uint8_t>& enc, int32_t pos) {
+        HG1A pt = HG1A::inf();
+        if (zkhost::g1_from_uncompressed(enc.data() + (size_t)pos * 96, &pt) != zkhost::DEC_OK) pt = HG1A::inf();
+        return pt;
+    };
+    auto g2_at = [](const std::vector<uint8_t>& enc, int32_t pos) {
+        HG2A pt = HG2A::inf();
+        if (zkhost::g2_from_uncompressed(enc.data() + (size_t)pos * 192, &pt) != zkhost::DEC_OK) pt = HG2A::inf();
+        return pt;
+    };
+    const size_t total = ca.size() + cb1.size() + cb2.size() + cl.size();
+    const unsigned nthreads = host_threads(total / 64 + 1, 32);
+    auto part = [&](unsigned t) {
+        auto range = [&](size_t n, auto&& fn) {
+            for (size_t k = n * t / nthreads; k < n * (t + 1) / nthreads; k++) fn(k);
+        };
+        range(ca.size(), [&](size_t k) { sa[k] = sum_of_two(g1_at(P->enc_a, ca[k].p), g1_at(P->enc_a, ca[k].q)); });
+        range(cb1.size(), [&](size_t k) { sb1[k] = sum_of_two(g1_at(P->enc_b1, cb1[k].p), g1_at(P->enc_b1, cb1[k].q)); });
+        range(cb2.size(), [&](size_t k) { sb2[k] = sum_of_two(g2_at(P->enc_b2, cb2[k].p), g2_at(P->enc_b2, cb2[k].q)); });
+        range(cl.size(), [&](size_t k) { sl[k] = sum_of_two(set[cl[k].p], set[cl[k].q]); });
+    };
+    run_threads(nthreads, part);
+    X.links.assign(10 * (size_t)nv, -1);
+    std::copy(chains.begin(), chains.end(), X.links.begin());
+    auto keep = [&](const std::vector<Cand>& c, const auto& sums, auto& bases, int32_t* q) {
+        for (size_t k = 0; k < c.size(); k++)
+            if (!sums[k].is_inf()) {
+                q[c[k].j] = (int32_t)bases.size();
+                bases.push_back(sums[k]);
+            }
+        return (uint32_t)bases.size();
+    };
+    int32_t* q = &X.links[6 * (size_t)nv];
+    X.n.a = keep(ca, sa, out.a, q);
+    X.n.b2 = keep(cb2, sb2, out.b2, q + nv);
+    X.n.l = keep(cl, sl, out.l, q + 2 * (size_t)nv);
+    X.n.b1 = keep(cb1, sb1, out.b1, q + 3 * (size_t)nv);
+    uint64_t merged[4] = {0, 0, 0, 0};
+    for (const std::vector<Fr>& z : probes) {
+        merged[0] += zkpairs::count_merges(pred_a, q, z);
+        merged[1] += zkpairs::count_merges(pred_b, q + nv, z);
+        merged[2] += zkpairs::count_merges(pred_l, q + 2 * (size_t)nv, z);
+        merged[3] += zkpairs::count_merges(pred_b, q + 3 * (size_t)nv, z);
+    }
+    const uint64_t np = probes.size();
+    X.exp_a = (uint32_t)(merged[0] / np);
+    X.exp_b2 = (uint32_t)(merged[1] / np);
+    X.exp_l = (uint32_t)(merged[2] / np);
+    X.exp_b1 = (uint32_t)(merged[3] / np);
+    X.ready = X.n.any();
 }
 
 zk_status ensure_derived(zk_params* P, zk_r1cs* R) {
@@ -1188,11 +1382,35 @@
             if (i < n_rows || i >= 2 * (size_t)n_rows) live++;
         }
     }
-    const uint32_t c_set = pick_window(live + P->n_b1, 1);
+    PairBases pb;
+    derived_pairs(P, R, pts, n_rows, pb);
+    zk_params::Pairs& X = P->prs;
+    X.base_l = (uint32_t)pts.size();
+    pts.insert(pts.end(), pb.l.begin(), pb.l.end());
+    X.base_b1 = (uint32_t)pts.size();
+    pts.insert(pts.end(), pb.b1.begin(), pb.b1.end());
+    X.base_a = (uint32_t)pts.size();
+    pts.insert(pts.end(), pb.a.begin(), pb.a.end());
+    X.base_b2 = P->n_b2 + 2;
+    const bool values = merge_values_on();
+    const uint32_t c_set = pick_window(live + P->n_b1 - (values ? std::min<size_t>(X.exp_l + X.exp_b1, live) : 0), 1);
     ZK_TRY(P->g1d.build_with_tail(pts, P->g1, P->off_a, P->g1.n_points - P->off_a, c_set));
     P->g1d_lone.alias(P->g1d, P->g1_lone.c);
+    if (X.ready) {
+        P->g1da.alias(P->g1d, values ? pick_window(P->n_a - std::min(X.exp_a, P->n_a), 3) : P->g1a.c);
+        std::vector<HG2A> pts2(P->n_b2 + 2, HG2A::inf());
+        bool ok = P->vk_bytes.size() >= 864;
+        for (uint32_t i = 0; ok && i < P->n_b2; i++) ok = zkhost::g2_from_uncompressed(P->enc_b2.data() + (size_t)i * 192, &pts2[i]) == zkhost::DEC_OK;
+        ok = ok && zkhost::g2_from_uncompressed(P->vk_bytes.data() + 192, &pts2[P->n_b2]) == zkhost::DEC_OK &&
+             zkhost::g2_from_uncompressed(P->vk_bytes.data() + 672, &pts2[P->n_b2 + 1]) == zkhost::DEC_OK;
+        if (!ok) return fail(ZK_ERR_IO, "internal: the b_g2 query does not decode a second time");
+        pts2.insert(pts2.end(), pb.b2.begin(), pb.b2.end());
+        const uint32_t c2 = values ? pick_window(P->n_b2 - std::min(X.exp_b2, P->n_b2), 2) : P->g2.c;
+        ZK_TRY(P->g2p.build(pts2, c2, false, "pair bases (G2)"));
+        P->g2p_lone.alias(P->g2p, getenv("ZKAMD_WINDOW_BITS_G2") || c2 <= 10 ? c2 : 10u);
+    }
     P->drv.n_rows = n_rows;
-    P->drv.off_a = (uint32_t)n_set;
+    P->drv.off_a = (uint32_t)pts.size();
     P->drv.off_b1 = P->drv.off_a + P->n_a + 2;
     P->drv.circuit = R->id;
     static std::atomic<uint32_t> serial{1};
@@ -1202,6 +1420,10 @@
     if (getenv("ZKAMD_TRACE_HOST"))
         fprintf(stderr, "[zkamd] derived bases: 2 x %u + %u points, %u entries of C, width %u, %.1f ms, table %.2f GB\n", n_rows, nv, nnz,
                 c_set, P->drv.bind_ms, (double)P->g1d.bytes / 1e9);
+    if (getenv("ZKAMD_TRACE_HOST") && X.ready)
+        fprintf(stderr, "[zkamd] value pairs: bases a %u, b_g2 %u, l %u, b_g1 %u; merges expected per proof %u, %u, %u, %u; widths "
+                        "C' %u, A %u, G2 %u; G2 table %.2f GB\n", X.n.a, X.n.b2, X.n.l, X.n.b1, X.exp_a, X.exp_b2, X.exp_l, X.exp_b1,
+                c_set, P->g1da.c, P->g2p.c, (double)P->g2p.bytes / 1e9);
     return ZK_OK;
 }
 
@@ -1778,6 +2000,13 @@
     out[2] = p->grp_b2.merged();
     return ZK_OK;
 } ZK_ABI_CATCH
+zk_status zk_params_get_pairs(const zk_params* p, uint32_t out[8]) try {
+    if (!p || !out) return fail(ZK_ERR_INVALID_ARGUMENT, "null argument");
+    const zk_params::Pairs& X = p->prs;
+    const uint32_t v[8] = {X.n.a, X.n.b1, X.n.b2, X.n.l, X.exp_a, X.exp_b1, X.exp_b2, X.exp_l};
+    for (int i = 0; i < 8; i++) out[i] = p->drv.ready && X.ready ? v[i] : 0u;
+    return ZK_OK;
+} ZK_ABI_CATCH
 void zk_params_free(zk_params* p) { delete p; }
 zk_status zk_params_write_vk(const zk_params* p, uint8_t* out, size_t cap, size_t* len) try {
     if (!p || !len) return fail(ZK_ERR_INVALID_ARGUMENT, "null argument");
@@ -1812,10 +2041,7 @@
 } ZK_ABI_CATCH
 void zk_r1cs_free(zk_r1cs* r) { delete r; }
 
-static const zkr1cs::System& transfer_system_cached() {
-    static const zkr1cs::System sys = zkr1cs::transfer_system();
-    return sys;
-}
+static const zkr1cs::System& transfer_system_cached() { return builtin_system(zkpairs::TRANSFER); }
 zk_status zk_transfer_r1cs_fingerprint(uint8_t hash_out[32], uint32_t* n_inputs, uint32_t* n_aux, uint32_t* n_constraints) try {
     const zkr1cs::System& sys = transfer_system_cached();
     if (hash_out) sys.fingerprint(hash_out);
@@ -1849,10 +2075,7 @@
         return fail(ZK_ERR_INVALID_ARGUMENT, "internal: emitted system has the wrong shape");
     return system_load(sys, device, out);
 } ZK_ABI_CATCH
-static const zkr1cs::System& anonymous_system_cached() {
-    static const zkr1cs::System sys = zkr1cs::anonymous_system();
-    return sys;
-}
+static const zkr1cs::System& anonymous_system_cached() { return builtin_system(zkpairs::ANONYMOUS); }
 zk_status zk_anonymous_r1cs_fingerprint(uint8_t hash_out[32], uint32_t* n_inputs, uint32_t* n_aux, uint32_t* n_constraints) try {
     const zkr1cs::System& sys = anonymous_system_cached();
     if (hash_out) sys.fingerprint(hash_out);
@@ -1907,6 +2130,101 @@
                             L.n_in, L.n_aux, L.head, L.ga, L.gb2, L.gb1, L.fold, L.derived, L.w_one, L.w_sum_a, L.w_sum_b2, L.wstride,
                             L.aux, L.rz, L.r, L.sz, L.s, L.rs, L.in_tail, L.sum_b1, L.sum_a, L.cstride};
     std::copy(f, f + 32, out);
+    return ZK_OK;
+} ZK_ABI_CATCH
+zk_status zk_hook_prove_plan_pairs(size_t np, uint32_t n_in, uint32_t n_aux, uint32_t n_rows, size_t m, uint32_t ga, uint32_t gb2,
+                                   uint32_t gb1, int derived, const uint32_t counts[4], uint64_t* out, size_t out_words) try {
+    if (!out || !counts || out_words < 44) return fail(ZK_ERR_INVALID_ARGUMENT, "output too short");
+    PairCounts pc;
+    pc.a = counts[0]; pc.b2 = counts[1]; pc.l = counts[2]; pc.b1 = counts[3];
+    const ProveTunables tun = ProveTunables::read();
+    const ProvePlan p = prove_plan(np, n_in, n_aux, n_rows, m, ga, gb2, gb1, derived != 0, tun, pc);
+    const CJobLayout& L = p.layout;
+    const uint64_t f[44] = {p.fold_in_msm, p.host_norm, p.g2_lone, p.split, p.one_stream, (uint64_t)p.g1, (uint64_t)p.map,
+                            tun.batch_chunk, tun.host_chunk, tun.trace_host,
+                            L.n_in, L.n_aux, L.head, L.ga, L.gb2, L.gb1, L.fold, L.derived, L.w_one, L.w_sum_a, L.w_sum_b2, L.wstride,
+                            L.aux, L.rz, L.r, L.sz, L.s, L.rs, L.in_tail, L.sum_b1, L.sum_a, L.cstride,
+                            L.pa, L.pb2, L.pl, L.pb1, L.w_end, L.w_b2v, L.w_pair_a, L.w_pair_b2, L.pair_l, L.pair_b1, L.pair_a, 0};
+    std::copy(f, f + 44, out);
+    return ZK_OK;
+} ZK_ABI_CATCH
+zk_status zk_hook_pair_chains(int circuit, int32_t* out, size_t cap, uint32_t* nv_out) try {
+    if (circuit != 0 && circuit != 1) return fail(ZK_ERR_INVALID_ARGUMENT, "no such circuit");
+    const zkr1cs::System& sys = circuit ? anonymous_system_cached() : transfer_system_cached();
+    const uint32_t nv = sys.n_inputs + sys.n_aux;
+    if (nv_out) *nv_out = nv;
+    if (!out) return ZK_OK;
+    if (cap < 8 * (size_t)nv) return fail(ZK_ERR_INVALID_ARGUMENT, "output too short");
+    std::vector<uint8_t> a_dense(nv, 0), b_dense(nv, 0);
+    for (uint32_t i = 0; i < sys.n_inputs; i++) a_dense[i] = 1;
+    for (uint32_t v : sys.m[0].col) a_dense[v] = 1;
+    for (uint32_t v : sys.m[1].col) b_dense[v] = 1;
+    const std::vector<int32_t> c = zkpairs::chains_of(zkpairs::circuit_probes((zkpairs::Circuit)circuit), sys.n_inputs, a_dense, b_dense);
+    std::copy(c.begin(), c.end(), out);
+    std::copy(a_dense.begin(), a_dense.end(), out + 6 * (size_t)nv);
+    std::copy(b_dense.begin(), b_dense.end(), out + 7 * (size_t)nv);
+    return ZK_OK;
+} ZK_ABI_CATCH
+zk_status zk_hook_chains_finalize(int32_t* pred, int32_t* succ, uint32_t nv) try {
+    if (!pred || !succ) return fail(ZK_ERR_INVALID_ARGUMENT, "null argument");
+    std::vector<int32_t> p(pred, pred + nv);
+    for (int32_t& x : p)
+        if (x >= (int32_t)nv) x = -1;
+    const std::vector<int32_t> s = zkpairs::chains_finalize(p);
+    std::copy(p.begin(), p.end(), pred);
+    std::copy(s.begin(), s.end(), succ);
+    return ZK_OK;
+} ZK_ABI_CATCH
+zk_status zk_hook_build_scalars(uint32_t n_in, uint32_t n_aux, const uint32_t counts[4], const int32_t* links, const uint32_t ngroups[3],
+                                const uint32_t* groups, int fold, const uint8_t* wit, const uint8_t r[32], const uint8_t s[32],
+                                uint8_t* wit_out, size_t wit_cap, uint8_t* cvec_out, size_t cvec_cap, uint32_t layout[20]) try {
+    if (!counts || !links || !ngroups || !groups || !wit || !r || !s || !layout || !n_in) return fail(ZK_ERR_INVALID_ARGUMENT, "null argument");
+    ZK_TRY(use_device(0));
+    const uint32_t nv = n_in + n_aux;
+    PairCounts pc;
+    pc.a = counts[0]; pc.b2 = counts[1]; pc.l = counts[2]; pc.b1 = counts[3];
+    for (size_t k = 0; k < 10 * (size_t)nv; k++) {
+        const uint32_t bound = k < 6 * (size_t)nv ? nv : counts[k / nv - 6];
+        if (links[k] < -1 || links[k] >= (int32_t)bound) return fail(ZK_ERR_INVALID_ARGUMENT, "link out of range");
+    }
+    const uint32_t ng = ngroups[0] + ngroups[1] + ngroups[2];
+    for (uint32_t g = 0; g < ng; g++)
+        if (groups[g] > groups[g + 1]) return fail(ZK_ERR_INVALID_ARGUMENT, "groups are not monotone");
+    if (groups[0] != 0) return fail(ZK_ERR_INVALID_ARGUMENT, "groups do not start at 0");
+    for (uint32_t k = 0; k < groups[ng]; k++)
+        if (groups[ng + 1 + k] >= nv) return fail(ZK_ERR_INVALID_ARGUMENT, "group member out of range");
+    const CJobLayout L = cjob_layout(n_in, n_aux, 0, ngroups[0], ngroups[1], ngroups[2], fold != 0, true, pc);
+    const uint32_t f[20] = {L.wstride, L.cstride, L.w_b2v, L.w_pair_a, L.w_pair_b2, L.aux, L.rz, L.r, L.sz, L.s, L.rs, L.in_tail,
+                            L.pair_l, L.pair_b1, L.pair_a, L.w_one, L.w_sum_a, L.w_sum_b2, L.sum_b1, L.sum_a};
+    std::copy(f, f + 20, layout);
+    if (!wit_out || !cvec_out) return ZK_OK;
+    if (wit_cap < (size_t)L.wstride * 32 || cvec_cap < (size_t)L.cstride * 32) return fail(ZK_ERR_INVALID_ARGUMENT, "output too short");
+    DevBuf d_wit, d_tail, d_links, d_grp, d_out, d_cv, d_bad;
+    ZK_TRY(d_wit.ensure((size_t)nv * 32));
+    ZK_TRY(d_tail.ensure(96));
+    ZK_TRY(d_links.ensure(10 * (size_t)nv * 4));
+    const size_t grp_words = (size_t)ng + 1 + groups[ng];
+    ZK_TRY(d_grp.ensure(grp_words * 4));
+    ZK_TRY(d_out.ensure((size_t)L.wstride * 32));
+    ZK_TRY(d_cv.ensure((size_t)L.cstride * 32));
+    ZK_TRY(d_bad.ensure(8));
+    uint8_t tail[96] = {1};
+    memcpy(tail + 32, r, 32);
+    memcpy(tail + 64, s, 32);
+    HIP_TRY(hipMemcpy(d_wit.p, wit, (size_t)nv * 32, hipMemcpyHostToDevice));
+    HIP_TRY(hipMemcpy(d_tail.p, tail, 96, hipMemcpyHostToDevice));
+    HIP_TRY(hipMemcpy(d_links.p, links, 10 * (size_t)nv * 4, hipMemcpyHostToDevice));
+    HIP_TRY(hipMemcpy(d_grp.p, groups, grp_words * 4, hipMemcpyHostToDevice));
+    HIP_TRY(hipMemset(d_out.p, 0xff, (size_t)L.wstride * 32));
+    HIP_TRY(hipMemset(d_cv.p, 0xff, (size_t)L.cstride * 32));
+    HIP_TRY(hipMemset(d_bad.p, 0, 8));
+    ZK_LAUNCH(zkdev::k_build_scalars, dim3((L.w_end + L.gb1 + 255) / 256, 1u), dim3(256), 0, g_stream, d_out.as<uint32_t>(),
+              d_cv.as<uint32_t>(), (const uint32_t*)d_wit.as<uint32_t>(), (const uint32_t*)d_tail.as<uint32_t>(), L, 0u, d_bad.as<uint32_t>(),
+              (const uint32_t*)d_grp.as<uint32_t>(), (const int32_t*)d_links.as<int32_t>());
+    HIP_TRY(hipGetLastError());
+    HIP_TRY(hipStreamSynchronize(g_stream));
+    HIP_TRY(hipMemcpy(wit_out, d_out.p, (size_t)L.wstride * 32, hipMemcpyDeviceToHost));
+    HIP_TRY(hipMemcpy(cvec_out, d_cv.p, (size_t)L.cstride * 32, hipMemcpyDeviceToHost));
     return ZK_OK;
 } ZK_ABI_CATCH
 #endif
```

New measurement: 4877, median of 6. 1.1x the previous value.
